# foolwood/SiamMask

Hardware: NVIDIA H100
Metric: search-region frames/sec (127/255 SiamMask-sharp) (higher is better)
Workload: dtype f16x3 (hi+lo split fp16 operands on wgmma, f32 accumulate; f32 CUDA-core xcorr/refine)

## Files before the change

### siammask_b200/csrc/common.cuh

```cuda
#pragma once
#include <cuda.h>
#include <cuda_fp16.h>
#include <cuda_runtime.h>
#include <cstdint>
#include <cstdio>
#include <stdexcept>
#include <string>
#include <vector>

struct sm_image_desc;

namespace smk {

struct Act {
  __half* hi = nullptr;
  __half* lo = nullptr;
  int B = 0, H = 0, W = 0, C = 0;
  int sexp = 0;
  __host__ __device__ size_t numel() const { return (size_t)B * H * W * C; }
  __host__ __device__ int M() const { return B * H * W; }
};

struct ConvGeom {
  int Cin, Cout, KH, KW, stride, pad, dil;
  __host__ __device__ int out_size(int in) const { return (in + 2 * pad - dil * (KH - 1) - 1) / stride + 1; }
};

enum OutMode : int { OUT_NHWC_SPLIT = 0, OUT_NHWC_F32 = 1, OUT_NCHW_F32 = 2 };

struct Epilogue {
  const float* alpha = nullptr;
  const float* beta = nullptr;
  const __half* res_hi = nullptr;
  const __half* res_lo = nullptr;
  __half* out_hi = nullptr;
  __half* out_lo = nullptr;
  float* out_f32 = nullptr;
  int out_mode = OUT_NHWC_SPLIT;
  int relu = 0;
  int* ovf = nullptr;
};

__device__ __forceinline__ void flag_if_out_of_range(float absmax, int* ovf) {
  if (ovf != nullptr && !(absmax <= 65504.f)) atomicOr(ovf, 1);
}
constexpr int kStatusBadSlot = 2;

struct GemmSegment {
  CUtensorMap tmA[2];
  int kind;
  int mode;
  int num_kb, cblks, KW;
  int stride, pad, dil;
  int b_col0;
};

struct GemmParams {
  GemmSegment seg[2];
  int nseg;
  CUtensorMap tmB[2];
  int M, Cout, Ho, Wo;
  int n_tiles, m_tiles;
  int reverse_m;
  Epilogue ep;
};

struct GemmInput {
  Act in;
  ConvGeom g;
  int w_col0;
};

struct TrackerHp {
  double context_amount, penalty_k, window_influence, lr;
  int32_t exemplar_size, instance_size, total_stride, base_size, out_size, reserved;
};

struct CudaError : std::runtime_error {
  using std::runtime_error::runtime_error;
};

#define SMK_CUDA(expr)                                                                              \
  do {                                                                                              \
    cudaError_t _e = (expr);                                                                        \
    if (_e != cudaSuccess)                                                                          \
      throw smk::CudaError(std::string(#expr) + " failed: " + cudaGetErrorString(_e) + " at " +    \
                           __FILE__ + ":" + std::to_string(__LINE__));                              \
  } while (0)

#define SMK_CHECK(cond, msg)                                                                        \
  do {                                                                                              \
    if (!(cond)) throw std::runtime_error(std::string("check failed: ") + #cond + " — " + (msg));   \
  } while (0)

template <typename K>
inline void ensure_dynamic_smem(K kernel, int bytes, unsigned long long& done_mask) {
  int dev = 0;
  SMK_CUDA(cudaGetDevice(&dev));
  const unsigned long long bit = 1ull << (dev & 63);
  if (done_mask & bit) return;
  SMK_CUDA(cudaFuncSetAttribute(kernel, cudaFuncAttributeMaxDynamicSharedMemorySize, bytes));
  done_mask |= bit;
}


bool gemm_conv_supported(const ConvGeom& g);
void launch_gemm_conv(const Act& in, const ConvGeom& g, const __half* w_hi, const __half* w_lo, int cout_pad,
                      const Epilogue& ep, int nsplit, int num_sms, cudaStream_t st);
void launch_gemm_multi(const GemmInput* convs, int nconv, const Act* residual, int res_col0, const __half* w_hi,
                       const __half* w_lo, int cout_pad, int w_ld, const Epilogue& ep, int nsplit, int num_sms,
                       cudaStream_t st, bool reverse_m = false);

CUtensorMap make_map_tiled_nd(const __half* base, int rank, const uint64_t* dims, const uint64_t* strides_bytes,
                              const uint32_t* box, int swizzle_bytes);

bool patch_conv_supported(const Act& in, const ConvGeom& g);
void launch_conv3x3_patch(const Act& in, const ConvGeom& g, const __half* w_hi, const __half* w_lo, int w_ld,
                          const Epilogue& ep, int nsplit, int num_sms, cudaStream_t st);

void launch_stem_tc(const float* x_nchw, int B, int S, const __half* w_hi, const __half* w_lo, const float* alpha,
                    const float* beta, Act out, int num_sms, cudaStream_t st, int* ovf = nullptr);

void launch_ref_conv(const Act& in, const ConvGeom& g, const float* w_krsc_cout, const Epilogue& ep,
                     cudaStream_t st);
void launch_stem(const float* x_nchw, int B, int S, const float* w, const float* alpha, const float* beta, Act out,
                 cudaStream_t st);
void launch_maxpool3s2(const Act& in, Act out, cudaStream_t st);
void launch_xcorr_nhwc(const Act& x, int c_off, const __half* k_hi, const __half* k_lo, int kh, int kw, Act out,
                       float mul, int* ovf, cudaStream_t st, const int32_t* slots = nullptr, int num_slots = 0);
void launch_scatter_slots(const __half* src_hi, const __half* src_lo, __half* dst_hi, __half* dst_lo,
                          const int32_t* slots, int B, int num_slots, int n, int* status, cudaStream_t st);
void launch_paste_labels(const float* masks, int side, const double* maps, const uint8_t* anno, const int32_t* obj_off,
                         const int32_t* objects, int G, int H, int W, double seg_thr, uint8_t* labels, cudaStream_t st,
                         const sm_image_desc* desc = nullptr);
void launch_paste_labels_iou(const float* masks, int side, const double* maps, const uint8_t* anno,
                             const int32_t* obj_off, const int32_t* objects, const int32_t* target_ids, int G, int H,
                             int W, double seg_thr, uint8_t* labels, const double* thrs, int T, int32_t* counts,
                             cudaStream_t st, const sm_image_desc* desc = nullptr);
void launch_label_boxes(const uint8_t* anno, int G, int H, int W, const int32_t* queries, int Q, int32_t* boxes,
                        cudaStream_t st, const sm_image_desc* desc = nullptr);
void launch_vot_overlap(const float* poly_a, const float* poly_b, int B, int W, int H, float* overlap, cudaStream_t st,
                        const int32_t* wh = nullptr);
void launch_absmax(const Act& a, float* slot, cudaStream_t st);
void launch_xcorr_nchw_f32(const float* x, const float* k, float* out, int planes, int H, int W, int kh, int kw,
                           cudaStream_t st);
int launch_xcorr_bulk_f32(const float* x, const float* k, float* out, int planes, int H, int W, int kh, int kw,
                          cudaStream_t st);
void launch_crop_center(const Act& in, int crop, Act out, cudaStream_t st);
void launch_refine_crop(const Act& in, const int32_t* pos, int pos_max, int scale, int padv, int size, Act out,
                        cudaStream_t st);
void launch_gather_corr(const Act& corr, const int32_t* pos, float* out, float mul, cudaStream_t st);
void launch_gather_mask_col(const float* mask, const int32_t* pos, int B, int C, int R, float* out, cudaStream_t st);
void launch_deconv(const float* p3, const float* w, const float* bias, float* out, int B, int Cin, int N,
                   int cout, cudaStream_t st);
void launch_split_to_f32(const Act& in, float* out, cudaStream_t st, float mul = 1.f);
void launch_import_nchw(const float* x_nchw, Act out, cudaStream_t st);
void launch_warp_affine(const float* src, int sh, int sw, const double* maps, float* dst, int dh, int dw, float border,
                        int B, cudaStream_t st, const sm_image_desc* dst_desc = nullptr);
void launch_tracker_prepare(int B, const double* state, const int32_t* avg, const TrackerHp& hp, int32_t* boxes,
                            double* tsz, double* aux, cudaStream_t st);
void launch_tracker_update(int B, double* state, const float* rec, const double* aux, const int32_t* imsize,
                           const TrackerHp& hp, int A, int R, double* maps, double* out, cudaStream_t st,
                           const double* hp_table = nullptr);
void launch_crop_resize(const uint8_t* frames, size_t frame_stride, int H, int W, const int32_t* box, int B, int model,
                        float* out, cudaStream_t st, const int32_t* frame_idx = nullptr,
                        const sm_image_desc* desc = nullptr);
void launch_select(const float* cls, const float* loc, const float* anchors, const float* window, const double* tsz,
                   int B, int A, int R, double penalty_k, double window_influence, int32_t* best_idx, int32_t* pos,
                   float* rec, cudaStream_t st, const double* hp = nullptr);
void launch_mask_iou(const float* masks, int side, const double* maps, const uint8_t* anno, const int32_t* video, int B,
                     int H, int W, const double* thrs, int T, int32_t* counts, cudaStream_t st);
void launch_small_conv3x3_maps(const float* a, const float* b, int B, int Hi, int Wi, int Ho, int Wo, int Cin, int Cout,
                               const int* ymap, const int* xmap, const float* w, const float* bias, int relu,
                               float* out, cudaStream_t st);
std::vector<int> nearest_index_table(int out_size, int in_size);
int gemm_cout_pad(int cout);

}
```

### siammask_b200/csrc/conv_gemm_sm90.cu

```cuda
#include "common.cuh"
#include "ptx.cuh"

#include <cstdlib>
#include <cstring>
#include <mutex>
#include <unordered_map>

namespace smk {

namespace {

constexpr int BLOCK_M = 128;
constexpr int BLOCK_K = 64;
constexpr int CIN_GRAIN = 64;
constexpr int MMA_K = 16;
constexpr int SMEM_LIMIT = 227 * 1024;
constexpr int NUM_CONSUMER_WARPS = 8;
constexpr int NUM_THREADS = 128 + 32 * NUM_CONSUMER_WARPS;
constexpr int PRODUCER_REGS = 40;
constexpr int CONSUMER_REGS = 232;

template <int BLOCK_N, int NSPLIT>
struct Cfg {
  static constexpr int A_TILE_BYTES = BLOCK_M * BLOCK_K * 2;
  static constexpr int B_TILE_BYTES = BLOCK_N * BLOCK_K * 2;
  static constexpr int STAGE_BYTES = NSPLIT * (A_TILE_BYTES + B_TILE_BYTES);
  static constexpr int RAW_STAGES = (SMEM_LIMIT - 2048) / STAGE_BYTES;
  static constexpr int STAGES = RAW_STAGES > 6 ? 6 : RAW_STAGES;
  static constexpr int SMEM_BYTES = STAGES * STAGE_BYTES + 1024  + 256 ;
  static constexpr int ACC = BLOCK_N / 2;
  static_assert(STAGES >= 2, "pipeline needs at least two stages");
  static_assert(BLOCK_N % 16 == 0 && BLOCK_N >= 16 && BLOCK_N <= 128, "N tile (register accumulators)");
  static_assert(B_TILE_BYTES % 1024 == 0, "stage parts stay 1024-aligned (swizzle atoms)");
  static_assert(SMEM_BYTES <= SMEM_LIMIT, "shared memory budget");
};

__device__ __forceinline__ int m_block(const GemmParams& p, int tile) {
  const int mb = tile / p.n_tiles;
  return p.reverse_m ? p.m_tiles - 1 - mb : mb;
}

template <int BLOCK_N, int NSPLIT>
__global__ void __launch_bounds__(NUM_THREADS, 1) conv_gemm_kernel(const __grid_constant__ GemmParams p) {
  using C = Cfg<BLOCK_N, NSPLIT>;
  constexpr int STAGES = C::STAGES;
  constexpr int A_TILE_BYTES = C::A_TILE_BYTES;

  extern __shared__ uint8_t smem_raw[];
  uint8_t* smem = reinterpret_cast<uint8_t*>((reinterpret_cast<uintptr_t>(smem_raw) + 1023) & ~uintptr_t(1023));
  uint64_t* full_bar = reinterpret_cast<uint64_t*>(smem + STAGES * C::STAGE_BYTES);
  uint64_t* empty_bar = full_bar + STAGES;

  const int warp = __shfl_sync(0xffffffffu, (int)(threadIdx.x >> 5), 0);
  const int lane = threadIdx.x & 31;
  const int num_tiles = p.m_tiles * p.n_tiles;

  if (threadIdx.x == 0) {
    for (int i = 0; i < NSPLIT; ++i) {
      for (int sgi = 0; sgi < p.nseg; ++sgi) tma_prefetch_desc(&p.seg[sgi].tmA[i]);
      tma_prefetch_desc(&p.tmB[i]);
    }
    for (int s = 0; s < STAGES; ++s) {
      mbar_init(&full_bar[s], 1);
      mbar_init(&empty_bar[s], NUM_CONSUMER_WARPS);
    }
    fence_barrier_init();
  }
  __syncthreads();

  if (warp < 4) {
    setmaxnreg_dec<PRODUCER_REGS>();
    if (warp != 0) return;
    const bool leader = elect_one();
    int stage = 0;
    uint32_t phase = 0;
    auto acquire = [&](uint32_t bytes) {
      mbar_wait(&empty_bar[stage], phase ^ 1);
      if (leader) mbar_arrive_expect_tx(&full_bar[stage], bytes);
    };
    auto load_2d = [&](void* dst, const CUtensorMap* map, int c0, int c1) {
      if (leader) tma_load_2d(dst, map, &full_bar[stage], c0, c1);
    };
    for (int tile = blockIdx.x; tile < num_tiles; tile += gridDim.x) {
      const int m0 = m_block(p, tile) * BLOCK_M;
      const int n0 = (tile % p.n_tiles) * BLOCK_N;
      const int q = m0 % p.Wo;
      const int t = m0 / p.Wo;
      const int pq = t % p.Ho;
      const int nb = t / p.Ho;
      for (int sgi = 0; sgi < p.nseg; ++sgi) {
        const GemmSegment& sg = p.seg[sgi];
        if (sg.kind == 1) {
#pragma unroll 1
          for (int kb = 0; kb < BLOCK_N / BLOCK_K; ++kb) {
            acquire(C::STAGE_BYTES);
            uint8_t* st = smem + stage * C::STAGE_BYTES;
#pragma unroll
            for (int s = 0; s < NSPLIT; ++s) {
              load_2d(st + s * A_TILE_BYTES, &sg.tmA[s], n0 + kb * BLOCK_K, m0);
              load_2d(st + NSPLIT * A_TILE_BYTES + s * C::B_TILE_BYTES, &p.tmB[s], sg.b_col0 + n0 + kb * BLOCK_K, n0);
            }
            __syncwarp();
            if (++stage == STAGES) { stage = 0; phase ^= 1; }
          }
          continue;
        }
        const int wb = q * sg.stride - sg.pad;
        const int hb = pq * sg.stride - sg.pad;
#pragma unroll 1
        for (int kb = 0; kb < sg.num_kb; ++kb) {
          acquire(C::STAGE_BYTES);
          uint8_t* st = smem + stage * C::STAGE_BYTES;
          const int tap = kb / sg.cblks;
          const int c0 = (kb - tap * sg.cblks) * BLOCK_K;
#pragma unroll
          for (int s = 0; s < NSPLIT; ++s) {
            uint8_t* a_dst = st + s * A_TILE_BYTES;
            if (sg.mode == 0) {
              load_2d(a_dst, &sg.tmA[s], c0, m0);
            } else if (leader) {
              const int r = tap / sg.KW;
              const int sx = tap - r * sg.KW;
              tma_load_im2col_4d(a_dst, &sg.tmA[s], &full_bar[stage], c0, wb, hb, nb,
                                 static_cast<uint16_t>(sx * sg.dil), static_cast<uint16_t>(r * sg.dil));
            }
            load_2d(st + NSPLIT * A_TILE_BYTES + s * C::B_TILE_BYTES, &p.tmB[s], sg.b_col0 + kb * BLOCK_K, n0);
          }
          __syncwarp();
          if (++stage == STAGES) { stage = 0; phase ^= 1; }
        }
      }
    }
    return;
  }

  setmaxnreg_inc<CONSUMER_REGS>();
  const int wg = (warp >> 2) - 1;
  const int wl = warp & 3;
  const Epilogue& ep = p.ep;
  const int HoWo = p.Ho * p.Wo;
  float acc[C::ACC];
  float acc2[C::ACC];
  int stage = 0;
  uint32_t phase = 0;
  for (int tile = blockIdx.x; tile < num_tiles; tile += gridDim.x) {
#pragma unroll
    for (int i = 0; i < C::ACC; ++i) { acc[i] = 0.f; acc2[i] = 0.f; }
    int prev = -1;
    for (int sgi = 0; sgi < p.nseg; ++sgi) {
      const GemmSegment& sg = p.seg[sgi];
      const bool ident = sg.kind == 1;
      const int nkb = ident ? BLOCK_N / BLOCK_K : sg.num_kb;
#pragma unroll 1
      for (int kb = 0; kb < nkb; ++kb) {
        mbar_wait(&full_bar[stage], phase);
        const uint32_t a_hi = smem_u32(smem + stage * C::STAGE_BYTES) + wg * (64 * BLOCK_K * 2);
        const uint32_t b_hi = smem_u32(smem + stage * C::STAGE_BYTES) + NSPLIT * A_TILE_BYTES;
        const uint64_t da_hi0 = wgmma_desc_kmajor<128>(a_hi);
        const uint64_t db_hi0 = wgmma_desc_kmajor<128>(b_hi);
        const uint64_t da_lo0 = wgmma_desc_kmajor<128>(a_hi + A_TILE_BYTES);
        const uint64_t db_lo0 = wgmma_desc_kmajor<128>(b_hi + C::B_TILE_BYTES);
        wgmma_fence();
#pragma unroll
        for (int k = 0; k < BLOCK_K / MMA_K; ++k) {
          const uint64_t kadd = static_cast<uint64_t>(k * MMA_K * 2 / 16);
          wgmma_f16<BLOCK_N>(acc, da_hi0 + kadd, db_hi0 + kadd);
          if constexpr (NSPLIT == 2) {
            wgmma_f16<BLOCK_N>(acc2, da_hi0 + kadd, db_lo0 + kadd);
            wgmma_f16<BLOCK_N>(acc2, da_lo0 + kadd, db_hi0 + kadd);
          }
        }
        wgmma_commit();
        wgmma_wait<1>();
        if (prev >= 0) {
          __syncwarp();
          if (lane == 0) mbar_arrive(&empty_bar[prev]);
        }
        prev = stage;
        if (++stage == STAGES) { stage = 0; phase ^= 1; }
      }
    }
    wgmma_wait<0>();
    fence_regs(acc);
    if constexpr (NSPLIT == 2) fence_regs(acc2);
    __syncwarp();
    if (lane == 0) mbar_arrive(&empty_bar[prev]);

    const int row0 = m_block(p, tile) * BLOCK_M + wg * 64 + wl * 16 + (lane >> 2);
    const int col0 = (tile % p.n_tiles) * BLOCK_N + 2 * (lane & 3);
    float amax = 0.f;
#pragma unroll
    for (int h = 0; h < 2; ++h) {
      const int m = row0 + 8 * h;
      if (m >= p.M) continue;
      const int b = m / HoWo;
      const int hw = m - b * HoWo;
#pragma unroll
      for (int j = 0; j < BLOCK_N / 8; ++j) {
        const int n = col0 + 8 * j;
        float v0 = acc[4 * j + 2 * h], v1 = acc[4 * j + 2 * h + 1];
        if constexpr (NSPLIT == 2) {
          v0 += acc2[4 * j + 2 * h];
          v1 += acc2[4 * j + 2 * h + 1];
        }
        const float2 al = __ldg(reinterpret_cast<const float2*>(ep.alpha + n));
        const float2 be = __ldg(reinterpret_cast<const float2*>(ep.beta + n));
        v0 = fmaf(v0, al.x, be.x);
        v1 = fmaf(v1, al.y, be.y);
        const size_t off = static_cast<size_t>(m) * p.Cout + n;
        if (ep.res_hi != nullptr) {
          const float2 f = __half22float2(*reinterpret_cast<const __half2*>(ep.res_hi + off));
          v0 += f.x;
          v1 += f.y;
          if (ep.res_lo != nullptr) {
            const float2 l = __half22float2(*reinterpret_cast<const __half2*>(ep.res_lo + off));
            v0 += l.x;
            v1 += l.y;
          }
        }
        if (ep.relu) {
          v0 = fmaxf(v0, 0.f);
          v1 = fmaxf(v1, 0.f);
        }
        if (ep.out_mode == OUT_NHWC_SPLIT) {
          amax = fmaxf(amax, fmaxf(fabsf(v0), fabsf(v1)));
          const __half2 hv = __floats2half2_rn(v0, v1);
          const float2 hf = __half22float2(hv);
          *reinterpret_cast<__half2*>(ep.out_hi + off) = hv;
          if (ep.out_lo != nullptr)
            *reinterpret_cast<__half2*>(ep.out_lo + off) = __floats2half2_rn(v0 - hf.x, v1 - hf.y);
        } else if (ep.out_mode == OUT_NHWC_F32) {
          *reinterpret_cast<float2*>(ep.out_f32 + off) = make_float2(v0, v1);
        } else if (n < p.Cout) {
          float* dst = ep.out_f32 + (static_cast<size_t>(b) * p.Cout + n) * HoWo + hw;
          __stcs(dst, v0);
          if (n + 1 < p.Cout) __stcs(dst + HoWo, v1);
        }
      }
    }
    if (ep.out_mode == OUT_NHWC_SPLIT) flag_if_out_of_range(amax, ep.ovf);
  }
}

using EncodeTiledFn = CUresult (*)(CUtensorMap*, CUtensorMapDataType, cuuint32_t, void*, const cuuint64_t*,
                                   const cuuint64_t*, const cuuint32_t*, const cuuint32_t*, CUtensorMapInterleave,
                                   CUtensorMapSwizzle, CUtensorMapL2promotion, CUtensorMapFloatOOBfill);
using EncodeIm2colFn = CUresult (*)(CUtensorMap*, CUtensorMapDataType, cuuint32_t, void*, const cuuint64_t*,
                                    const cuuint64_t*, const int*, const int*, cuuint32_t, cuuint32_t,
                                    const cuuint32_t*, CUtensorMapInterleave, CUtensorMapSwizzle,
                                    CUtensorMapL2promotion, CUtensorMapFloatOOBfill);

struct DriverApi {
  EncodeTiledFn tiled = nullptr;
  EncodeIm2colFn im2col = nullptr;
  int driver_version = 0;
};

const DriverApi& driver_api() {
  static DriverApi api;
  static std::once_flag once;
  std::call_once(once, [] {
    void* fn = nullptr;
    cudaDriverEntryPointQueryResult q;
    SMK_CUDA(cudaGetDriverEntryPoint("cuTensorMapEncodeTiled", &fn, cudaEnableDefault, &q));
    SMK_CHECK(fn != nullptr && q == cudaDriverEntryPointSuccess, "cuTensorMapEncodeTiled not available");
    api.tiled = reinterpret_cast<EncodeTiledFn>(fn);
    fn = nullptr;
    SMK_CUDA(cudaGetDriverEntryPoint("cuTensorMapEncodeIm2col", &fn, cudaEnableDefault, &q));
    SMK_CHECK(fn != nullptr && q == cudaDriverEntryPointSuccess, "cuTensorMapEncodeIm2col not available");
    api.im2col = reinterpret_cast<EncodeIm2colFn>(fn);
    SMK_CUDA(cudaDriverGetVersion(&api.driver_version));
  });
  return api;
}

struct MapKey {
  uint64_t v[16];
  bool operator==(const MapKey& o) const { return std::memcmp(v, o.v, sizeof v) == 0; }
};
struct MapKeyHash {
  size_t operator()(const MapKey& k) const {
    uint64_t h = 0x9E3779B97F4A7C15ull;
    for (uint64_t x : k.v) { h ^= x + 0x9E3779B97F4A7C15ull + (h << 6) + (h >> 2); }
    return (size_t)h;
  }
};
template <typename F>
CUtensorMap cached_map(const MapKey& key, F&& encode) {
  static std::mutex mu;
  static std::unordered_map<MapKey, CUtensorMap, MapKeyHash> cache;
  int dev = 0;
  cudaGetDevice(&dev);
  MapKey k = key;
  k.v[15] = (uint64_t)dev;
  std::lock_guard<std::mutex> lock(mu);
  auto it = cache.find(k);
  if (it != cache.end()) return it->second;
  if (cache.size() > 65536) cache.clear();
  CUtensorMap m = encode();
  cache.emplace(k, m);
  return m;
}

CUtensorMap make_map_2d_raw(const __half* base, uint64_t inner, uint64_t outer, uint32_t box_inner, uint32_t box_outer) {
  CUtensorMap m;
  cuuint64_t dims[2] = {inner, outer};
  cuuint64_t strides[1] = {inner * sizeof(__half)};
  cuuint32_t box[2] = {box_inner, box_outer};
  cuuint32_t estr[2] = {1, 1};
  const CUtensorMapSwizzle sw = box_inner == 64 ? CU_TENSOR_MAP_SWIZZLE_128B : CU_TENSOR_MAP_SWIZZLE_64B;
  CUresult r = driver_api().tiled(&m, CU_TENSOR_MAP_DATA_TYPE_FLOAT16, 2, const_cast<__half*>(base), dims, strides,
                                  box, estr, CU_TENSOR_MAP_INTERLEAVE_NONE, sw,
                                  CU_TENSOR_MAP_L2_PROMOTION_L2_256B, CU_TENSOR_MAP_FLOAT_OOB_FILL_NONE);
  SMK_CHECK(r == CUDA_SUCCESS, "cuTensorMapEncodeTiled failed, code " + std::to_string((int)r));
  return m;
}

CUtensorMap make_map_2d(const __half* base, uint64_t inner, uint64_t outer, uint32_t box_inner, uint32_t box_outer) {
  MapKey k{};
  k.v[0] = 1; k.v[1] = (uint64_t)base; k.v[2] = inner; k.v[3] = outer; k.v[4] = box_inner; k.v[5] = box_outer;
  return cached_map(k, [&] { return make_map_2d_raw(base, inner, outer, box_inner, box_outer); });
}

CUtensorMap make_map_im2col_raw(const __half* base, const Act& in, const ConvGeom& g, int bk) {
  CUtensorMap m;
  cuuint64_t dims[4] = {(cuuint64_t)in.C, (cuuint64_t)in.W, (cuuint64_t)in.H, (cuuint64_t)in.B};
  cuuint64_t strides[3] = {(cuuint64_t)in.C * 2, (cuuint64_t)in.W * in.C * 2, (cuuint64_t)in.H * in.W * in.C * 2};
  int lower[2] = {-g.pad, -g.pad};
  int upper[2] = {g.pad - (g.KW - 1) * g.dil, g.pad - (g.KH - 1) * g.dil};
  cuuint32_t estr[4] = {1, (cuuint32_t)g.stride, (cuuint32_t)g.stride, 1};
  const DriverApi& api = driver_api();
  CUresult r = api.im2col(&m, CU_TENSOR_MAP_DATA_TYPE_FLOAT16, 4, const_cast<__half*>(base), dims, strides, lower,
                          upper, bk, BLOCK_M, estr, CU_TENSOR_MAP_INTERLEAVE_NONE,
                          bk == 64 ? CU_TENSOR_MAP_SWIZZLE_128B : CU_TENSOR_MAP_SWIZZLE_64B,
                          CU_TENSOR_MAP_L2_PROMOTION_L2_256B, CU_TENSOR_MAP_FLOAT_OOB_FILL_NONE);
  SMK_CHECK(r == CUDA_SUCCESS, "cuTensorMapEncodeIm2col failed, code " + std::to_string((int)r));
  if (api.driver_version <= 13010 && in.numel() * sizeof(__half) < 131072)
    reinterpret_cast<uint64_t*>(&m)[1] &= ~(1ull << 21);
  return m;
}

CUtensorMap make_map_im2col(const __half* base, const Act& in, const ConvGeom& g, int bk) {
  MapKey k{};
  k.v[0] = 3; k.v[1] = (uint64_t)base;
  k.v[2] = ((uint64_t)in.B << 32) | (uint32_t)in.H; k.v[3] = ((uint64_t)in.W << 32) | (uint32_t)in.C;
  k.v[4] = ((uint64_t)g.KH << 32) | (uint32_t)g.KW; k.v[5] = ((uint64_t)g.stride << 32) | (uint32_t)g.pad;
  k.v[6] = ((uint64_t)g.dil << 32) | (uint32_t)bk;
  return cached_map(k, [&] { return make_map_im2col_raw(base, in, g, bk); });
}

template <int BLOCK_N, int NSPLIT>
void launch_cfg(const GemmParams& p, int num_sms, cudaStream_t st) {
  using C = Cfg<BLOCK_N, NSPLIT>;
  auto kern = conv_gemm_kernel<BLOCK_N, NSPLIT>;
  static unsigned long long attr_done = 0;
  ensure_dynamic_smem(kern, C::SMEM_BYTES, attr_done);
  const int tiles = p.m_tiles * p.n_tiles;
  const int grid = tiles < num_sms ? tiles : num_sms;
  kern<<<grid, NUM_THREADS, C::SMEM_BYTES, st>>>(p);
  SMK_CUDA(cudaGetLastError());
}

}

static CUtensorMap make_map_2d_any_raw(const __half* base, uint64_t inner, uint64_t outer, uint32_t box_inner, uint32_t box_outer,
                            int swizzle_bytes) {
  CUtensorMap m;
  cuuint64_t dims[2] = {inner, outer};
  cuuint64_t strides[1] = {inner * sizeof(__half)};
  cuuint32_t box[2] = {box_inner, box_outer};
  cuuint32_t estr[2] = {1, 1};
  const CUtensorMapSwizzle sw = swizzle_bytes == 128 ? CU_TENSOR_MAP_SWIZZLE_128B
                                : swizzle_bytes == 64 ? CU_TENSOR_MAP_SWIZZLE_64B : CU_TENSOR_MAP_SWIZZLE_32B;
  CUresult r = driver_api().tiled(&m, CU_TENSOR_MAP_DATA_TYPE_FLOAT16, 2, const_cast<__half*>(base), dims, strides,
                                  box, estr, CU_TENSOR_MAP_INTERLEAVE_NONE, sw, CU_TENSOR_MAP_L2_PROMOTION_L2_128B,
                                  CU_TENSOR_MAP_FLOAT_OOB_FILL_NONE);
  SMK_CHECK(r == CUDA_SUCCESS, "cuTensorMapEncodeTiled failed, code " + std::to_string((int)r));
  return m;
}

CUtensorMap make_map_2d_any(const __half* base, uint64_t inner, uint64_t outer, uint32_t box_inner, uint32_t box_outer,
                            int swizzle_bytes) {
  MapKey k{};
  k.v[0] = 5; k.v[1] = (uint64_t)base; k.v[2] = inner; k.v[3] = outer; k.v[4] = box_inner; k.v[5] = box_outer;
  k.v[6] = (uint64_t)swizzle_bytes;
  return cached_map(k, [&] { return make_map_2d_any_raw(base, inner, outer, box_inner, box_outer, swizzle_bytes); });
}

static CUtensorMap make_map_tiled_nd_raw(const __half* base, int rank, const uint64_t* dims,
                                         const uint64_t* strides_bytes, const uint32_t* box, int swizzle_bytes) {
  SMK_CHECK(rank >= 2 && rank <= 5, "tensor map rank");
  CUtensorMap m;
  cuuint64_t d[5], sb[4];
  cuuint32_t bx[5], es[5];
  for (int i = 0; i < rank; ++i) { d[i] = dims[i]; bx[i] = box[i]; es[i] = 1; }
  for (int i = 0; i + 1 < rank; ++i) sb[i] = strides_bytes[i];
  const CUtensorMapSwizzle sw = swizzle_bytes == 128 ? CU_TENSOR_MAP_SWIZZLE_128B
                                : swizzle_bytes == 64 ? CU_TENSOR_MAP_SWIZZLE_64B
                                : swizzle_bytes == 32 ? CU_TENSOR_MAP_SWIZZLE_32B : CU_TENSOR_MAP_SWIZZLE_NONE;
  CUresult r = driver_api().tiled(&m, CU_TENSOR_MAP_DATA_TYPE_FLOAT16, (cuuint32_t)rank, const_cast<__half*>(base), d, sb,
                                  bx, es, CU_TENSOR_MAP_INTERLEAVE_NONE, sw, CU_TENSOR_MAP_L2_PROMOTION_L2_256B,
                                  CU_TENSOR_MAP_FLOAT_OOB_FILL_NONE);
  SMK_CHECK(r == CUDA_SUCCESS, "cuTensorMapEncodeTiled (nd) failed, code " + std::to_string((int)r));
  return m;
}

CUtensorMap make_map_tiled_nd(const __half* base, int rank, const uint64_t* dims, const uint64_t* strides_bytes,
                              const uint32_t* box, int swizzle_bytes) {
  SMK_CHECK(rank >= 2 && rank <= 5, "tensor map rank");
  MapKey k{};
  k.v[0] = 4 | ((uint64_t)rank << 8) | ((uint64_t)swizzle_bytes << 16);
  k.v[1] = (uint64_t)base;
  for (int i = 0; i < rank; ++i) k.v[2 + i] = dims[i] | ((uint64_t)box[i] << 40);
  for (int i = 0; i + 1 < rank; ++i) k.v[7 + i] = strides_bytes[i];
  return cached_map(k, [&] { return make_map_tiled_nd_raw(base, rank, dims, strides_bytes, box, swizzle_bytes); });
}

bool gemm_conv_supported(const ConvGeom& g) { return g.Cin % CIN_GRAIN == 0 && g.Cout >= 1; }

int gemm_cout_pad(int cout) {
  if (cout <= 16) return 16;
  if (cout <= 32) return 32;
  if (cout <= 64) return 64;
  if (cout <= 128) return 128;
  return (cout + 255) / 256 * 256;
}

void launch_gemm_conv(const Act& in, const ConvGeom& g, const __half* w_hi, const __half* w_lo, int cout_pad,
                      const Epilogue& ep, int nsplit, int num_sms, cudaStream_t st) {
  GemmInput gi{in, g, 0};
  launch_gemm_multi(&gi, 1, nullptr, -1, w_hi, w_lo, cout_pad, g.KH * g.KW * g.Cin, ep, nsplit, num_sms, st);
}

void launch_gemm_multi(const GemmInput* convs, int nconv, const Act* residual, int res_col0, const __half* w_hi,
                       const __half* w_lo, int cout_pad, int w_ld, const Epilogue& ep_in, int nsplit, int num_sms,
                       cudaStream_t st, bool reverse_m) {
  SMK_CHECK(nconv >= 1 && nconv <= 2, "1 or 2 convolution segments");
  SMK_CHECK(nconv + (residual != nullptr ? 1 : 0) <= 2, "at most two K segments");
  Epilogue ep = ep_in;
  const ConvGeom& g0 = convs[0].g;
  const Act& in0 = convs[0].in;
  const int Ho = g0.out_size(in0.H), Wo = g0.out_size(in0.W);
  GemmParams p;
  p.M = in0.B * Ho * Wo;
  p.Cout = g0.Cout;
  p.Ho = Ho;
  p.Wo = Wo;
  const int block_n = cout_pad < 128 ? cout_pad : 128;
  const int bk = BLOCK_K;
  SMK_CHECK(cout_pad % block_n == 0, "cout_pad must be a multiple of the N tile");
  if (ep.out_mode != OUT_NCHW_F32) SMK_CHECK(g0.Cout == cout_pad, "NHWC outputs need Cout to match the padded tile width");
  p.n_tiles = cout_pad / block_n;
  p.m_tiles = (p.M + BLOCK_M - 1) / BLOCK_M;
  p.reverse_m = reverse_m ? 1 : 0;
  p.nseg = 0;
  for (int i = 0; i < nconv; ++i) {
    const ConvGeom& g = convs[i].g;
    const Act& in = convs[i].in;
    SMK_CHECK(gemm_conv_supported(g), "Cin must be a multiple of 64 for the tensor-core conv");
    SMK_CHECK(in.C == g.Cin && g.Cout == g0.Cout && in.B == in0.B, "segment channels/batch mismatch");
    SMK_CHECK(g.out_size(in.H) == Ho && g.out_size(in.W) == Wo, "segments must produce the same output size");
    SMK_CHECK(nsplit == 1 || (in.lo != nullptr && w_lo != nullptr), "exact mode needs lo planes");
    GemmSegment& sg = p.seg[p.nseg++];
    sg.kind = 0;
    sg.cblks = g.Cin / bk;
    sg.num_kb = g.KH * g.KW * sg.cblks;
    sg.KW = g.KW;
    sg.stride = g.stride;
    sg.pad = g.pad;
    sg.dil = g.dil;
    sg.mode = (g.KH == 1 && g.KW == 1 && g.stride == 1 && g.pad == 0) ? 0 : 1;
    sg.b_col0 = convs[i].w_col0;
    SMK_CHECK(sg.b_col0 % 64 == 0 && sg.b_col0 + g.KH * g.KW * g.Cin <= w_ld, "weight column range");
    for (int s = 0; s < nsplit; ++s) {
      const __half* a = s == 0 ? in.hi : in.lo;
      sg.tmA[s] = sg.mode == 0 ? make_map_2d(a, g.Cin, (uint64_t)in.M(), bk, BLOCK_M) : make_map_im2col(a, in, g, bk);
    }
    if (nsplit == 1) sg.tmA[1] = sg.tmA[0];
  }
  if (residual != nullptr) {
    SMK_CHECK(res_col0 >= 0 && res_col0 % 64 == 0 && res_col0 + g0.Cout <= w_ld && block_n % 64 == 0,
              "identity segment needs a diagonal block in the packed weights");
    SMK_CHECK(residual->C == g0.Cout && residual->M() == p.M, "residual shape");
    SMK_CHECK(nsplit == 1 || residual->lo != nullptr, "exact mode residual needs both planes");
    GemmSegment& sg = p.seg[p.nseg++];
    sg.kind = 1;
    sg.mode = 0;
    sg.num_kb = block_n / bk;
    sg.cblks = sg.KW = sg.stride = sg.dil = 1;
    sg.pad = 0;
    sg.b_col0 = res_col0;
    for (int s = 0; s < nsplit; ++s)
      sg.tmA[s] = make_map_2d(s == 0 ? residual->hi : residual->lo, g0.Cout, (uint64_t)p.M, bk, BLOCK_M);
    if (nsplit == 1) sg.tmA[1] = sg.tmA[0];
    ep.res_hi = ep.res_lo = nullptr;
  }
  if (p.nseg == 1) p.seg[1] = p.seg[0];
  for (int s = 0; s < nsplit; ++s)
    p.tmB[s] = make_map_2d(s == 0 ? w_hi : w_lo, (uint64_t)w_ld, cout_pad, bk, block_n);
  if (nsplit == 1) p.tmB[1] = p.tmB[0];
  p.ep = ep;

#define SMK_DISPATCH(BN)                                             \
  case BN:                                                           \
    if (nsplit == 2) launch_cfg<BN, 2>(p, num_sms, st);              \
    else launch_cfg<BN, 1>(p, num_sms, st);                          \
    break;
  switch (block_n) {
    SMK_DISPATCH(16)
    SMK_DISPATCH(32)
    SMK_DISPATCH(64)
    SMK_DISPATCH(128)
    default: SMK_CHECK(false, "unsupported N tile");
  }
#undef SMK_DISPATCH
}

}
```

### siammask_b200/csrc/engine.cu

```cuda
#include "../../include/siammask_b200.h"
#include "common.cuh"

#include <algorithm>
#include <cmath>
#include <cstdlib>
#include <cstring>
#include <map>
#include <memory>
#include <unordered_map>

namespace smk {

namespace {

constexpr float BN_EPS = 1e-5f;
constexpr size_t ALIGN = 256;
inline size_t align_up(size_t x) { return (x + ALIGN - 1) / ALIGN * ALIGN; }

thread_local std::string g_last_error;

struct ConvW {
  ConvGeom g{};
  int cout_pad = 0;
  bool gemm_ok = false;
  std::string conv_key, bn_key;
  ConvGeom g2{};
  std::string conv_key2, bn_key2;
  bool fused2 = false, has_diag = false;
  int w_ld = 0, col2 = 0, col_diag = -1;
  size_t off_beta2 = 0;
  float* beta2 = nullptr;
  size_t off_whi = 0, off_wlo = 0, off_wref = 0, off_alpha = 0, off_beta = 0;
  __half* w_hi = nullptr;
  __half* w_lo = nullptr;
  float* w_ref = nullptr;
  float* alpha = nullptr;
  float* beta = nullptr;
  int s_in = 0, s_in2 = 0, s_res = 0, s_out = 0;
  bool f32_out = false;
  std::vector<std::string> cat_keys;
  std::string src_in, src_in2, src_res;
  std::vector<double> shift, shift2;
};

constexpr const char* kSearchCat = "heads.conv_search_cat";

struct F32T {
  float* p = nullptr;
  int B = 0, H = 0, W = 0, C = 0;
};

struct ProfRec {
  std::string name, cat;
  double flops = 0, bytes = 0;
  cudaEvent_t e0 = nullptr, e1 = nullptr;
};

struct Arena {
  uint8_t* base = nullptr;
  size_t cap = 0, off = 0, peak = 0;
  bool measure = false;
  void reset() { off = 0; }
  void* alloc(size_t bytes) {
    off = align_up(off);
    void* p = base + off;
    off += bytes;
    peak = std::max(peak, off);
    if (!measure) SMK_CHECK(off <= cap, "workspace arena exhausted");
    return p;
  }
};

struct Lane {
  int id = 0;
  Arena search, refine;
  cudaStream_t own = nullptr;
  cudaStream_t aux[3] = {nullptr, nullptr, nullptr};
  int cap_B = 0;
};
constexpr int kMaxLanes = 2;
constexpr int kLaneMinB = 8;

}

class Engine {
 public:
  explicit Engine(const sm_config& cfg);
  ~Engine() { release(); }

  void load_weights(const sm_tensor_desc* t, int n);
  void adopt_weights();
  void calibrate(int B, const float* z, const float* x, cudaStream_t st);
  int status();
  void weight_blob(void** p, size_t* bytes) { *p = blob_; *bytes = blob_bytes_; }

  void do_template(int slot0, int B, const float* z, cudaStream_t st, const int32_t* slots = nullptr);
  void do_track(int slot0, int B, const float* x, float* cls, float* loc, float* mask, int flags, cudaStream_t st);
  void do_refine(int B, const int32_t* pos, float* out, cudaStream_t st);
  void set_graphs(bool on) { use_graphs_ = on; }
  void track_host(int slot0, int B, const float* xh, float* clsh, float* loch, const int32_t* posh, float* maskh,
                  cudaStream_t st);
  int track_host_async(int slot0, int B, const float* xh, float* clsh, float* loch, const int32_t* posh, float* maskh,
                       cudaStream_t st);
  void host_wait(int ticket);
  struct StepIO {
    const float* x = nullptr;
    const double* tsz = nullptr;
    const float* anchors = nullptr;
    const float* window = nullptr;
    double penalty_k = 0, window_influence = 0;
    const double* hp = nullptr;
    int flags = 0;
    float* cls = nullptr; float* loc = nullptr; float* mask = nullptr;
    int32_t* best = nullptr; int32_t* pos = nullptr; float* rec = nullptr;
    float* refine = nullptr;
    float* mask_col = nullptr;
  };
  void do_step(int slot0, int B, const StepIO& io, cudaStream_t st, const int32_t* slots = nullptr);
  int step_host_async(int slot0, int B, const sm_step_io& io, cudaStream_t st);
  void do_export(const char* what, float* out, int64_t* shape4, cudaStream_t st);

  void set_profiling(bool on) { profiling_ = on; }
  std::string profile_dump();
  int64_t launches() const { return launches_; }
  size_t bytes() const { return total_bytes_; }
  const sm_config& cfg() const { return cfg_; }
  int score_size() const { return R_; }

 private:
  void construct(const sm_config& cfg);
  ConvW& add_layer(const std::string& conv_key, const std::string& bn_key, ConvGeom g);
  void build_layer_table();
  void assign_blob_layout();
  void size_arenas();
  void fold_layer(ConvW& L, const std::map<std::string, const sm_tensor_desc*>& sd, uint8_t* host);
  void quantize_layer(ConvW& L, uint8_t* host);
  void quantize_stem(uint8_t* host);
  void write_scale_table(uint8_t* host);
  void read_scale_table(const uint8_t* host);
  void upload_blob();
  int tscale(const std::string& name) const {
    auto it = tscale_.find(name);
    return it == tscale_.end() ? 0 : it->second;
  }
  void note_tensor(const Act& a, const std::string& name, cudaStream_t st, const Act* same_scale_as = nullptr);
  void note_tensor(const F32T& t, const std::string& name);
  Act alloc_act(Arena& ar, int B, int H, int W, int C);
  F32T alloc_f32(Arena& ar, int B, int H, int W, int C);
  Act conv(const Act& in, const ConvW& L, bool relu, const Act* res, Arena& ar, cudaStream_t st,
           const Act* in2 = nullptr);
  void conv_into(const Act& in, const ConvW& L, Epilogue ep, cudaStream_t st, const Act* res = nullptr,
                 const Act* in2 = nullptr);
  F32T conv_f32(const Act& in, const ConvW& L, bool relu, Arena& ar, cudaStream_t st);
  Act backbone(const float* x, int B, int S, Arena& ar, std::map<std::string, Act>* keep, cudaStream_t st);
  F32T small(const F32T& a, const F32T* b, int Ho, const ConvW& L, bool relu, float* out_override, Arena& ar,
             cudaStream_t st);
  const ConvW& L(const std::string& k) const {
    auto it = layers_.find(k);
    SMK_CHECK(it != layers_.end(), "unknown layer " + k);
    return it->second;
  }
  const int* updown_map(int out, int in) const {
    auto it = maps_.find(out * 1000 + in);
    SMK_CHECK(it != maps_.end(), "no upsample map");
    return it->second;
  }

  sm_config cfg_;
  bool exact_;
  int num_sms_ = 132;
  int R_ = 0;
  std::map<std::string, ConvW> layers_;
  std::vector<std::string> layer_order_;
  size_t off_deconv_w_ = 0, off_deconv_b_ = 0, off_ones_ = 0;
  size_t off_stem_whi_ = 0, off_stem_wlo_ = 0, off_stem_alpha_ = 0;
  __half* stem_whi_ = nullptr;
  __half* stem_wlo_ = nullptr;
  float* stem_alpha_ = nullptr;
  float* deconv_w_ = nullptr;
  float* deconv_b_ = nullptr;
  float* ones_ = nullptr;
  uint8_t* blob_ = nullptr;
  size_t blob_bytes_ = 0;
  bool weights_ready_ = false;
  std::vector<uint8_t> host_blob_;
  size_t off_scales_ = 0;
  std::map<std::string, int> tscale_;
  int* ovf_flag_ = nullptr;
  bool calibrating_ = false;
  std::unordered_map<const void*, std::string> tensor_name_;
  std::vector<std::string> absmax_names_;
  float* absmax_dev_ = nullptr;
  static constexpr int kAbsmaxSlots = 256;

  Arena templ_arena_;
  Lane lanes_[kMaxLanes];
  int n_lanes_ = 1;
  __half* kcache_hi_ = nullptr;
  __half* kcache_lo_ = nullptr;
  __half* kscatter_ = nullptr;
  int n_branches_ = 2;
  float* stage_x_[2] = {nullptr, nullptr};
  float* stage_cls_[2] = {nullptr, nullptr};
  float* stage_loc_[2] = {nullptr, nullptr};
  float* stage_mask_[2] = {nullptr, nullptr};
  int32_t* stage_pos_[2] = {nullptr, nullptr};
  double* stage_tsz_[2] = {nullptr, nullptr};
  float* stage_rec_[2] = {nullptr, nullptr};
  int32_t* stage_best_[2] = {nullptr, nullptr};
  float* stage_maskcol_[2] = {nullptr, nullptr};
  float* mask_raw_ = nullptr;
  void step_lane(Lane& ln, int slot0, int B, const StepIO& io, cudaStream_t st, const int32_t* slots = nullptr);
  void release();
  cudaStream_t h2d_stream_ = nullptr, d2h_stream_ = nullptr;
  cudaEvent_t h2d_done_[2] = {nullptr, nullptr}, d2h_done_[2] = {nullptr, nullptr};
  bool set_busy_[2] = {false, false};
  uint64_t host_calls_ = 0;
  int* maps_dev_ = nullptr;
  std::map<int, const int*> maps_;

  std::map<std::string, Act> templ_named_;
  std::map<std::string, Act>* taps_ = nullptr;
  std::map<std::string, F32T>* taps_f32_ = nullptr;
  struct CallState {
    std::map<std::string, Act> named[kMaxLanes];
    std::map<std::string, F32T> named_f32[kMaxLanes];
    int split_n = 1;
    int split_off[kMaxLanes + 1] = {};
    int last_B = 0;
    bool have_mask_feats = false;
  };
  CallState state_;

  int64_t launches_ = 0;
  size_t total_bytes_ = 0;
  bool measuring_ = false;

  std::unordered_map<const void*, int> last_end_;
  int end_of(const Act& a) const {
    auto it = last_end_.find(a.hi);
    return it == last_end_.end() ? +1 : it->second;
  }

  struct GraphEntry {
    int seen = 0;
    cudaGraphExec_t exec = nullptr;
    CallState state;
    int64_t launches = 0;
  };
  bool use_graphs_ = false;
  std::map<std::vector<uint64_t>, GraphEntry> graphs_;
  void track_lane(Lane& ln, int slot0, int B, const float* x, float* cls, float* loc, float* mask, int flags,
                  cudaStream_t st, const int32_t* slots = nullptr);
  void refine_lane(Lane& ln, int B, const int32_t* pos, float* out, cudaStream_t st);
  bool lanes_dirty_ = false;
  cudaEvent_t lane_done_[2][kMaxLanes] = {};
  void join_lanes(cudaStream_t st) {
    if (!lanes_dirty_) return;
    for (int l = 0; l < n_lanes_; ++l) order_after(lanes_[l].own, st);
    lanes_dirty_ = false;
  }
  static int lanes_for(int n_lanes, int B) { return std::max(1, std::min(n_lanes, B / kLaneMinB)); }
  static int chunk(int B, int nl, int l) { return B / nl + (l < B % nl ? 1 : 0); }
  void split_batch(int B) {
    CallState& s = state_;
    s.split_n = (profiling_ || calibrating_) ? 1 : lanes_for(n_lanes_, B);
    s.split_off[0] = 0;
    for (int l = 0; l < s.split_n; ++l) {
      s.split_off[l + 1] = s.split_off[l] + chunk(B, s.split_n, l);
      SMK_CHECK(chunk(B, s.split_n, l) <= lanes_[l].cap_B, "lane workspace too small for this batch");
    }
  }
  static constexpr int kJoined = -1;
  template <typename F>
  void run_lanes(cudaStream_t st, int set, F&& body);
  struct Copy { void* dst; const void* src; size_t bytes; };
  int next_set();
  template <typename Coupled, typename F>
  int host_call(int t, int B, bool mask_feats, cudaStream_t st, std::initializer_list<Copy> h2d,
                std::initializer_list<Copy> d2h, Coupled&& coupled, F&& body);
  template <typename F>
  void run_with_graph(const std::vector<uint64_t>& key, cudaStream_t st, F&& body) {
    if (!use_graphs_ || profiling_ || calibrating_) { body(); return; }
    GraphEntry& ge = graphs_[key];
    if (ge.exec != nullptr) {
      SMK_CUDA(cudaGraphLaunch(ge.exec, st));
      state_ = ge.state;
      launches_ += ge.launches;
      return;
    }
    if (ge.seen++ == 0) { body(); return; }
    const int64_t l0 = launches_;
    cudaGraph_t graph = nullptr;
    SMK_CUDA(cudaStreamBeginCapture(st, cudaStreamCaptureModeThreadLocal));
    try {
      body();
    } catch (...) {
      cudaStreamEndCapture(st, &graph);
      if (graph) cudaGraphDestroy(graph);
      throw;
    }
    SMK_CUDA(cudaStreamEndCapture(st, &graph));
    SMK_CUDA(cudaGraphInstantiate(&ge.exec, graph, 0));
    SMK_CUDA(cudaGraphDestroy(graph));
    ge.state = state_;
    ge.launches = launches_ - l0;
    SMK_CUDA(cudaGraphLaunch(ge.exec, st));
  }

  static constexpr int kAux = 3;
  std::vector<cudaEvent_t> sync_events_;
  size_t sync_next_ = 0;
  cudaEvent_t next_sync_event() {
    cudaEvent_t e = sync_events_[sync_next_];
    sync_next_ = (sync_next_ + 1) % sync_events_.size();
    return e;
  }
  bool concurrent() const { return !profiling_ && !calibrating_; }
  void order_after(cudaStream_t from, cudaStream_t to) {
    if (from == to || measuring_) return;
    cudaEvent_t e = next_sync_event();
    SMK_CUDA(cudaEventRecord(e, from));
    SMK_CUDA(cudaStreamWaitEvent(to, e, 0));
  }

  bool profiling_ = false;
  std::vector<ProfRec> prof_;
  std::vector<cudaEvent_t> event_pool_;
  cudaEvent_t get_event() {
    if (!event_pool_.empty()) { cudaEvent_t e = event_pool_.back(); event_pool_.pop_back(); return e; }
    cudaEvent_t e;
    SMK_CUDA(cudaEventCreate(&e));
    return e;
  }
  template <typename F>
  void launch(cudaStream_t st, int n, const std::string& name, const char* cat, double flops, double bytes,
              F&& enqueue) {
    if (measuring_) return;
    const bool row = profiling_;
    const size_t idx = prof_.size();
    if (row) {
      prof_.push_back(ProfRec{name, cat, flops, bytes, get_event(), get_event()});
      cudaEventRecord(prof_[idx].e0, st);
    }
    enqueue();
    if (row) cudaEventRecord(prof_[idx].e1, st);
    launches_ += n;
  }
};


ConvW& Engine::add_layer(const std::string& conv_key, const std::string& bn_key, ConvGeom g) {
  ConvW w;
  w.g = g;
  w.conv_key = conv_key;
  w.bn_key = bn_key;
  w.gemm_ok = gemm_conv_supported(g);
  w.cout_pad = w.gemm_ok ? gemm_cout_pad(g.Cout) : g.Cout;
  w.w_ld = g.KH * g.KW * g.Cin;
  layer_order_.push_back(conv_key);
  return layers_[conv_key] = w;
}

void Engine::build_layer_table() {
  const std::string F = "features.features.";
  add_layer(F + "conv1", F + "bn1", {3, 64, 7, 7, 2, 0, 1});
  struct LayerSpec { const char* name; int planes, blocks, stride, dilation; };
  const LayerSpec specs[3] = {{"layer1", 64, 3, 1, 1}, {"layer2", 128, 4, 2, 1}, {"layer3", 256, 6, 1, 2}};
  int inplanes = 64;
  for (const auto& sp : specs) {
    for (int i = 0; i < sp.blocks; ++i) {
      const std::string P = F + sp.name + "." + std::to_string(i) + ".";
      int stride = 1, dil = sp.dilation;
      if (i == 0) {
        stride = sp.stride;
        dil = sp.dilation > 1 ? sp.dilation / 2 : 1;
        ConvGeom ds;
        if (sp.stride == 1 && sp.dilation == 1) ds = {inplanes, sp.planes * 4, 1, 1, 1, 0, 1};
        else if (sp.dilation > 1) ds = {inplanes, sp.planes * 4, 3, 3, sp.stride, sp.dilation / 2, sp.dilation / 2};
        else ds = {inplanes, sp.planes * 4, 3, 3, sp.stride, 0, 1};
        add_layer(P + "downsample.0", P + "downsample.1", ds);
      }
      const int pad = dil > 1 ? dil : 2 - stride;
      add_layer(P + "conv1", P + "bn1", {inplanes, sp.planes, 1, 1, 1, 0, 1});
      add_layer(P + "conv2", P + "bn2", {sp.planes, sp.planes, 3, 3, stride, pad, dil});
      ConvW& c3 = add_layer(P + "conv3", P + "bn3", {sp.planes, sp.planes * 4, 1, 1, 1, 0, 1});
      if (i == 0) {
        const ConvW& ds = layers_[P + "downsample.0"];
        c3.fused2 = true;
        c3.g2 = ds.g;
        c3.conv_key2 = ds.conv_key;
        c3.bn_key2 = ds.bn_key;
      } else {
        c3.has_diag = true;
      }
      inplanes = sp.planes * 4;
    }
  }
  add_layer("features.downsample.downsample.0", "features.downsample.downsample.1", {1024, 256, 1, 1, 1, 0, 1});
  std::vector<std::pair<std::string, int>> heads = {{"rpn_model.cls.", 2 * cfg_.anchor_num},
                                                    {"rpn_model.loc.", 4 * cfg_.anchor_num}};
  if (cfg_.with_mask) heads.push_back({"mask_model.mask.", 63 * 63});
  n_branches_ = (int)heads.size();
  for (auto& h : heads) {
    add_layer(h.first + "conv_kernel.0", h.first + "conv_kernel.1", {256, 256, 3, 3, 1, 0, 1});
    add_layer(h.first + "conv_search.0", h.first + "conv_search.1", {256, 256, 3, 3, 1, 0, 1});
    add_layer(h.first + "head.0", h.first + "head.1", {256, 256, 1, 1, 1, 0, 1});
    add_layer(h.first + "head.3", "", {256, h.second, 1, 1, 1, 0, 1});
  }
  {
    ConvW& cat = add_layer(kSearchCat, "", {256, 256 * n_branches_, 3, 3, 1, 0, 1});
    for (auto& h : heads) cat.cat_keys.push_back(h.first + "conv_search.0");
  }
  if (cfg_.with_mask) {
    const std::string R = "refine_model.";
    auto c3 = [&](const std::string& k, int ci, int co) { add_layer(R + k, "", {ci, co, 3, 3, 1, 1, 1}); };
    c3("v0.0", 64, 16);  c3("v0.2", 16, 4);
    c3("v1.0", 256, 64); c3("v1.2", 64, 16);
    c3("v2.0", 512, 128); c3("v2.2", 128, 32);
    c3("h2.0", 32, 32);  c3("h2.2", 32, 32);
    c3("h1.0", 16, 16);  c3("h1.2", 16, 16);
    c3("h0.0", 4, 4);    c3("h0.2", 4, 4);
    c3("post0", 32, 16); c3("post1", 16, 4); c3("post2", 4, 1);
  }
}

void Engine::assign_blob_layout() {
  size_t off = 0;
  for (const auto& k : layer_order_) {
    ConvW& w = layers_[k];
    const size_t K = (size_t)w.g.KH * w.g.KW * w.g.Cin;
    w.w_ld = (int)K;
    if (w.fused2) { w.col2 = w.w_ld; w.w_ld += w.g2.KH * w.g2.KW * w.g2.Cin; }
    if (w.has_diag) { w.col_diag = w.w_ld; w.w_ld += w.g.Cout; }
    if (w.gemm_ok) {
      w.off_whi = off; off = align_up(off + (size_t)w.cout_pad * w.w_ld * sizeof(__half));
      w.off_wlo = off; off = align_up(off + (size_t)w.cout_pad * w.w_ld * sizeof(__half));
    }
    w.off_beta2 = off; off = align_up(off + (size_t)w.cout_pad * sizeof(float));
    w.off_wref = off;  off = align_up(off + K * w.g.Cout * sizeof(float));
    w.off_alpha = off; off = align_up(off + (size_t)w.cout_pad * sizeof(float));
    w.off_beta = off;  off = align_up(off + (size_t)w.cout_pad * sizeof(float));
  }
  off_ones_ = off; off = align_up(off + 4096 * sizeof(float));
  off_stem_whi_ = off; off = align_up(off + 64 * 192 * sizeof(__half));
  off_stem_wlo_ = off; off = align_up(off + 64 * 192 * sizeof(__half));
  off_stem_alpha_ = off; off = align_up(off + 64 * sizeof(float));
  if (cfg_.with_mask) {
    off_deconv_w_ = off; off = align_up(off + (size_t)256 * 7200 * sizeof(float));
    off_deconv_b_ = off; off = align_up(off + 32 * sizeof(float));
  }
  off_scales_ = off; off = align_up(off + (layer_order_.size() * 4 + 4) * sizeof(int32_t));
  blob_bytes_ = off;
}

Engine::Engine(const sm_config& cfg) : cfg_(cfg), exact_(cfg.precision == SM_PRECISION_EXACT) {
  try {
    construct(cfg);
  } catch (...) {
    release();
    throw;
  }
}

void Engine::construct(const sm_config& cfg) {
  SMK_CHECK(cfg.search_size >= 127 && (cfg.search_size - 127) % 8 == 0, "search_size must be 127 + 8k");
  SMK_CHECK(cfg.max_batch >= 1 && cfg.num_slots >= cfg.max_batch, "need num_slots >= max_batch >= 1");
  SMK_CHECK(cfg.anchor_num >= 1, "anchor_num");
  int dev = 0;
  SMK_CUDA(cudaGetDevice(&dev));
  cudaDeviceProp prop;
  SMK_CUDA(cudaGetDeviceProperties(&prop, dev));
  SMK_CHECK(prop.major == 9 && prop.minor == 0, "siammask_b200 kernels are built for sm_90a only (found sm_" +
                                                    std::to_string(prop.major) + std::to_string(prop.minor) + ")");
  num_sms_ = prop.multiProcessorCount;
  R_ = (cfg.search_size - 127) / 8 + 1 + 8;

  build_layer_table();
  assign_blob_layout();
  SMK_CUDA(cudaMalloc(&blob_, blob_bytes_));
  SMK_CUDA(cudaMalloc(&ovf_flag_, sizeof(int)));
  SMK_CUDA(cudaMemset(ovf_flag_, 0, sizeof(int)));
  for (auto& kv : layers_) {
    ConvW& w = kv.second;
    if (w.gemm_ok) {
      w.w_hi = reinterpret_cast<__half*>(blob_ + w.off_whi);
      w.w_lo = reinterpret_cast<__half*>(blob_ + w.off_wlo);
    }
    w.w_ref = reinterpret_cast<float*>(blob_ + w.off_wref);
    w.alpha = reinterpret_cast<float*>(blob_ + w.off_alpha);
    w.beta = reinterpret_cast<float*>(blob_ + w.off_beta);
    w.beta2 = reinterpret_cast<float*>(blob_ + w.off_beta2);
  }
  ones_ = reinterpret_cast<float*>(blob_ + off_ones_);
  stem_whi_ = reinterpret_cast<__half*>(blob_ + off_stem_whi_);
  stem_wlo_ = reinterpret_cast<__half*>(blob_ + off_stem_wlo_);
  stem_alpha_ = reinterpret_cast<float*>(blob_ + off_stem_alpha_);
  if (cfg_.with_mask) {
    deconv_w_ = reinterpret_cast<float*>(blob_ + off_deconv_w_);
    deconv_b_ = reinterpret_cast<float*>(blob_ + off_deconv_b_);
  }

  n_lanes_ = lanes_for(kMaxLanes, cfg.max_batch);
  lanes_[0].cap_B = cfg.max_batch;
  for (int B = 1; B <= cfg.max_batch; ++B) {
    const int nl = lanes_for(n_lanes_, B);
    for (int l = 0; l < nl; ++l) lanes_[l].cap_B = std::max(lanes_[l].cap_B, chunk(B, nl, l));
  }
  size_arenas();
  SMK_CUDA(cudaMalloc(&templ_arena_.base, templ_arena_.cap));
  for (int l = 0; l < n_lanes_; ++l) {
    Lane& ln = lanes_[l];
    ln.id = l;
    SMK_CUDA(cudaMalloc(&ln.search.base, ln.search.cap));
    if (cfg_.with_mask) SMK_CUDA(cudaMalloc(&ln.refine.base, ln.refine.cap));
    for (int i = 0; i < kAux; ++i) SMK_CUDA(cudaStreamCreateWithFlags(&ln.aux[i], cudaStreamNonBlocking));
    SMK_CUDA(cudaStreamCreateWithFlags(&ln.own, cudaStreamNonBlocking));
  }
  const size_t kc = (size_t)n_branches_ * cfg.num_slots * 25 * 256;
  SMK_CUDA(cudaMalloc(&kcache_hi_, kc * sizeof(__half)));
  SMK_CUDA(cudaMalloc(&kcache_lo_, kc * sizeof(__half)));
  SMK_CUDA(cudaMemset(kcache_hi_, 0, kc * sizeof(__half)));
  SMK_CUDA(cudaMemset(kcache_lo_, 0, kc * sizeof(__half)));

  const size_t B = cfg.max_batch, S = cfg.search_size, A = cfg.anchor_num;
  for (int i = 0; i < 2; ++i) {
    SMK_CUDA(cudaMalloc(&stage_x_[i], B * 3 * S * S * sizeof(float)));
    SMK_CUDA(cudaMalloc(&stage_cls_[i], B * 2 * A * R_ * R_ * sizeof(float)));
    SMK_CUDA(cudaMalloc(&stage_loc_[i], B * 4 * A * R_ * R_ * sizeof(float)));
    SMK_CUDA(cudaMalloc(&stage_mask_[i], B * 127 * 127 * sizeof(float)));
    SMK_CUDA(cudaMalloc(&stage_pos_[i], B * 2 * sizeof(int32_t)));
    SMK_CUDA(cudaMalloc(&stage_tsz_[i], B * 2 * sizeof(double)));
    SMK_CUDA(cudaMalloc(&stage_rec_[i], B * 8 * sizeof(float)));
    SMK_CUDA(cudaMalloc(&stage_best_[i], B * sizeof(int32_t)));
    if (cfg_.with_mask) SMK_CUDA(cudaMalloc(&stage_maskcol_[i], B * 3969 * sizeof(float)));
    SMK_CUDA(cudaEventCreateWithFlags(&h2d_done_[i], cudaEventDisableTiming));
    SMK_CUDA(cudaEventCreateWithFlags(&d2h_done_[i], cudaEventDisableTiming));
    for (int l = 0; l < kMaxLanes; ++l) SMK_CUDA(cudaEventCreateWithFlags(&lane_done_[i][l], cudaEventDisableTiming));
  }
  SMK_CUDA(cudaStreamCreateWithFlags(&h2d_stream_, cudaStreamNonBlocking));
  SMK_CUDA(cudaStreamCreateWithFlags(&d2h_stream_, cudaStreamNonBlocking));

  const int pairs[6][2] = {{31, 15}, {61, 31}, {127, 61}, {15, 15}, {31, 31}, {61, 61}};
  std::vector<int> all;
  std::vector<size_t> offs;
  for (auto& pr : pairs) {
    offs.push_back(all.size());
    auto t = nearest_index_table(pr[0], pr[1]);
    all.insert(all.end(), t.begin(), t.end());
  }
  SMK_CUDA(cudaMalloc(&maps_dev_, all.size() * sizeof(int)));
  SMK_CUDA(cudaMemcpy(maps_dev_, all.data(), all.size() * sizeof(int), cudaMemcpyHostToDevice));
  for (int i = 0; i < 6; ++i) maps_[pairs[i][0] * 1000 + pairs[i][1]] = maps_dev_ + offs[i];
  sync_events_.resize(64);
  for (auto& e : sync_events_) SMK_CUDA(cudaEventCreateWithFlags(&e, cudaEventDisableTiming));

  size_t lane_bytes = 0;
  for (auto& ln : lanes_) lane_bytes += ln.search.cap + ln.refine.cap;
  total_bytes_ = blob_bytes_ + templ_arena_.cap + lane_bytes + 2 * kc * sizeof(__half) +
                 2 * (B * 3 * S * S + B * 6 * A * R_ * R_ + B * 127 * 127) * sizeof(float);
}

void Engine::release() {
  cudaFree(blob_);
  cudaFree(templ_arena_.base);
  for (auto& ln : lanes_) {
    cudaFree(ln.search.base);
    cudaFree(ln.refine.base);
    for (int i = 0; i < kAux; ++i) if (ln.aux[i]) cudaStreamDestroy(ln.aux[i]);
    if (ln.own) cudaStreamDestroy(ln.own);
  }
  cudaFree(kcache_hi_);
  cudaFree(kcache_lo_);
  cudaFree(kscatter_);
  for (int i = 0; i < 2; ++i) {
    cudaFree(stage_x_[i]); cudaFree(stage_cls_[i]); cudaFree(stage_loc_[i]); cudaFree(stage_mask_[i]); cudaFree(stage_pos_[i]);
    cudaFree(stage_tsz_[i]); cudaFree(stage_rec_[i]); cudaFree(stage_best_[i]); cudaFree(stage_maskcol_[i]);
    if (h2d_done_[i]) cudaEventDestroy(h2d_done_[i]);
    if (d2h_done_[i]) cudaEventDestroy(d2h_done_[i]);
    for (int l = 0; l < kMaxLanes; ++l) if (lane_done_[i][l]) cudaEventDestroy(lane_done_[i][l]);
  }
  if (h2d_stream_) cudaStreamDestroy(h2d_stream_);
  if (d2h_stream_) cudaStreamDestroy(d2h_stream_);
  cudaFree(maps_dev_);
  cudaFree(mask_raw_);
  cudaFree(ovf_flag_);
  cudaFree(absmax_dev_);
  for (auto e : sync_events_) cudaEventDestroy(e);
  for (auto e : event_pool_) cudaEventDestroy(e);
  for (auto& kv : graphs_) if (kv.second.exec) cudaGraphExecDestroy(kv.second.exec);
}

void Engine::size_arenas() {
  measuring_ = true;
  Arena templ;
  templ.measure = true;
  backbone(nullptr, cfg_.max_batch, 127, templ, nullptr, nullptr);
  templ_arena_.cap = align_up(templ.peak + (1u << 20));
  const int max_flags = cfg_.with_mask ? (SM_TRACK_MASK_FEATURES | SM_TRACK_MASK_HEAD) : 0;
  for (int l = 0; l < n_lanes_; ++l) {
    Lane probe;
    probe.search.measure = probe.refine.measure = true;
    const int B = lanes_[l].cap_B;
    for (int flags = 0; flags <= max_flags; ++flags)
      track_lane(probe, 0, B, nullptr, nullptr, nullptr, nullptr, flags, nullptr, nullptr);
    float out;
    if (cfg_.with_mask) refine_lane(probe, B, nullptr, &out, nullptr);
    lanes_[l].search.cap = align_up(probe.search.peak + (1u << 20));
    if (cfg_.with_mask) lanes_[l].refine.cap = align_up(probe.refine.peak + (1u << 16));
  }
  measuring_ = false;
  state_ = CallState();
}


namespace {
const float* find_tensor(const std::map<std::string, const sm_tensor_desc*>& sd, const std::string& name,
                         size_t expect_numel) {
  auto it = sd.find(name);
  SMK_CHECK(it != sd.end(), "checkpoint is missing tensor '" + name + "'");
  size_t n = 1;
  for (int i = 0; i < it->second->ndim; ++i) n *= (size_t)it->second->shape[i];
  SMK_CHECK(n == expect_numel, "tensor '" + name + "' has " + std::to_string(n) + " elements, expected " +
                                   std::to_string(expect_numel));
  return it->second->data;
}
}

namespace {
void fold_affine(const std::map<std::string, const sm_tensor_desc*>& sd, const std::string& conv_key,
                 const std::string& bn_key, int cout, std::vector<double>& scale, std::vector<double>& shift) {
  scale.assign(cout, 1.0);
  shift.assign(cout, 0.0);
  if (!bn_key.empty()) {
    const float* gm = find_tensor(sd, bn_key + ".weight", cout);
    const float* bt = find_tensor(sd, bn_key + ".bias", cout);
    const float* mu = find_tensor(sd, bn_key + ".running_mean", cout);
    const float* var = find_tensor(sd, bn_key + ".running_var", cout);
    for (int n = 0; n < cout; ++n) {
      scale[n] = (double)gm[n] / std::sqrt((double)var[n] + (double)BN_EPS);
      shift[n] = (double)bt[n] - (double)mu[n] * scale[n];
    }
  } else {
    const float* b = find_tensor(sd, conv_key + ".bias", cout);
    for (int n = 0; n < cout; ++n) shift[n] = b[n];
  }
}
}

void Engine::fold_layer(ConvW& L, const std::map<std::string, const sm_tensor_desc*>& sd, uint8_t* host) {
  const ConvGeom& g = L.g;
  const size_t K = (size_t)g.KH * g.KW * g.Cin;
  if (!L.cat_keys.empty()) {
    float* w_cat = reinterpret_cast<float*>(host + L.off_wref);
    L.shift.assign(g.Cout, 0.0);
    int n0 = 0;
    for (const auto& key : L.cat_keys) {
      const ConvW& src = layers_.at(key);
      SMK_CHECK(src.g.Cin == g.Cin && src.g.KH == g.KH && !src.shift.empty(), "concatenated layers must share their geometry");
      const float* ws = reinterpret_cast<const float*>(host + src.off_wref);
      for (size_t k = 0; k < K; ++k)
        for (int n = 0; n < src.g.Cout; ++n) w_cat[k * g.Cout + n0 + n] = ws[k * src.g.Cout + n];
      for (int n = 0; n < src.g.Cout; ++n) L.shift[n0 + n] = src.shift[n];
      n0 += src.g.Cout;
    }
    return;
  }
  const float* w = find_tensor(sd, L.conv_key + ".weight", K * g.Cout);
  std::vector<double> scale;
  fold_affine(sd, L.conv_key, L.bn_key, g.Cout, scale, L.shift);
  float* w_ref = reinterpret_cast<float*>(host + L.off_wref);
  const int HW = g.KH * g.KW;
  for (int n = 0; n < g.Cout; ++n)
    for (int c = 0; c < g.Cin; ++c)
      for (int t = 0; t < HW; ++t)
        w_ref[((size_t)t * g.Cin + c) * g.Cout + n] = (float)((double)w[((size_t)n * g.Cin + c) * HW + t] * scale[n]);
}

namespace {
int weight_exp(float amax) {
  const int e = amax > 0.f ? (int)std::floor(std::log2(16384.0 / (double)amax)) : 0;
  return std::max(-24, std::min(24, e));
}
}

void Engine::quantize_layer(ConvW& L, uint8_t* host) {
  const ConvGeom& g = L.g;
  const size_t K = (size_t)g.KH * g.KW * g.Cin;
  const size_t K2 = L.fused2 ? (size_t)L.g2.KH * L.g2.KW * L.g2.Cin : 0;
  const float* w_ref = reinterpret_cast<const float*>(host + L.off_wref);
  const ConvW* L2 = L.fused2 ? &layers_.at(L.conv_key2) : nullptr;
  const float* w_ref2 = L2 ? reinterpret_cast<const float*>(host + L2->off_wref) : nullptr;
  float* alpha = reinterpret_cast<float*>(host + L.off_alpha);
  float* beta = reinterpret_cast<float*>(host + L.off_beta);
  float* beta2 = reinterpret_cast<float*>(host + L.off_beta2);
  __half* w_hi = L.gemm_ok ? reinterpret_cast<__half*>(host + L.off_whi) : nullptr;
  __half* w_lo = L.gemm_ok ? reinterpret_cast<__half*>(host + L.off_wlo) : nullptr;
  for (int n = 0; n < L.cout_pad; ++n) { alpha[n] = 0.f; beta[n] = 0.f; beta2[n] = 0.f; }
  const size_t ld = (size_t)L.w_ld;
  const int d2 = L.s_in - L.s_in2;
  for (int n = 0; n < g.Cout; ++n) {
    float amax = 0.f;
    for (size_t k = 0; k < K; ++k) amax = std::max(amax, std::fabs(w_ref[k * g.Cout + n]));
    for (size_t k = 0; k < K2; ++k) amax = std::max(amax, std::fabs(std::ldexp(w_ref2[k * g.Cout + n], d2)));
    beta[n] = (float)std::ldexp(L.shift[n], L.s_out);
    beta2[n] = (float)std::ldexp(L.shift[n] + (L2 ? L2->shift[n] : 0.0), L.s_out);
    alpha[n] = std::ldexp(1.f, L.s_out - L.s_in);
    if (!L.gemm_ok) continue;
    int e = weight_exp(amax);
    if (L.has_diag) {
      const int d = L.s_in - L.s_res;
      e = std::max(-14 - d, std::min(14 - d, e));
      SMK_CHECK(e >= -24 && e <= 24, "activation scales of a residual block are too far apart");
    }
    alpha[n] = std::ldexp(1.f, L.s_out - L.s_in - e);
    __half* rh = w_hi + (size_t)n * ld;
    __half* rl = w_lo + (size_t)n * ld;
    for (size_t k = 0; k < K; ++k) {
      const float fw = std::ldexp(w_ref[k * g.Cout + n], e);
      const __half h = __float2half_rn(fw);
      rh[k] = h;
      rl[k] = __float2half_rn(fw - __half2float(h));
    }
    for (size_t k = 0; k < K2; ++k) {
      const float fw = std::ldexp(w_ref2[k * g.Cout + n], e + d2);
      const __half h = __float2half_rn(fw);
      rh[L.col2 + k] = h;
      rl[L.col2 + k] = __float2half_rn(fw - __half2float(h));
    }
    if (L.has_diag) rh[L.col_diag + n] = __float2half_rn(std::ldexp(1.f, e + L.s_in - L.s_res));
  }
}

void Engine::quantize_stem(uint8_t* host) {
  ConvW& stem = layers_["features.features.conv1"];
  const int s_out = tscale("stem");
  stem.s_out = s_out;
  const float* wref = reinterpret_cast<const float*>(host + stem.off_wref);
  __half* sh = reinterpret_cast<__half*>(host + off_stem_whi_);
  __half* sl = reinterpret_cast<__half*>(host + off_stem_wlo_);
  float* sa = reinterpret_cast<float*>(host + off_stem_alpha_);
  float* sb = reinterpret_cast<float*>(host + stem.off_beta);
  for (int n = 0; n < 64; ++n) {
    float amax = 0.f;
    for (int k = 0; k < 147; ++k) amax = std::max(amax, std::fabs(wref[(size_t)k * 64 + n]));
    const int e = weight_exp(amax);
    sa[n] = std::ldexp(1.f, s_out - e);
    sb[n] = (float)std::ldexp(stem.shift[n], s_out);
    for (int k = 0; k < 147; ++k) {
      const float fw = std::ldexp(wref[(size_t)k * 64 + n], e);
      const __half h = __float2half_rn(fw);
      sh[n * 192 + k] = h;
      sl[n * 192 + k] = __float2half_rn(fw - __half2float(h));
    }
  }
}

static const char* kNamedTensors[4] = {"stem", "corr_cls", "corr_loc", "corr_mask"};
void Engine::write_scale_table(uint8_t* host) {
  int32_t* t = reinterpret_cast<int32_t*>(host + off_scales_);
  size_t i = 0;
  for (const auto& k : layer_order_) {
    const ConvW& w = layers_[k];
    t[i++] = w.s_in; t[i++] = w.s_in2; t[i++] = w.s_res; t[i++] = w.s_out;
  }
  for (const char* nm : kNamedTensors) t[i++] = tscale(nm);
}
void Engine::read_scale_table(const uint8_t* host) {
  const int32_t* t = reinterpret_cast<const int32_t*>(host + off_scales_);
  size_t i = 0;
  for (const auto& k : layer_order_) {
    ConvW& w = layers_[k];
    w.s_in = t[i++]; w.s_in2 = t[i++]; w.s_res = t[i++]; w.s_out = t[i++];
  }
  for (const char* nm : kNamedTensors) tscale_[nm] = t[i++];
}

void Engine::upload_blob() {
  write_scale_table(host_blob_.data());
  SMK_CUDA(cudaMemcpy(blob_, host_blob_.data(), blob_bytes_, cudaMemcpyHostToDevice));
}

void Engine::adopt_weights() {
  std::vector<uint8_t> tbl(blob_bytes_ - off_scales_);
  SMK_CUDA(cudaMemcpy(tbl.data(), blob_ + off_scales_, tbl.size(), cudaMemcpyDeviceToHost));
  read_scale_table(tbl.data() - off_scales_);
  host_blob_.clear();
  weights_ready_ = true;
}

void Engine::load_weights(const sm_tensor_desc* t, int n) {
  std::map<std::string, const sm_tensor_desc*> sd;
  for (int i = 0; i < n; ++i) {
    SMK_CHECK(t[i].name != nullptr && t[i].data != nullptr, "null tensor descriptor");
    std::string name = t[i].name;
    if (name.rfind("module.", 0) == 0) name = name.substr(7);
    sd[name] = &t[i];
  }
  host_blob_.assign(blob_bytes_, 0);
  uint8_t* host = host_blob_.data();
  tscale_.clear();
  for (const auto& k : layer_order_) {
    ConvW& w = layers_[k];
    w.s_in = w.s_in2 = w.s_res = w.s_out = 0;
    fold_layer(w, sd, host);
  }
  for (const auto& k : layer_order_) quantize_layer(layers_[k], host);
  float* ones = reinterpret_cast<float*>(host + off_ones_);
  for (int i = 0; i < 4096; ++i) ones[i] = 1.f;
  quantize_stem(host);
  if (cfg_.with_mask) {
    const float* dw = find_tensor(sd, "refine_model.deconv.weight", (size_t)256 * 32 * 225);
    const float* db = find_tensor(sd, "refine_model.deconv.bias", 32);
    float* wd = reinterpret_cast<float*>(host + off_deconv_w_);
    for (int k = 0; k < 256; ++k)
      for (int co = 0; co < 32; ++co)
        for (int p = 0; p < 225; ++p) wd[(size_t)k * 7200 + p * 32 + co] = dw[((size_t)k * 32 + co) * 225 + p];
    std::memcpy(host + off_deconv_b_, db, 32 * sizeof(float));
  }
  upload_blob();
  weights_ready_ = true;
}


void Engine::calibrate(int B, const float* z, const float* x, cudaStream_t st) {
  SMK_CHECK(weights_ready_ && !host_blob_.empty(), "calibrate() needs weights loaded through sm_engine_load_weights on this engine");
  SMK_CHECK(cfg_.backend == SM_BACKEND_TENSOR, "calibrate() applies to the tensor-core backend");
  SMK_CHECK(B >= 1 && B <= cfg_.max_batch && z != nullptr && x != nullptr, "calibration batch");
  join_lanes(st);
  const size_t A = cfg_.anchor_num, RR = (size_t)R_ * R_;
  float *cls = nullptr, *loc = nullptr, *mask = nullptr, *ref = nullptr;
  int32_t* pos = nullptr;
  struct Tmp { std::vector<void*> p; ~Tmp() { for (void* q : p) cudaFree(q); } } tmp;
  auto dalloc = [&](size_t bytes) { void* q = nullptr; SMK_CUDA(cudaMalloc(&q, bytes)); tmp.p.push_back(q); return q; };
  cls = static_cast<float*>(dalloc(B * 2 * A * RR * sizeof(float)));
  loc = static_cast<float*>(dalloc(B * 4 * A * RR * sizeof(float)));
  if (cfg_.with_mask) {
    mask = static_cast<float*>(dalloc((size_t)B * 3969 * RR * sizeof(float)));
    ref = static_cast<float*>(dalloc((size_t)B * 127 * 127 * sizeof(float)));
    pos = static_cast<int32_t*>(dalloc((size_t)B * 2 * sizeof(int32_t)));
    std::vector<int32_t> hp((size_t)B * 2, R_ / 2);
    SMK_CUDA(cudaMemcpy(pos, hp.data(), hp.size() * sizeof(int32_t), cudaMemcpyHostToDevice));
  }
  if (absmax_dev_ == nullptr) SMK_CUDA(cudaMalloc(&absmax_dev_, kAbsmaxSlots * sizeof(float)));
  for (auto& kv : graphs_) if (kv.second.exec) cudaGraphExecDestroy(kv.second.exec);
  graphs_.clear();

  auto scale_of = [&](const std::string& name) -> int {
    auto it = layers_.find(name);
    return it != layers_.end() ? it->second.s_out : tscale(name);
  };
  auto set_scale = [&](const std::string& name, int v) {
    auto it = layers_.find(name);
    if (it != layers_.end()) it->second.s_out = it->second.f32_out ? 0 : v;
    else tscale_[name] = v;
  };
  auto rewire_and_upload = [&]() {
    {
      const ConvW& cat = layers_.at(kSearchCat);
      if (!cat.src_in.empty())
        for (const auto& k : cat.cat_keys) {
          ConvW& w = layers_.at(k);
          w.src_in = cat.src_in;
          w.s_out = cat.s_out;
        }
    }
    for (auto& kv : layers_) {
      ConvW& w = kv.second;
      if (!w.src_in.empty()) w.s_in = scale_of(w.src_in);
      if (!w.src_in2.empty()) w.s_in2 = scale_of(w.src_in2);
      if (!w.src_res.empty()) w.s_res = scale_of(w.src_res);
    }
    for (const auto& k : layer_order_) quantize_layer(layers_[k], host_blob_.data());
    quantize_stem(host_blob_.data());
    upload_blob();
  };

  bool settled = false;
  for (int iter = 0; iter < 12 && !settled; ++iter) {
    SMK_CUDA(cudaMemsetAsync(absmax_dev_, 0, kAbsmaxSlots * sizeof(float), st));
    SMK_CUDA(cudaMemsetAsync(ovf_flag_, 0, sizeof(int), st));
    struct Guard { Engine* e; ~Guard() { e->calibrating_ = false; e->tensor_name_.clear(); } } guard{this};
    calibrating_ = true;
    absmax_names_.clear();
    tensor_name_.clear();
    do_template(0, B, z, st);
    if (cfg_.with_mask) {
      do_track(0, B, x, cls, loc, mask, SM_TRACK_MASK_FEATURES | SM_TRACK_MASK_HEAD, st);
      do_refine(B, pos, ref, st);
    } else {
      do_track(0, B, x, cls, loc, nullptr, 0, st);
    }
    SMK_CUDA(cudaStreamSynchronize(st));
    calibrating_ = false;
    std::vector<float> mx(absmax_names_.size());
    SMK_CUDA(cudaMemcpy(mx.data(), absmax_dev_, mx.size() * sizeof(float), cudaMemcpyDeviceToHost));
    bool any_inf = false, any_zero = false;
    for (float v : mx) {
      if (!(v <= 65504.f)) any_inf = true;
      if (v == 0.f) any_zero = true;
    }
    if (any_inf || (any_zero && iter < 8)) {
      for (size_t i = 0; i < mx.size(); ++i) {
        const int step = !(mx[i] <= 65504.f) ? -10 : (mx[i] == 0.f && iter < 8) ? +10 : 0;
        if (step != 0) set_scale(absmax_names_[i], std::max(-60, std::min(60, scale_of(absmax_names_[i]) + step)));
      }
      rewire_and_upload();
      continue;
    }
    settled = true;
    for (size_t i = 0; i < mx.size(); ++i) {
      if (mx[i] == 0.f) continue;
      const int cur = scale_of(absmax_names_[i]);
      if (mx[i] >= 256.f && mx[i] <= 4096.f) continue;
      int want = cur + (int)std::lround(std::log2(1024.0 / (double)mx[i]));
      want = std::max(-60, std::min(60, want));
      const auto it = layers_.find(absmax_names_[i]);
      if (it != layers_.end() && it->second.f32_out) want = 0;
      if (want != cur) { set_scale(absmax_names_[i], want); settled = false; }
    }
    if (!settled) rewire_and_upload();
  }
  SMK_CHECK(settled, "calibrate(): activation scales did not settle (non-finite network outputs?)");
}

int Engine::status() {
  int v = 0;
  SMK_CUDA(cudaDeviceSynchronize());
  SMK_CUDA(cudaMemcpy(&v, ovf_flag_, sizeof(int), cudaMemcpyDeviceToHost));
  return v;
}


Act Engine::alloc_act(Arena& ar, int B, int H, int W, int C) {
  Act a;
  a.B = B; a.H = H; a.W = W; a.C = C;
  a.hi = static_cast<__half*>(ar.alloc(a.numel() * sizeof(__half)));
  a.lo = exact_ ? static_cast<__half*>(ar.alloc(a.numel() * sizeof(__half))) : nullptr;
  return a;
}

F32T Engine::alloc_f32(Arena& ar, int B, int H, int W, int C) {
  F32T t;
  t.B = B; t.H = H; t.W = W; t.C = C;
  t.p = static_cast<float*>(ar.alloc((size_t)B * H * W * C * sizeof(float)));
  return t;
}

void Engine::conv_into(const Act& in, const ConvW& Lw, Epilogue ep, cudaStream_t st, const Act* res,
                       const Act* in2) {
  ep.beta = Lw.beta;
  const double M = (double)in.B * Lw.g.out_size(in.H) * Lw.g.out_size(in.W);
  double K = (double)Lw.g.KH * Lw.g.KW * Lw.g.Cin;
  const bool tc = cfg_.backend == SM_BACKEND_TENSOR && Lw.gemm_ok;
  SMK_CHECK(in2 == nullptr || (tc && Lw.fused2), "fused second input needs the tensor-core path");
  if (in2 != nullptr) K += (double)Lw.g2.KH * Lw.g2.KW * Lw.g2.Cin;
  if (calibrating_) {
    ConvW& W = const_cast<ConvW&>(Lw);
    auto name_of = [&](const Act& a) {
      auto it = tensor_name_.find(a.hi);
      return it == tensor_name_.end() ? std::string() : it->second;
    };
    W.src_in = name_of(in);
    W.src_in2 = in2 ? name_of(*in2) : std::string();
    W.src_res = res ? name_of(*res) : std::string();
    W.f32_out = ep.out_mode != OUT_NHWC_SPLIT;
  }
  SMK_CHECK(in.sexp == Lw.s_in && (in2 == nullptr || in2->sexp == Lw.s_in2) && (res == nullptr || res->sexp == Lw.s_res),
            "activation scale mismatch at " + Lw.conv_key + " (weights were packed for other scales: re-run calibrate)");
  SMK_CHECK(ep.out_mode == OUT_NHWC_SPLIT || Lw.s_out == 0, "fp32 outputs are unscaled");
  if (ep.out_mode == OUT_NHWC_SPLIT) ep.ovf = ovf_flag_;
  const double flops = 2.0 * M * K * Lw.g.Cout;
  const double bytes = 4.0 * ((double)in.numel() + (in2 ? (double)in2->numel() : 0.0) + M * Lw.g.Cout * (res ? 2 : 1) +
                              K * Lw.g.Cout);
  if (!tc) {
    SMK_CHECK(Lw.s_in == 0 && Lw.s_out == 0, "the SIMT backend runs unscaled activations only");
    ep.alpha = ones_;
    if (res != nullptr) { ep.res_hi = res->hi; ep.res_lo = res->lo; }
    launch(st, 1, Lw.conv_key, "conv_simt", flops, bytes, [&] { launch_ref_conv(in, Lw.g, Lw.w_ref, ep, st); });
    return;
  }
  ep.alpha = Lw.alpha;
  const Act* big = &in;
  if (in2 != nullptr && in2->numel() > big->numel()) big = in2;
  if (res != nullptr && res->numel() > big->numel()) big = res;
  const bool use_patch = in2 == nullptr && res == nullptr && ep.out_mode == OUT_NHWC_SPLIT &&
                         patch_conv_supported(in, Lw.g);
  const bool reverse = !use_patch && end_of(*big) > 0;
  GemmInput gi[2] = {{in, Lw.g, 0}, {in, Lw.g, 0}};
  int nconv = 1;
  const Act* ident = nullptr;
  if (in2 != nullptr) {
    gi[1] = {*in2, Lw.g2, Lw.col2};
    nconv = 2;
    ep.beta = Lw.beta2;
  } else if (res != nullptr) {
    if (Lw.has_diag) ident = res;
    else { ep.res_hi = res->hi; ep.res_lo = res->lo; }
  }
  launch(st, 1, Lw.conv_key, "conv_gemm", flops, bytes, [&] {
    const int now_end = reverse ? -1 : +1;
    last_end_[in.hi] = now_end;
    if (in2 != nullptr) last_end_[in2->hi] = now_end;
    if (res != nullptr) last_end_[res->hi] = now_end;
    if (ep.out_mode == OUT_NHWC_SPLIT) last_end_[ep.out_hi] = now_end;
    if (use_patch)
      launch_conv3x3_patch(in, Lw.g, Lw.w_hi, Lw.w_lo, Lw.w_ld, ep, exact_ ? 2 : 1, num_sms_, st);
    else
      launch_gemm_multi(gi, nconv, ident, Lw.col_diag, Lw.w_hi, Lw.w_lo, Lw.cout_pad, Lw.w_ld, ep, exact_ ? 2 : 1,
                        num_sms_, st, reverse);
  });
}

void Engine::note_tensor(const Act& a, const std::string& name, cudaStream_t st, const Act* same_scale_as) {
  if (measuring_) return;
  if (taps_ != nullptr) (*taps_)[name] = a;
  if (!calibrating_) return;
  if (same_scale_as != nullptr) {
    tensor_name_[a.hi] = tensor_name_[same_scale_as->hi];
    return;
  }
  tensor_name_[a.hi] = name;
  size_t slot = 0;
  for (; slot < absmax_names_.size(); ++slot)
    if (absmax_names_[slot] == name) break;
  if (slot == absmax_names_.size()) {
    SMK_CHECK((int)slot < kAbsmaxSlots, "too many calibrated tensors");
    absmax_names_.push_back(name);
  }
  launch_absmax(a, absmax_dev_ + slot, st);
}

void Engine::note_tensor(const F32T& t, const std::string& name) {
  if (!measuring_ && taps_f32_ != nullptr) (*taps_f32_)[name] = t;
}

Act Engine::conv(const Act& in, const ConvW& Lw, bool relu, const Act* res, Arena& ar, cudaStream_t st,
                 const Act* in2) {
  Act out = alloc_act(ar, in.B, Lw.g.out_size(in.H), Lw.g.out_size(in.W), Lw.g.Cout);
  Epilogue ep;
  ep.relu = relu ? 1 : 0;
  ep.out_mode = OUT_NHWC_SPLIT;
  ep.out_hi = out.hi;
  ep.out_lo = out.lo;
  out.sexp = Lw.s_out;
  conv_into(in, Lw, ep, st, res, in2);
  note_tensor(out, Lw.conv_key, st);
  return out;
}

F32T Engine::conv_f32(const Act& in, const ConvW& Lw, bool relu, Arena& ar, cudaStream_t st) {
  F32T out = alloc_f32(ar, in.B, Lw.g.out_size(in.H), Lw.g.out_size(in.W), Lw.g.Cout);
  Epilogue ep;
  ep.relu = relu ? 1 : 0;
  ep.out_mode = OUT_NHWC_F32;
  ep.out_f32 = out.p;
  conv_into(in, Lw, ep, st);
  note_tensor(out, Lw.conv_key);
  return out;
}

Act Engine::backbone(const float* x, int B, int S, Arena& ar, std::map<std::string, Act>* keep, cudaStream_t st) {
  const std::string F = "features.features.";
  const int So = (S - 7) / 2 + 1;
  Act p0 = alloc_act(ar, B, So, So, 64);
  const ConvW& stem = L(F + "conv1");
  launch(st, 1, "stem", "stem", 2.0 * B * So * So * 64 * 147, 4.0 * B * (3.0 * S * S + 64.0 * So * So), [&] {
    if (cfg_.backend == SM_BACKEND_TENSOR)
      launch_stem_tc(x, B, S, stem_whi_, stem_wlo_, stem_alpha_, stem.beta, p0, num_sms_, st, ovf_flag_);
    else launch_stem(x, B, S, stem.w_ref, ones_, stem.beta, p0, st);
  });
  p0.sexp = stem.s_out;
  note_tensor(p0, "stem", st);
  const int Sp = (So + 2 - 3) / 2 + 1;
  Act y = alloc_act(ar, B, Sp, Sp, 64);
  y.sexp = p0.sexp;
  launch(st, 1, "maxpool", "pool", 0, 4.0 * (p0.numel() + y.numel()), [&] { launch_maxpool3s2(p0, y, st); });
  note_tensor(y, "maxpool", st, &p0);
  last_end_[p0.hi] = +1;
  last_end_[y.hi] = +1;
  if (keep) (*keep)["p0"] = p0;
  const char* names[3] = {"layer1", "layer2", "layer3"};
  const int blocks[3] = {3, 4, 6};
  for (int l = 0; l < 3; ++l) {
    for (int i = 0; i < blocks[l]; ++i) {
      const std::string P = F + names[l] + "." + std::to_string(i) + ".";
      Act t1 = conv(y, L(P + "conv1"), true, nullptr, ar, st);
      Act t2 = conv(t1, L(P + "conv2"), true, nullptr, ar, st);
      const ConvW& c3 = L(P + "conv3");
      if (i == 0 && cfg_.backend == SM_BACKEND_TENSOR && c3.fused2) {
        y = conv(t2, c3, true, nullptr, ar, st, &y);
      } else {
        Act res = y;
        if (i == 0) res = conv(y, L(P + "downsample.0"), false, nullptr, ar, st);
        y = conv(t2, c3, true, &res, ar, st);
      }
    }
    if (keep) (*keep)[std::string("p") + std::to_string(l + 1)] = y;
  }
  Act xf = conv(y, L("features.downsample.downsample.0"), false, nullptr, ar, st);
  if (xf.W < 20) {
    Act c = alloc_act(ar, B, xf.H - 8, xf.W - 8, xf.C);
    c.sexp = xf.sexp;
    launch(st, 1, "crop_center", "misc", 0, 4.0 * (xf.numel() + c.numel()), [&] { launch_crop_center(xf, 4, c, st); });
    note_tensor(c, "crop_center", st, &xf);
    xf = c;
  }
  return xf;
}

static const char* kBranch[3] = {"rpn_model.cls.", "rpn_model.loc.", "mask_model.mask."};
static const char* kCorrName[3] = {"corr_cls", "corr_loc", "corr_mask"};

void Engine::do_template(int slot0, int B, const float* z, cudaStream_t st, const int32_t* slots) {
  SMK_CHECK(weights_ready_, "weights not loaded");
  SMK_CHECK(B >= 1 && B <= cfg_.max_batch && (slots != nullptr || (slot0 >= 0 && slot0 + B <= cfg_.num_slots)),
            "template batch/slot range");
  join_lanes(st);
  const size_t kslot = 25 * 256;
  if (slots != nullptr && kscatter_ == nullptr) {
    const size_t n = (size_t)n_branches_ * cfg_.max_batch * kslot;
    SMK_CUDA(cudaMalloc(&kscatter_, 2 * n * sizeof(__half)));
    total_bytes_ += 2 * n * sizeof(__half);
  }
  templ_arena_.reset();
  templ_named_.clear();
  taps_ = &templ_named_;
  taps_f32_ = nullptr;
  Act zf = backbone(z, B, 127, templ_arena_, nullptr, st);
  SMK_CHECK(zf.H == 7 && zf.W == 7, "template feature must be 7x7");
  templ_named_["zf"] = zf;
  for (int br = 0; br < n_branches_; ++br) {
    const ConvW& ck = L(std::string(kBranch[br]) + "conv_kernel.0");
    Epilogue ep;
    ep.relu = 1;
    ep.out_mode = OUT_NHWC_SPLIT;
    if (slots == nullptr) {
      const size_t off = ((size_t)br * cfg_.num_slots + slot0) * kslot;
      ep.out_hi = kcache_hi_ + off;
      ep.out_lo = exact_ ? kcache_lo_ + off : nullptr;
    } else {
      const size_t n = (size_t)n_branches_ * cfg_.max_batch * kslot;
      ep.out_hi = kscatter_ + (size_t)br * cfg_.max_batch * kslot;
      ep.out_lo = exact_ ? ep.out_hi + n : nullptr;
    }
    conv_into(zf, ck, ep, st);
    if (slots != nullptr) {
      const size_t cache_off = (size_t)br * cfg_.num_slots * kslot;
      launch(st, 1, "scatter_slots", "misc", 0, 2.0 * 2 * B * kslot * (exact_ ? 2 : 1), [&] {
        launch_scatter_slots(ep.out_hi, ep.out_lo, kcache_hi_ + cache_off, exact_ ? kcache_lo_ + cache_off : nullptr,
                             slots, B, cfg_.num_slots, (int)kslot, ovf_flag_, st);
      });
    }
    Act kc;
    kc.hi = ep.out_hi; kc.lo = ep.out_lo; kc.B = B; kc.H = 5; kc.W = 5; kc.C = 256; kc.sexp = ck.s_out;
    note_tensor(kc, ck.conv_key, st);
  }
  taps_ = nullptr;
}

template <typename F>
void Engine::run_lanes(cudaStream_t st, int set, F&& body) {
  const CallState& s = state_;
  if (set != kJoined) {
    lanes_dirty_ = true;
    for (int l = s.split_n - 1; l >= 0; --l) {
      Lane& ln = lanes_[l];
      order_after(st, ln.own);
      SMK_CUDA(cudaStreamWaitEvent(ln.own, h2d_done_[set], 0));
      body(ln, s.split_off[l], s.split_off[l + 1] - s.split_off[l], ln.own);
      SMK_CUDA(cudaEventRecord(lane_done_[set][l], ln.own));
      SMK_CUDA(cudaStreamWaitEvent(d2h_stream_, lane_done_[set][l], 0));
    }
    return;
  }
  const int nl = s.split_n;
  const bool fork = nl > 1 && concurrent();
  auto join = [&] {
    if (fork) for (int l = 1; l < nl; ++l) order_after(lanes_[l].own, st);
  };
  if (fork) for (int l = 1; l < nl; ++l) order_after(st, lanes_[l].own);
  try {
    for (int l = nl - 1; l >= 0; --l)
      body(lanes_[l], s.split_off[l], s.split_off[l + 1] - s.split_off[l], fork && l > 0 ? lanes_[l].own : st);
  } catch (...) {
    try { join(); } catch (...) {}
    throw;
  }
  join();
}

void Engine::do_track(int slot0, int B, const float* x, float* cls, float* loc, float* mask, int flags,
                      cudaStream_t st) {
  SMK_CHECK(weights_ready_, "weights not loaded");
  SMK_CHECK(B >= 1 && B <= cfg_.max_batch && slot0 >= 0 && slot0 + B <= cfg_.num_slots, "track batch/slot range");
  SMK_CHECK(cls != nullptr && loc != nullptr, "cls/loc outputs required");
  const bool want_feats = (flags & SM_TRACK_MASK_FEATURES) != 0;
  const bool want_mask_head = (flags & SM_TRACK_MASK_HEAD) != 0;
  SMK_CHECK(!(want_feats || want_mask_head) || cfg_.with_mask, "engine was built without the mask branch");
  SMK_CHECK(!want_mask_head || mask != nullptr, "mask output buffer required");
  join_lanes(st);
  const std::vector<uint64_t> key = {1, (uint64_t)slot0, (uint64_t)B, (uint64_t)x, (uint64_t)cls, (uint64_t)loc,
                                     (uint64_t)mask, (uint64_t)flags, (uint64_t)st};
  const size_t S = cfg_.search_size, A = cfg_.anchor_num, RR = (size_t)R_ * R_;
  run_with_graph(key, st, [&] {
    split_batch(B);
    run_lanes(st, kJoined, [&](Lane& ln, int b0, int nbat, cudaStream_t ls) {
      track_lane(ln, slot0 + b0, nbat, x + b0 * 3 * S * S, cls + b0 * 2 * A * RR, loc + b0 * 4 * A * RR,
                 mask != nullptr ? mask + (size_t)b0 * 63 * 63 * RR : nullptr, flags, ls);
    });
    state_.last_B = B;
    state_.have_mask_feats = want_feats || want_mask_head;
  });
}

void Engine::track_lane(Lane& ln, int slot0, int B, const float* x, float* cls, float* loc, float* mask, int flags,
                        cudaStream_t st, const int32_t* slots) {
  const bool want_feats = (flags & SM_TRACK_MASK_FEATURES) != 0;
  const bool want_mask_head = (flags & SM_TRACK_MASK_HEAD) != 0;
  Arena& search_arena = ln.search;
  search_arena.reset();
  std::map<std::string, Act>& named = state_.named[ln.id];
  named.clear();
  state_.named_f32[ln.id].clear();
  taps_ = &named;
  taps_f32_ = nullptr;
  Act xf = backbone(x, B, cfg_.search_size, search_arena, &named, st);
  named["search"] = xf;
  const int nb = (want_feats || want_mask_head) ? 3 : 2;
  float* outs[3] = {cls, loc, mask};
  const bool use_cat = nb == n_branches_ && cfg_.backend == SM_BACKEND_TENSOR;
  Act cs_all;
  if (use_cat) cs_all = conv(xf, L(kSearchCat), true, nullptr, search_arena, st);
  for (int br = 0; br < nb; ++br) {
    cudaStream_t bs = (concurrent() && br > 0) ? ln.aux[br - 1] : st;
    order_after(st, bs);
    const std::string P = kBranch[br];
    Act cs = use_cat ? cs_all : conv(xf, L(P + "conv_search.0"), true, nullptr, search_arena, bs);
    Act corr = alloc_act(search_arena, B, cs.H - 4, cs.W - 4, 256);
    const size_t off = ((size_t)br * cfg_.num_slots + (slots != nullptr ? 0 : slot0)) * 25 * 256;
    corr.sexp = tscale(kCorrName[br]);
    const int s_kc = L(P + "conv_kernel.0").s_out;
    launch(bs, 1, kCorrName[br], "xcorr", 2.0 * 25 * corr.numel(),
           4.0 * (2.0 * corr.numel() + (double)B * cs.H * cs.W * 256 + (double)B * 25 * 256), [&] {
      launch_xcorr_nhwc(cs, use_cat ? 256 * br : 0, kcache_hi_ + off, exact_ ? kcache_lo_ + off : nullptr, 5, 5, corr,
                        std::ldexp(1.f, corr.sexp - cs.sexp - s_kc), ovf_flag_, bs, slots, cfg_.num_slots);
      last_end_[corr.hi] = +1;
    });
    note_tensor(corr, kCorrName[br], bs);
    named[kCorrName[br]] = corr;
    if (!(br == 2 && !want_mask_head)) {
      Act h = conv(corr, L(P + "head.0"), true, nullptr, search_arena, bs);
      Epilogue ep;
      ep.relu = 0;
      ep.out_mode = OUT_NCHW_F32;
      ep.out_f32 = outs[br];
      conv_into(h, L(P + "head.3"), ep, bs);
    }
  }
  for (int br = 1; br < nb; ++br) order_after((concurrent()) ? ln.aux[br - 1] : st, st);
  taps_ = nullptr;
}

F32T Engine::small(const F32T& a, const F32T* b, int Ho, const ConvW& Lw, bool relu, float* out_override, Arena& ar,
                   cudaStream_t st) {
  F32T out;
  out.B = a.B; out.H = Ho; out.W = Ho; out.C = Lw.g.Cout;
  out.p = out_override != nullptr ? out_override
                                  : static_cast<float*>(ar.alloc((size_t)a.B * Ho * Ho * Lw.g.Cout * sizeof(float)));
  SMK_CHECK(a.C == Lw.g.Cin && (b == nullptr || (b->C == a.C && b->H == a.H)), "small conv operand shapes");
  launch(st, 1, Lw.conv_key, "refine_small", 2.0 * a.B * Ho * Ho * 9.0 * a.C * Lw.g.Cout,
         4.0 * a.B * ((double)a.H * a.W * a.C * (b ? 2 : 1) + (double)Ho * Ho * Lw.g.Cout), [&] {
    const int* map = updown_map(Ho, a.H);
    launch_small_conv3x3_maps(a.p, b ? b->p : nullptr, a.B, a.H, a.W, Ho, Ho, a.C, Lw.g.Cout, map, map, Lw.w_ref,
                              Lw.beta, relu ? 1 : 0, out.p, st);
  });
  if (out_override == nullptr) note_tensor(out, Lw.conv_key);
  return out;
}

void Engine::do_refine(int B, const int32_t* pos, float* out, cudaStream_t st) {
  SMK_CHECK(state_.have_mask_feats && B == state_.last_B,
            "sm_refine must follow sm_track(..., SM_TRACK_MASK_FEATURES) with the same B");
  SMK_CHECK(cfg_.with_mask, "engine was built without the mask branch");
  join_lanes(st);
  const std::vector<uint64_t> key = {2, (uint64_t)B, (uint64_t)pos, (uint64_t)out, (uint64_t)st,
                                     (uint64_t)state_.named[0]["p0"].hi};
  run_with_graph(key, st, [&] {
    run_lanes(st, kJoined, [&](Lane& ln, int b0, int nbat, cudaStream_t ls) {
      refine_lane(ln, nbat, pos + 2 * b0, out + (size_t)b0 * 127 * 127, ls);
    });
  });
}

void Engine::refine_lane(Lane& ln, int B, const int32_t* pos, float* out, cudaStream_t st) {
  Arena& ar = ln.refine;
  ar.reset();
  const std::string R = "refine_model.";
  std::map<std::string, Act>& named = state_.named[ln.id];
  const Act& p0 = named["p0"];
  const Act& p1 = named["p1"];
  const Act& p2 = named["p2"];
  const Act& corr = named["corr_mask"];
  taps_ = &named;
  taps_f32_ = &state_.named_f32[ln.id];
  cudaStream_t s2 = concurrent() ? ln.aux[0] : st, s1 = concurrent() ? ln.aux[1] : st,
               s0 = concurrent() ? ln.aux[2] : st;
  order_after(st, s2);
  order_after(st, s1);
  order_after(st, s0);
  Act c2 = alloc_act(ar, B, 15, 15, 512);
  c2.sexp = p2.sexp;
  launch(s2, 1, "crop_p2", "refine_misc", 0, 8.0 * c2.numel(), [&] {
    last_end_[c2.hi] = +1;
    launch_refine_crop(p2, pos, R_ - 1, 1, 4, 15, c2, s2);
  });
  note_tensor(c2, "refine:crop_p2", s2, &p2);
  Act v2a = conv(c2, L(R + "v2.0"), true, nullptr, ar, s2);
  F32T v2b = conv_f32(v2a, L(R + "v2.2"), true, ar, s2);
  Act c1 = alloc_act(ar, B, 31, 31, 256);
  c1.sexp = p1.sexp;
  launch(s1, 1, "crop_p1", "refine_misc", 0, 8.0 * c1.numel(), [&] {
    last_end_[c1.hi] = +1;
    launch_refine_crop(p1, pos, R_ - 1, 2, 8, 31, c1, s1);
  });
  note_tensor(c1, "refine:crop_p1", s1, &p1);
  Act v1a = conv(c1, L(R + "v1.0"), true, nullptr, ar, s1);
  F32T v1b = conv_f32(v1a, L(R + "v1.2"), true, ar, s1);
  Act c0 = alloc_act(ar, B, 61, 61, 64);
  c0.sexp = p0.sexp;
  launch(s0, 1, "crop_p0", "refine_misc", 0, 8.0 * c0.numel(), [&] {
    last_end_[c0.hi] = +1;
    launch_refine_crop(p0, pos, R_ - 1, 4, 16, 61, c0, s0);
  });
  note_tensor(c0, "refine:crop_p0", s0, &p0);
  F32T v0a = conv_f32(c0, L(R + "v0.0"), true, ar, s0);
  F32T v0b = small(v0a, nullptr, 61, L(R + "v0.2"), true, nullptr, ar, s0);
  float* p3 = static_cast<float*>(ar.alloc((size_t)B * 256 * sizeof(float)));
  F32T d = alloc_f32(ar, B, 15, 15, 32);
  launch(st, 2, "deconv", "refine_misc", 2.0 * B * 256 * 7200, 4.0 * (256.0 * 7200 + B * 7200.0), [&] {
    launch_gather_corr(corr, pos, p3, std::ldexp(1.f, -corr.sexp), st);
    launch_deconv(p3, deconv_w_, deconv_b_, d.p, B, 256, 7200, 32, st);
  });
  note_tensor(F32T{p3, B, 1, 1, 256}, "refine:p3");
  note_tensor(d, "refine:deconv");
  F32T h2a = small(d, nullptr, 15, L(R + "h2.0"), true, nullptr, ar, st);
  F32T h2b = small(h2a, nullptr, 15, L(R + "h2.2"), true, nullptr, ar, st);
  order_after(s2, st);
  F32T o0 = small(h2b, &v2b, 31, L(R + "post0"), false, nullptr, ar, st);
  F32T h1a = small(o0, nullptr, 31, L(R + "h1.0"), true, nullptr, ar, st);
  F32T h1b = small(h1a, nullptr, 31, L(R + "h1.2"), true, nullptr, ar, st);
  order_after(s1, st);
  F32T o1 = small(h1b, &v1b, 61, L(R + "post1"), false, nullptr, ar, st);
  F32T h0a = small(o1, nullptr, 61, L(R + "h0.0"), true, nullptr, ar, st);
  F32T h0b = small(h0a, nullptr, 61, L(R + "h0.2"), true, nullptr, ar, st);
  order_after(s0, st);
  small(h0b, &v0b, 127, L(R + "post2"), false, out, ar, st);
  taps_ = nullptr;
  taps_f32_ = nullptr;
}

int Engine::next_set() {
  const int t = (int)(host_calls_++ & 1);
  if (set_busy_[t]) host_wait(t);
  return t;
}

template <typename Coupled, typename F>
int Engine::host_call(int t, int B, bool mask_feats, cudaStream_t st, std::initializer_list<Copy> h2d,
                      std::initializer_list<Copy> d2h, Coupled&& coupled, F&& body) {
  for (const Copy& c : h2d)
    if (c.src != nullptr) SMK_CUDA(cudaMemcpyAsync(c.dst, c.src, c.bytes, cudaMemcpyHostToDevice, h2d_stream_));
  SMK_CUDA(cudaEventRecord(h2d_done_[t], h2d_stream_));
  if (lanes_for(n_lanes_, B) >= 2 && !use_graphs_ && concurrent()) {
    split_batch(B);
    run_lanes(st, t, body);
    state_.last_B = B;
    state_.have_mask_feats = mask_feats;
  } else {
    SMK_CUDA(cudaStreamWaitEvent(st, h2d_done_[t], 0));
    coupled();
    SMK_CUDA(cudaEventRecord(lane_done_[t][0], st));
    SMK_CUDA(cudaStreamWaitEvent(d2h_stream_, lane_done_[t][0], 0));
  }
  for (const Copy& c : d2h)
    if (c.dst != nullptr) SMK_CUDA(cudaMemcpyAsync(c.dst, c.src, c.bytes, cudaMemcpyDeviceToHost, d2h_stream_));
  SMK_CUDA(cudaEventRecord(d2h_done_[t], d2h_stream_));
  set_busy_[t] = true;
  return t;
}

int Engine::track_host_async(int slot0, int B, const float* xh, float* clsh, float* loch, const int32_t* posh,
                             float* maskh, cudaStream_t st) {
  const size_t S = cfg_.search_size, A = cfg_.anchor_num, RR = (size_t)R_ * R_;
  SMK_CHECK(B >= 1 && B <= cfg_.max_batch, "batch");
  SMK_CHECK(weights_ready_, "weights not loaded");
  SMK_CHECK(slot0 >= 0 && slot0 + B <= cfg_.num_slots, "track batch/slot range");
  const bool refine = posh != nullptr && maskh != nullptr;
  SMK_CHECK(!refine || cfg_.with_mask, "engine was built without the mask branch");
  const int flags = refine ? SM_TRACK_MASK_FEATURES : 0;
  const int t = next_set();
  return host_call(
      t, B, refine, st,
      {{stage_x_[t], xh, (size_t)B * 3 * S * S * sizeof(float)},
       {stage_pos_[t], refine ? posh : nullptr, (size_t)B * 2 * sizeof(int32_t)}},
      {{clsh, stage_cls_[t], (size_t)B * 2 * A * RR * sizeof(float)},
       {loch, stage_loc_[t], (size_t)B * 4 * A * RR * sizeof(float)},
       {refine ? maskh : nullptr, stage_mask_[t], (size_t)B * 127 * 127 * sizeof(float)}},
      [&] {
        do_track(slot0, B, stage_x_[t], stage_cls_[t], stage_loc_[t], nullptr, flags, st);
        if (refine) do_refine(B, stage_pos_[t], stage_mask_[t], st);
      },
      [&](Lane& ln, int b0, int nbat, cudaStream_t ls) {
        track_lane(ln, slot0 + b0, nbat, stage_x_[t] + b0 * 3 * S * S, stage_cls_[t] + b0 * 2 * A * RR,
                   stage_loc_[t] + b0 * 4 * A * RR, nullptr, flags, ls);
        if (refine) refine_lane(ln, nbat, stage_pos_[t] + 2 * b0, stage_mask_[t] + (size_t)b0 * 127 * 127, ls);
      });
}

void Engine::host_wait(int ticket) {
  SMK_CHECK(ticket == 0 || ticket == 1, "bad ticket");
  if (!set_busy_[ticket]) return;
  SMK_CUDA(cudaEventSynchronize(d2h_done_[ticket]));
  set_busy_[ticket] = false;
}

void Engine::track_host(int slot0, int B, const float* xh, float* clsh, float* loch, const int32_t* posh, float* maskh,
                        cudaStream_t st) {
  host_wait(track_host_async(slot0, B, xh, clsh, loch, posh, maskh, st));
}


namespace {
Engine::StepIO slice_io(const Engine::StepIO& io, int b0, size_t S, size_t A, size_t RR) {
  Engine::StepIO o = io;
  o.x = io.x + (size_t)b0 * 3 * S * S;
  o.tsz = io.tsz + 2 * (size_t)b0;
  if (io.hp) o.hp = io.hp + 3 * (size_t)b0;
  o.cls = io.cls + (size_t)b0 * 2 * A * RR;
  o.loc = io.loc + (size_t)b0 * 4 * A * RR;
  if (io.mask) o.mask = io.mask + (size_t)b0 * 3969 * RR;
  o.best = io.best + b0;
  o.pos = io.pos + 2 * (size_t)b0;
  o.rec = io.rec + 8 * (size_t)b0;
  if (io.refine) o.refine = io.refine + (size_t)b0 * 127 * 127;
  if (io.mask_col) o.mask_col = io.mask_col + (size_t)b0 * 3969;
  return o;
}
}

void Engine::step_lane(Lane& ln, int slot0, int B, const StepIO& io, cudaStream_t st, const int32_t* slots) {
  track_lane(ln, slot0, B, io.x, io.cls, io.loc, io.mask, io.flags, st, slots);
  launch(st, 1, "select", "select", 0, 4.0 * B * 6.0 * cfg_.anchor_num * R_ * R_, [&] {
    launch_select(io.cls, io.loc, io.anchors, io.window, io.tsz, B, cfg_.anchor_num, R_, io.penalty_k,
                  io.window_influence, io.best, io.pos, io.rec, st, io.hp);
  });
  if (io.refine != nullptr) refine_lane(ln, B, io.pos, io.refine, st);
  if (io.mask_col != nullptr)
    launch(st, 1, "mask_col", "misc", 0, 8.0 * B * 3969, [&] {
      launch_gather_mask_col(io.mask, io.pos, B, 3969, R_, io.mask_col, st);
    });
}

void Engine::do_step(int slot0, int B, const StepIO& io, cudaStream_t st, const int32_t* slots) {
  SMK_CHECK(weights_ready_, "weights not loaded");
  SMK_CHECK(B >= 1 && B <= cfg_.max_batch && (slots != nullptr || (slot0 >= 0 && slot0 + B <= cfg_.num_slots)),
            "step batch/slot range");
  SMK_CHECK(io.x && io.tsz && io.anchors && io.window && io.cls && io.loc && io.best && io.pos && io.rec, "null argument");
  const bool want_feats = (io.flags & SM_TRACK_MASK_FEATURES) != 0, want_head = (io.flags & SM_TRACK_MASK_HEAD) != 0;
  SMK_CHECK(!(want_feats || want_head || io.refine) || cfg_.with_mask, "engine was built without the mask branch");
  SMK_CHECK(io.refine == nullptr || want_feats, "refine output needs SM_TRACK_MASK_FEATURES");
  SMK_CHECK(!want_head || io.mask != nullptr, "mask output buffer required");
  SMK_CHECK(io.mask_col == nullptr || want_head, "mask column needs SM_TRACK_MASK_HEAD");
  join_lanes(st);
  uint64_t pk_bits, wi_bits;
  std::memcpy(&pk_bits, &io.penalty_k, sizeof(pk_bits));
  std::memcpy(&wi_bits, &io.window_influence, sizeof(wi_bits));
  const std::vector<uint64_t> key = {3, (uint64_t)slot0, (uint64_t)B, (uint64_t)io.x, (uint64_t)io.tsz, (uint64_t)io.cls,
                                     (uint64_t)io.loc, (uint64_t)io.mask, (uint64_t)io.flags, (uint64_t)io.pos,
                                     (uint64_t)io.rec, (uint64_t)io.refine, (uint64_t)io.mask_col, (uint64_t)st,
                                     (uint64_t)io.anchors, (uint64_t)io.window, (uint64_t)slots, pk_bits, wi_bits,
                                     (uint64_t)io.hp};
  const size_t S = cfg_.search_size, A = cfg_.anchor_num, RR = (size_t)R_ * R_;
  run_with_graph(key, st, [&] {
    split_batch(B);
    run_lanes(st, kJoined, [&](Lane& ln, int b0, int nbat, cudaStream_t ls) {
      step_lane(ln, slot0 + b0, nbat, slice_io(io, b0, S, A, RR), ls, slots != nullptr ? slots + b0 : nullptr);
    });
    state_.last_B = B;
    state_.have_mask_feats = want_feats || want_head;
  });
}

int Engine::step_host_async(int slot0, int B, const sm_step_io& h, cudaStream_t st) {
  const size_t S = cfg_.search_size, A = cfg_.anchor_num, RR = (size_t)R_ * R_;
  SMK_CHECK(B >= 1 && B <= cfg_.max_batch, "batch");
  SMK_CHECK(weights_ready_, "weights not loaded");
  SMK_CHECK(slot0 >= 0 && slot0 + B <= cfg_.num_slots, "step batch/slot range");
  SMK_CHECK(h.x_host && h.tsz_host && h.anchors_dev && h.window_dev && h.records_host, "null argument");
  const bool want_feats = (h.flags & SM_TRACK_MASK_FEATURES) != 0, want_head = (h.flags & SM_TRACK_MASK_HEAD) != 0;
  SMK_CHECK(!(want_feats || want_head || h.refine_host) || cfg_.with_mask, "engine was built without the mask branch");
  SMK_CHECK(h.refine_host == nullptr || want_feats, "refine output needs SM_TRACK_MASK_FEATURES");
  SMK_CHECK(h.mask_col_host == nullptr || want_head, "mask column needs SM_TRACK_MASK_HEAD");
  if (want_head && mask_raw_ == nullptr)
    SMK_CUDA(cudaMalloc(&mask_raw_, (size_t)cfg_.max_batch * 3969 * RR * sizeof(float)));
  const int t = next_set();
  StepIO io;
  io.x = stage_x_[t]; io.tsz = stage_tsz_[t]; io.anchors = h.anchors_dev; io.window = h.window_dev;
  io.penalty_k = h.penalty_k; io.window_influence = h.window_influence; io.flags = h.flags;
  io.cls = stage_cls_[t]; io.loc = stage_loc_[t]; io.mask = want_head ? mask_raw_ : nullptr;
  io.best = stage_best_[t]; io.pos = stage_pos_[t]; io.rec = stage_rec_[t];
  io.refine = h.refine_host != nullptr ? stage_mask_[t] : nullptr;
  io.mask_col = h.mask_col_host != nullptr ? stage_maskcol_[t] : nullptr;
  return host_call(
      t, B, want_feats || want_head, st,
      {{stage_x_[t], h.x_host, (size_t)B * 3 * S * S * sizeof(float)},
       {stage_tsz_[t], h.tsz_host, (size_t)B * 2 * sizeof(double)}},
      {{h.records_host, stage_rec_[t], (size_t)B * 8 * sizeof(float)},
       {h.refine_host, stage_mask_[t], (size_t)B * 127 * 127 * sizeof(float)},
       {h.mask_col_host, stage_maskcol_[t], (size_t)B * 3969 * sizeof(float)},
       {h.cls_host, stage_cls_[t], (size_t)B * 2 * A * RR * sizeof(float)},
       {h.loc_host, stage_loc_[t], (size_t)B * 4 * A * RR * sizeof(float)}},
      [&] { do_step(slot0, B, io, st); },
      [&](Lane& ln, int b0, int nbat, cudaStream_t ls) {
        step_lane(ln, slot0 + b0, nbat, slice_io(io, b0, S, A, RR), ls);
      });
}

void Engine::do_export(const char* what, float* out, int64_t* shape4, cudaStream_t st) {
  join_lanes(st);
  const std::string name = what;
  const std::string missing = "no cached tensor named '" + name + "'";
  auto put_act = [&](const Act& a, float* dst) {
    if (dst != nullptr)
      launch(st, 1, "export", "misc", 0, 8.0 * a.numel(), [&] { launch_split_to_f32(a, dst, st, std::ldexp(1.f, -a.sexp)); });
  };
  if (name == "zf" || name.rfind("template:", 0) == 0) {
    auto it = templ_named_.find(name == "zf" ? name : name.substr(9));
    SMK_CHECK(it != templ_named_.end(), missing);
    const Act& a = it->second;
    if (shape4 != nullptr) { shape4[0] = a.B; shape4[1] = a.C; shape4[2] = a.H; shape4[3] = a.W; }
    put_act(a, out);
    return;
  }
  int total_B = 0;
  for (int l = 0; l < state_.split_n; ++l) {
    const std::map<std::string, Act>& named = state_.named[l];
    const std::map<std::string, F32T>& named_f32 = state_.named_f32[l];
    auto it = named.find(name);
    auto jt = named_f32.find(name);
    SMK_CHECK(it != named.end() || jt != named_f32.end(), missing);
    int B, C, H, W;
    if (it != named.end()) {
      const Act& a = it->second;
      B = a.B; C = a.C; H = a.H; W = a.W;
      put_act(a, out != nullptr ? out + (size_t)total_B * C * H * W : nullptr);
    } else {
      const F32T& t = jt->second;
      B = t.B; C = t.C; H = t.H; W = t.W;
      if (out != nullptr) {
        const size_t n = (size_t)B * H * W * C, hw = (size_t)H * W;
        std::vector<float> nhwc(n), nchw(n);
        SMK_CUDA(cudaMemcpyAsync(nhwc.data(), t.p, n * sizeof(float), cudaMemcpyDeviceToHost, st));
        SMK_CUDA(cudaStreamSynchronize(st));
        for (size_t b = 0; b < (size_t)B; ++b)
          for (size_t p = 0; p < hw; ++p)
            for (size_t c = 0; c < (size_t)C; ++c) nchw[(b * C + c) * hw + p] = nhwc[(b * hw + p) * C + c];
        SMK_CUDA(cudaMemcpyAsync(out + (size_t)total_B * C * hw, nchw.data(), n * sizeof(float), cudaMemcpyHostToDevice,
                                 st));
        SMK_CUDA(cudaStreamSynchronize(st));
      }
    }
    if (shape4 != nullptr) { shape4[1] = C; shape4[2] = H; shape4[3] = W; }
    total_B += B;
  }
  if (shape4 != nullptr) shape4[0] = total_B;
}

std::string Engine::profile_dump() {
  SMK_CUDA(cudaDeviceSynchronize());
  std::string out;
  for (auto& r : prof_) {
    float ms = 0.f;
    cudaEventElapsedTime(&ms, r.e0, r.e1);
    char line[512];
    snprintf(line, sizeof line, "%s\t%s\t%.6f\t%.0f\t%.0f\n", r.name.c_str(), r.cat.c_str(), ms, r.flops, r.bytes);
    out += line;
    event_pool_.push_back(r.e0);
    event_pool_.push_back(r.e1);
  }
  prof_.clear();
  return out;
}


static void conv2d_op(const float* x, const float* w, const float* scale, const float* shift, float* out, int B,
                      int Cin, int H, int W, int Cout, int KH, int KW, int stride, int pad, int dil, int relu,
                      int backend, int precision, cudaStream_t st) {
  ConvGeom g{Cin, Cout, KH, KW, stride, pad, dil};
  const bool exact = precision == SM_PRECISION_EXACT;
  const bool use_gemm = backend == SM_BACKEND_TENSOR;
  SMK_CHECK(!use_gemm || gemm_conv_supported(g), "tensor-core conv needs Cin % 64 == 0");
  const size_t K = (size_t)KH * KW * Cin;
  const int cout_pad = use_gemm ? gemm_cout_pad(Cout) : Cout;
  std::vector<float> hw(K * Cout), hs(Cout, 1.f), hb(Cout, 0.f);
  SMK_CUDA(cudaStreamSynchronize(st));
  SMK_CUDA(cudaMemcpy(hw.data(), w, hw.size() * sizeof(float), cudaMemcpyDeviceToHost));
  if (scale) SMK_CUDA(cudaMemcpy(hs.data(), scale, Cout * sizeof(float), cudaMemcpyDeviceToHost));
  if (shift) SMK_CUDA(cudaMemcpy(hb.data(), shift, Cout * sizeof(float), cudaMemcpyDeviceToHost));
  std::vector<float> wref(K * Cout), alpha(cout_pad, 0.f), beta(cout_pad, 0.f);
  std::vector<__half> whi((size_t)cout_pad * K, __float2half_rn(0.f)), wlo((size_t)cout_pad * K, __float2half_rn(0.f));
  const int HW = KH * KW;
  for (int n = 0; n < Cout; ++n) {
    float amax = 0.f;
    for (int c = 0; c < Cin; ++c)
      for (int t = 0; t < HW; ++t) {
        const float fw = (float)((double)hw[((size_t)n * Cin + c) * HW + t] * (double)hs[n]);
        wref[((size_t)t * Cin + c) * Cout + n] = fw;
        amax = std::max(amax, std::fabs(fw));
      }
    beta[n] = hb[n];
    alpha[n] = 1.f;
    if (use_gemm) {
      const int e = weight_exp(amax);
      alpha[n] = std::ldexp(1.f, -e);
      for (int c = 0; c < Cin; ++c)
        for (int t = 0; t < HW; ++t) {
          const float fw = std::ldexp(wref[((size_t)t * Cin + c) * Cout + n], e);
          const __half h = __float2half_rn(fw);
          whi[((size_t)n * HW + t) * Cin + c] = h;
          wlo[((size_t)n * HW + t) * Cin + c] = __float2half_rn(fw - __half2float(h));
        }
    }
  }
  const int Ho = g.out_size(H), Wo = g.out_size(W);
  Act in;
  in.B = B; in.H = H; in.W = W; in.C = Cin;
  __half *d_whi = nullptr, *d_wlo = nullptr;
  float *d_wref = nullptr, *d_alpha = nullptr, *d_beta = nullptr;
  SMK_CUDA(cudaMalloc(&in.hi, in.numel() * sizeof(__half)));
  if (exact) SMK_CUDA(cudaMalloc(&in.lo, in.numel() * sizeof(__half)));
  SMK_CUDA(cudaMalloc(&d_whi, whi.size() * sizeof(__half)));
  SMK_CUDA(cudaMalloc(&d_wlo, wlo.size() * sizeof(__half)));
  SMK_CUDA(cudaMalloc(&d_wref, wref.size() * sizeof(float)));
  SMK_CUDA(cudaMalloc(&d_alpha, alpha.size() * sizeof(float)));
  SMK_CUDA(cudaMalloc(&d_beta, beta.size() * sizeof(float)));
  SMK_CUDA(cudaMemcpy(d_whi, whi.data(), whi.size() * sizeof(__half), cudaMemcpyHostToDevice));
  SMK_CUDA(cudaMemcpy(d_wlo, wlo.data(), wlo.size() * sizeof(__half), cudaMemcpyHostToDevice));
  SMK_CUDA(cudaMemcpy(d_wref, wref.data(), wref.size() * sizeof(float), cudaMemcpyHostToDevice));
  SMK_CUDA(cudaMemcpy(d_alpha, alpha.data(), alpha.size() * sizeof(float), cudaMemcpyHostToDevice));
  SMK_CUDA(cudaMemcpy(d_beta, beta.data(), beta.size() * sizeof(float), cudaMemcpyHostToDevice));
  launch_import_nchw(x, in, st);
  Epilogue ep;
  ep.alpha = d_alpha;
  ep.beta = d_beta;
  ep.relu = relu;
  ep.out_mode = OUT_NCHW_F32;
  ep.out_f32 = out;
  int dev = 0, sms = 132;
  SMK_CUDA(cudaGetDevice(&dev));
  SMK_CUDA(cudaDeviceGetAttribute(&sms, cudaDevAttrMultiProcessorCount, dev));
  (void)Ho; (void)Wo;
  if (use_gemm && patch_conv_supported(in, g)) {
    Act o;
    o.B = B; o.H = Ho; o.W = Wo; o.C = Cout;
    SMK_CUDA(cudaMalloc(&o.hi, o.numel() * sizeof(__half)));
    if (exact) SMK_CUDA(cudaMalloc(&o.lo, o.numel() * sizeof(__half)));
    Epilogue e2 = ep;
    e2.out_mode = OUT_NHWC_SPLIT;
    e2.out_hi = o.hi;
    e2.out_lo = o.lo;
    e2.out_f32 = nullptr;
    launch_conv3x3_patch(in, g, d_whi, d_wlo, (int)K, e2, exact ? 2 : 1, sms, st);
    launch_split_to_f32(o, out, st);
    SMK_CUDA(cudaStreamSynchronize(st));
    cudaFree(o.hi); cudaFree(o.lo);
  } else if (use_gemm) launch_gemm_conv(in, g, d_whi, d_wlo, cout_pad, ep, exact ? 2 : 1, sms, st);
  else launch_ref_conv(in, g, d_wref, ep, st);
  SMK_CUDA(cudaStreamSynchronize(st));
  cudaFree(in.hi); cudaFree(in.lo); cudaFree(d_whi); cudaFree(d_wlo); cudaFree(d_wref); cudaFree(d_alpha); cudaFree(d_beta);
}

}


struct sm_engine {
  std::unique_ptr<smk::Engine> impl;
};

#define SM_API_BEGIN try {
#define SM_API_END                                  \
  return 0;                                         \
  }                                                 \
  catch (const std::exception& ex) {                \
    smk::g_last_error = ex.what();                  \
    return -1;                                      \
  }                                                 \
  catch (...) {                                     \
    smk::g_last_error = "unknown error";            \
    return -1;                                      \
  }

static void require_device() {
  int ndev = 0;
  SMK_CHECK(cudaGetDeviceCount(&ndev) == cudaSuccess && ndev > 0, "no CUDA device: siammask_b200 has no CPU fallback");
}

extern "C" {

const char* sm_last_error(void) { return smk::g_last_error.c_str(); }
const char* sm_version(void) { return "siammask_b200 0.1 (sm_90a)"; }

int sm_engine_create(const sm_config* cfg, sm_engine** out) {
  SM_API_BEGIN
  SMK_CHECK(cfg != nullptr && out != nullptr, "null argument");
  require_device();
  auto* e = new sm_engine;
  try {
    e->impl.reset(new smk::Engine(*cfg));
  } catch (...) {
    delete e;
    throw;
  }
  *out = e;
  SM_API_END
}

void sm_engine_destroy(sm_engine* e) { delete e; }

int sm_engine_load_weights(sm_engine* e, const sm_tensor_desc* tensors, int32_t n) {
  SM_API_BEGIN
  SMK_CHECK(e && tensors && n > 0, "null argument");
  e->impl->load_weights(tensors, n);
  SM_API_END
}

int sm_engine_weight_blob(sm_engine* e, void** dev_ptr, size_t* bytes) {
  SM_API_BEGIN
  SMK_CHECK(e && dev_ptr && bytes, "null argument");
  e->impl->weight_blob(dev_ptr, bytes);
  SM_API_END
}

int sm_engine_adopt_weights(sm_engine* e) {
  SM_API_BEGIN
  SMK_CHECK(e, "null argument");
  e->impl->adopt_weights();
  SM_API_END
}

int sm_engine_calibrate(sm_engine* e, int32_t B, const float* z_nchw, const float* x_nchw, void* stream) {
  SM_API_BEGIN
  SMK_CHECK(e && z_nchw && x_nchw, "null argument");
  e->impl->calibrate(B, z_nchw, x_nchw, static_cast<cudaStream_t>(stream));
  SM_API_END
}

int sm_engine_status(sm_engine* e, int32_t* flags) {
  SM_API_BEGIN
  SMK_CHECK(e && flags, "null argument");
  *flags = e->impl->status();
  SM_API_END
}

int sm_template(sm_engine* e, int32_t slot0, int32_t B, const float* z, void* stream) {
  SM_API_BEGIN
  SMK_CHECK(e && z, "null argument");
  e->impl->do_template(slot0, B, z, static_cast<cudaStream_t>(stream));
  SM_API_END
}

int sm_track(sm_engine* e, int32_t slot0, int32_t B, const float* x, float* cls, float* loc, float* mask, int32_t flags,
             void* stream) {
  SM_API_BEGIN
  SMK_CHECK(e && x, "null argument");
  e->impl->do_track(slot0, B, x, cls, loc, mask, flags, static_cast<cudaStream_t>(stream));
  SM_API_END
}

int sm_refine(sm_engine* e, int32_t B, const int32_t* pos, float* out, void* stream) {
  SM_API_BEGIN
  SMK_CHECK(e && pos && out, "null argument");
  e->impl->do_refine(B, pos, out, static_cast<cudaStream_t>(stream));
  SM_API_END
}

int sm_track_host(sm_engine* e, int32_t slot0, int32_t B, const float* x_host, float* cls_host, float* loc_host,
                  const int32_t* pos_host, float* mask_out_host, void* stream) {
  SM_API_BEGIN
  SMK_CHECK(e && x_host && cls_host && loc_host, "null argument");
  e->impl->track_host(slot0, B, x_host, cls_host, loc_host, pos_host, mask_out_host, static_cast<cudaStream_t>(stream));
  SM_API_END
}

int sm_track_host_async(sm_engine* e, int32_t slot0, int32_t B, const float* x_host, float* cls_host, float* loc_host,
                        const int32_t* pos_host, float* mask_out_host, void* stream, int32_t* ticket) {
  SM_API_BEGIN
  SMK_CHECK(e && x_host && cls_host && loc_host && ticket, "null argument");
  *ticket = e->impl->track_host_async(slot0, B, x_host, cls_host, loc_host, pos_host, mask_out_host,
                                      static_cast<cudaStream_t>(stream));
  SM_API_END
}

int sm_track_host_wait(sm_engine* e, int32_t ticket) {
  SM_API_BEGIN
  SMK_CHECK(e, "null argument");
  e->impl->host_wait(ticket);
  SM_API_END
}

int sm_step(sm_engine* e, int32_t slot0, int32_t B, const float* x, const double* target_sz_in_crop, const float* anchors,
            const float* window, double penalty_k, double window_influence, int32_t flags, float* cls, float* loc,
            float* mask, int32_t* best_idx, int32_t* pos, float* records, float* refine_out, float* mask_col,
            void* stream) {
  SM_API_BEGIN
  SMK_CHECK(e, "null argument");
  smk::Engine::StepIO io;
  io.x = x; io.tsz = target_sz_in_crop; io.anchors = anchors; io.window = window;
  io.penalty_k = penalty_k; io.window_influence = window_influence; io.flags = flags;
  io.cls = cls; io.loc = loc; io.mask = mask; io.best = best_idx; io.pos = pos; io.rec = records;
  io.refine = refine_out; io.mask_col = mask_col;
  e->impl->do_step(slot0, B, io, static_cast<cudaStream_t>(stream));
  SM_API_END
}

int sm_template_slots(sm_engine* e, int32_t B, const int32_t* slots, const float* z, void* stream) {
  SM_API_BEGIN
  SMK_CHECK(e && slots && z, "null argument");
  e->impl->do_template(0, B, z, static_cast<cudaStream_t>(stream), slots);
  SM_API_END
}

int sm_step_slots(sm_engine* e, int32_t B, const int32_t* slots, const float* x, const double* target_sz_in_crop,
                  const float* anchors, const float* window, double penalty_k, double window_influence, int32_t flags,
                  float* cls, float* loc, float* mask, int32_t* best_idx, int32_t* pos, float* records, float* refine_out,
                  float* mask_col, void* stream) {
  SM_API_BEGIN
  SMK_CHECK(e && slots, "null argument");
  smk::Engine::StepIO io;
  io.x = x; io.tsz = target_sz_in_crop; io.anchors = anchors; io.window = window;
  io.penalty_k = penalty_k; io.window_influence = window_influence; io.flags = flags;
  io.cls = cls; io.loc = loc; io.mask = mask; io.best = best_idx; io.pos = pos; io.rec = records;
  io.refine = refine_out; io.mask_col = mask_col;
  e->impl->do_step(0, B, io, static_cast<cudaStream_t>(stream), slots);
  SM_API_END
}

int sm_step_slots_hp(sm_engine* e, int32_t B, const int32_t* slots, const double* hp, const float* x,
                     const double* target_sz_in_crop, const float* anchors, const float* window, int32_t flags, float* cls,
                     float* loc, float* mask, int32_t* best_idx, int32_t* pos, float* records, float* refine_out,
                     float* mask_col, void* stream) {
  SM_API_BEGIN
  SMK_CHECK(e && slots && hp, "null argument");
  smk::Engine::StepIO io;
  io.x = x; io.tsz = target_sz_in_crop; io.anchors = anchors; io.window = window; io.hp = hp; io.flags = flags;
  io.cls = cls; io.loc = loc; io.mask = mask; io.best = best_idx; io.pos = pos; io.rec = records;
  io.refine = refine_out; io.mask_col = mask_col;
  e->impl->do_step(0, B, io, static_cast<cudaStream_t>(stream), slots);
  SM_API_END
}

int sm_step_host_async(sm_engine* e, int32_t slot0, int32_t B, const sm_step_io* io, void* stream, int32_t* ticket) {
  SM_API_BEGIN
  SMK_CHECK(e && io && ticket, "null argument");
  *ticket = e->impl->step_host_async(slot0, B, *io, static_cast<cudaStream_t>(stream));
  SM_API_END
}

int sm_xcorr_depthwise(const float* x, const float* k, float* out, int32_t B, int32_t C, int32_t H, int32_t W, int32_t kh,
                       int32_t kw, void* stream) {
  SM_API_BEGIN
  SMK_CHECK(x && k && out, "null argument");
  require_device();
  smk::launch_xcorr_nchw_f32(x, k, out, B * C, H, W, kh, kw, static_cast<cudaStream_t>(stream));
  SM_API_END
}

int sm_conv2d(const float* x, const float* w, const float* scale, const float* shift, float* out, int32_t B, int32_t Cin,
              int32_t H, int32_t W, int32_t Cout, int32_t KH, int32_t KW, int32_t stride, int32_t pad, int32_t dil,
              int32_t relu, int32_t backend, int32_t precision, void* stream) {
  SM_API_BEGIN
  SMK_CHECK(x && w && out, "null argument");
  require_device();
  smk::conv2d_op(x, w, scale, shift, out, B, Cin, H, W, Cout, KH, KW, stride, pad, dil, relu, backend, precision,
                 static_cast<cudaStream_t>(stream));
  SM_API_END
}

int sm_crop_resize(const uint8_t* frames, size_t frame_stride, int32_t H, int32_t W, const int32_t* boxes, int32_t B,
                   int32_t model_size, float* out, void* stream) {
  SM_API_BEGIN
  SMK_CHECK(frames && boxes && out && B >= 1 && H > 0 && W > 0 && model_size > 0, "bad argument");
  require_device();
  smk::launch_crop_resize(frames, frame_stride, H, W, boxes, B, model_size, out, static_cast<cudaStream_t>(stream));
  SM_API_END
}

int sm_crop_resize_indexed(const uint8_t* frames, size_t frame_stride, int32_t H, int32_t W, const int32_t* frame_idx,
                           const int32_t* boxes, int32_t B, int32_t model_size, float* out, void* stream) {
  SM_API_BEGIN
  SMK_CHECK(frames && frame_idx && boxes && out && B >= 1 && H > 0 && W > 0 && model_size > 0, "bad argument");
  require_device();
  smk::launch_crop_resize(frames, frame_stride, H, W, boxes, B, model_size, out, static_cast<cudaStream_t>(stream),
                          frame_idx);
  SM_API_END
}

int sm_crop_resize_ragged(const uint8_t* frames, const sm_image_desc* frame_desc, const int32_t* frame_idx,
                          const int32_t* boxes, int32_t B, int32_t model_size, float* out, void* stream) {
  SM_API_BEGIN
  SMK_CHECK(B >= 0 && model_size > 0, "bad argument");
  if (B == 0) return 0;
  SMK_CHECK(frames && frame_desc && frame_idx && boxes && out, "null argument");
  require_device();
  smk::launch_crop_resize(frames, 0, 0, 0, boxes, B, model_size, out, static_cast<cudaStream_t>(stream), frame_idx,
                          frame_desc);
  SM_API_END
}

int sm_paste_labels_ragged(const float* masks, int32_t side, const double* maps, const uint8_t* anno,
                           const int32_t* obj_offsets, const int32_t* objects, const sm_image_desc* video_desc, int32_t G,
                           int32_t max_h, int32_t max_w, double seg_thr, uint8_t* labels, void* stream) {
  SM_API_BEGIN
  SMK_CHECK(G >= 0 && max_h >= 1 && max_w >= 1 && side > 0, "bad argument");
  SMK_CHECK(seg_thr >= -1.0, "seg_thr must be >= -1 (objects that miss a pixel are skipped as value -1)");
  if (G == 0) return 0;
  SMK_CHECK(obj_offsets && objects && video_desc && labels, "null argument");
  require_device();
  smk::launch_paste_labels(masks, side, maps, anno, obj_offsets, objects, G, max_h, max_w, seg_thr, labels,
                           static_cast<cudaStream_t>(stream), video_desc);
  SM_API_END
}

int sm_paste_labels_iou_ragged(const float* masks, int32_t side, const double* maps, const uint8_t* anno,
                               const int32_t* obj_offsets, const int32_t* objects, const int32_t* target_ids,
                               const sm_image_desc* video_desc, int32_t G, int32_t max_h, int32_t max_w, double seg_thr,
                               uint8_t* labels, const double* thrs, int32_t T, int32_t* counts, void* stream) {
  SM_API_BEGIN
  SMK_CHECK(G >= 0 && max_h >= 1 && max_w >= 1 && side > 0, "bad argument");
  SMK_CHECK(seg_thr >= -1.0, "seg_thr must be >= -1 (objects that miss a pixel are skipped as value -1)");
  SMK_CHECK((int64_t)max_h * max_w <= INT32_MAX, "frame too large for int32 counts");
  SMK_CHECK(T >= 1 && T <= 32, "1 <= T <= 32 thresholds");
  if (G == 0) return 0;
  SMK_CHECK(anno && obj_offsets && objects && target_ids && video_desc && labels && thrs && counts, "null argument");
  require_device();
  smk::launch_paste_labels_iou(masks, side, maps, anno, obj_offsets, objects, target_ids, G, max_h, max_w, seg_thr,
                               labels, thrs, T, counts, static_cast<cudaStream_t>(stream), video_desc);
  SM_API_END
}

int sm_label_boxes_ragged(const uint8_t* anno, const sm_image_desc* video_desc, int32_t G, const int32_t* queries,
                          int32_t Q, int32_t* boxes, void* stream) {
  SM_API_BEGIN
  SMK_CHECK(G >= 0 && Q >= 0, "bad argument");
  if (Q == 0) return 0;
  SMK_CHECK(anno && video_desc && queries && boxes, "null argument");
  require_device();
  smk::launch_label_boxes(anno, G, 0, 0, queries, Q, boxes, static_cast<cudaStream_t>(stream), video_desc);
  SM_API_END
}

int sm_vot_overlap_sized(const float* poly_a, const float* poly_b, int32_t B, const int32_t* wh, float* overlap,
                         void* stream) {
  SM_API_BEGIN
  SMK_CHECK(B >= 0, "bad argument");
  if (B == 0) return 0;
  SMK_CHECK(poly_a && poly_b && wh && overlap, "null argument");
  require_device();
  smk::launch_vot_overlap(poly_a, poly_b, B, 0, 0, overlap, static_cast<cudaStream_t>(stream), wh);
  SM_API_END
}

int sm_warp_affine_ragged(const float* src, int32_t side, const double* maps, float* dst, const sm_image_desc* dst_desc,
                          int32_t B, int32_t max_h, int32_t max_w, float border_value, void* stream) {
  SM_API_BEGIN
  SMK_CHECK(B >= 0 && side > 0 && max_h >= 1 && max_w >= 1, "bad argument");
  if (B == 0) return 0;
  SMK_CHECK(src && maps && dst && dst_desc, "null argument");
  require_device();
  smk::launch_warp_affine(src, side, side, maps, dst, max_h, max_w, border_value, B, static_cast<cudaStream_t>(stream),
                          dst_desc);
  SM_API_END
}

int sm_paste_labels(const float* masks, int32_t side, const double* maps, const uint8_t* anno, const int32_t* obj_offsets,
                    const int32_t* objects, int32_t G, int32_t H, int32_t W, double seg_thr, uint8_t* labels,
                    void* stream) {
  SM_API_BEGIN
  SMK_CHECK(obj_offsets && objects && labels && G >= 1 && H > 0 && W > 0 && side > 0, "bad argument");
  SMK_CHECK(seg_thr >= -1.0, "seg_thr must be >= -1 (objects that miss a pixel are skipped as value -1)");
  require_device();
  smk::launch_paste_labels(masks, side, maps, anno, obj_offsets, objects, G, H, W, seg_thr, labels,
                           static_cast<cudaStream_t>(stream));
  SM_API_END
}

int sm_paste_labels_iou(const float* masks, int32_t side, const double* maps, const uint8_t* anno,
                        const int32_t* obj_offsets, const int32_t* objects, const int32_t* target_ids, int32_t G,
                        int32_t H, int32_t W, double seg_thr, uint8_t* labels, const double* thrs, int32_t T,
                        int32_t* counts, void* stream) {
  SM_API_BEGIN
  SMK_CHECK(anno && obj_offsets && objects && target_ids && labels && thrs && counts && G >= 1 && H > 0 && W > 0 &&
            side > 0, "bad argument");
  SMK_CHECK(seg_thr >= -1.0, "seg_thr must be >= -1 (objects that miss a pixel are skipped as value -1)");
  SMK_CHECK((int64_t)H * W <= INT32_MAX, "frame too large for int32 counts");
  SMK_CHECK(T >= 1 && T <= 32, "1 <= T <= 32 thresholds");
  require_device();
  smk::launch_paste_labels_iou(masks, side, maps, anno, obj_offsets, objects, target_ids, G, H, W, seg_thr, labels, thrs,
                               T, counts, static_cast<cudaStream_t>(stream));
  SM_API_END
}

int sm_mask_iou(const float* masks, int32_t side, const double* maps, const uint8_t* anno, const int32_t* video,
                int32_t B, int32_t H, int32_t W, const double* thrs, int32_t T, int32_t* counts, void* stream) {
  SM_API_BEGIN
  SMK_CHECK(masks && maps && anno && video && thrs && counts && B >= 1 && H > 0 && W > 0 && side > 0, "bad argument");
  SMK_CHECK((int64_t)H * W <= INT32_MAX, "frame too large for int32 counts");
  SMK_CHECK(T >= 1 && T <= 32, "1 <= T <= 32 thresholds");
  require_device();
  smk::launch_mask_iou(masks, side, maps, anno, video, B, H, W, thrs, T, counts, static_cast<cudaStream_t>(stream));
  SM_API_END
}

int sm_label_boxes(const uint8_t* anno, int32_t G, int32_t H, int32_t W, const int32_t* queries, int32_t Q, int32_t* boxes,
                   void* stream) {
  SM_API_BEGIN
  SMK_CHECK(anno && queries && boxes && G >= 1 && H > 0 && W > 0 && Q >= 1, "bad argument");
  require_device();
  smk::launch_label_boxes(anno, G, H, W, queries, Q, boxes, static_cast<cudaStream_t>(stream));
  SM_API_END
}

int sm_vot_overlap(const float* poly_a, const float* poly_b, int32_t B, int32_t W, int32_t H, float* overlap, void* stream) {
  SM_API_BEGIN
  SMK_CHECK(poly_a && poly_b && overlap && B >= 1 && W > 0 && H > 0, "bad argument");
  SMK_CHECK(((int64_t)W + 1) * ((int64_t)H + 1) <= INT32_MAX, "frame too large for int32 pixel counts");
  require_device();
  smk::launch_vot_overlap(poly_a, poly_b, B, W, H, overlap, static_cast<cudaStream_t>(stream));
  SM_API_END
}

int sm_warp_affine(const float* src, int32_t src_h, int32_t src_w, const double* maps, float* dst, int32_t dst_h,
                   int32_t dst_w, float border_value, int32_t B, void* stream) {
  SM_API_BEGIN
  SMK_CHECK(src && maps && dst && B >= 1 && src_h > 0 && src_w > 0 && dst_h > 0 && dst_w > 0, "bad argument");
  require_device();
  smk::launch_warp_affine(src, src_h, src_w, maps, dst, dst_h, dst_w, border_value, B, static_cast<cudaStream_t>(stream));
  SM_API_END
}

static smk::TrackerHp to_hp(const sm_tracker_hp* h) {
  smk::TrackerHp t;
  t.context_amount = h->context_amount; t.penalty_k = h->penalty_k; t.window_influence = h->window_influence; t.lr = h->lr;
  t.exemplar_size = h->exemplar_size; t.instance_size = h->instance_size; t.total_stride = h->total_stride;
  t.base_size = h->base_size; t.out_size = h->out_size; t.reserved = 0;
  return t;
}

int sm_tracker_prepare(int32_t B, const double* state, const int32_t* avg_chans, const sm_tracker_hp* hp, int32_t* boxes,
                       double* target_sz_in_crop, double* aux, void* stream) {
  SM_API_BEGIN
  SMK_CHECK(state && avg_chans && hp && boxes && target_sz_in_crop && aux && B >= 1, "bad argument");
  require_device();
  smk::launch_tracker_prepare(B, state, avg_chans, to_hp(hp), boxes, target_sz_in_crop, aux, static_cast<cudaStream_t>(stream));
  SM_API_END
}

int sm_tracker_update(int32_t B, double* state, const float* records, const double* aux, const int32_t* im_wh,
                      const sm_tracker_hp* hp, int32_t anchor_num, int32_t score_size, double* maps, double* out,
                      void* stream) {
  SM_API_BEGIN
  SMK_CHECK(state && records && aux && im_wh && hp && B >= 1 && score_size >= 1, "bad argument");
  require_device();
  smk::launch_tracker_update(B, state, records, aux, im_wh, to_hp(hp), anchor_num, score_size, maps, out,
                             static_cast<cudaStream_t>(stream));
  SM_API_END
}

int sm_tracker_update_hp(int32_t B, double* state, const float* records, const double* aux, const int32_t* im_wh,
                         const sm_tracker_hp* hp, const double* hp_table, int32_t anchor_num, int32_t score_size,
                         double* maps, double* out, void* stream) {
  SM_API_BEGIN
  SMK_CHECK(state && records && aux && im_wh && hp && hp_table && B >= 1 && score_size >= 1, "bad argument");
  require_device();
  smk::launch_tracker_update(B, state, records, aux, im_wh, to_hp(hp), anchor_num, score_size, maps, out,
                             static_cast<cudaStream_t>(stream), hp_table);
  SM_API_END
}

int sm_select(sm_engine* e, int32_t B, const float* cls, const float* loc, const float* anchors, const float* window,
              const double* target_sz_in_crop, double penalty_k, double window_influence, int32_t* best_idx, int32_t* pos,
              float* records, void* stream) {
  SM_API_BEGIN
  SMK_CHECK(e && cls && loc && anchors && window && target_sz_in_crop && best_idx && pos && records, "null argument");
  SMK_CHECK(B >= 1, "batch");
  const smk::Engine& eng = *e->impl;
  smk::launch_select(cls, loc, anchors, window, target_sz_in_crop, B, eng.cfg().anchor_num, eng.score_size(), penalty_k,
                     window_influence,
                     best_idx, pos, records, static_cast<cudaStream_t>(stream));
  SM_API_END
}

int sm_export(sm_engine* e, const char* what, float* out, int64_t* shape4, void* stream) {
  SM_API_BEGIN
  SMK_CHECK(e && what, "null argument");
  e->impl->do_export(what, out, shape4, static_cast<cudaStream_t>(stream));
  SM_API_END
}

int sm_engine_set_graphs(sm_engine* e, int32_t on) {
  SM_API_BEGIN
  SMK_CHECK(e, "null argument");
  e->impl->set_graphs(on != 0);
  SM_API_END
}

int sm_profile_enable(sm_engine* e, int32_t on) {
  SM_API_BEGIN
  SMK_CHECK(e, "null argument");
  e->impl->set_profiling(on != 0);
  SM_API_END
}

int64_t sm_profile_dump(sm_engine* e, char* buf, size_t cap) {
  try {
    if (!e) return -1;
    static thread_local std::string pending;
    if (pending.empty()) pending = e->impl->profile_dump();
    if (buf == nullptr || cap <= pending.size()) return (int64_t)pending.size() + 1;
    std::memcpy(buf, pending.c_str(), pending.size() + 1);
    const int64_t n = (int64_t)pending.size();
    pending.clear();
    return n;
  } catch (const std::exception& ex) {
    smk::g_last_error = ex.what();
    return -1;
  }
}

int64_t sm_launch_count(const sm_engine* e) { return e ? e->impl->launches() : 0; }
size_t sm_engine_bytes(const sm_engine* e) { return e ? e->impl->bytes() : 0; }

}
```

### siammask_b200/custom.py

```python
from __future__ import annotations

import ctypes as C
from collections import OrderedDict

import numpy as np
import torch

from . import _lib
from .checkpoint import expected_keys, normalize_keys

DEFAULT_ANCHORS = {"stride": 8, "ratios": [0.33, 0.5, 1, 2, 3], "scales": [8], "round_dight": 0}


class Custom:
    def __init__(self, pretrain: bool = False, anchors: dict | None = None, *, search_size: int = 255,
                 max_batch: int = 1, num_slots: int | None = None, precision: str = "exact",
                 backend: str = "tensor", mask: bool = True, graphs: bool = False, **_unused):
        self.anchors = anchors if anchors is not None else dict(DEFAULT_ANCHORS)
        self.anchor_num = len(self.anchors["ratios"]) * len(self.anchors["scales"])
        self.search_size = int(search_size)
        self.max_batch = int(max_batch)
        self.num_slots = int(num_slots) if num_slots is not None else self.max_batch
        self.precision = {"exact": _lib.SM_PRECISION_EXACT, "fast": _lib.SM_PRECISION_FAST}[precision]
        self.backend = {"tensor": _lib.SM_BACKEND_TENSOR, "simt": _lib.SM_BACKEND_SIMT}[backend]
        self.with_mask = bool(mask)
        self.graphs = bool(graphs)
        self._io: dict = {}
        self.score_size = (self.search_size - 127) // 8 + 1 + 8
        self.training = False
        self._sd: dict[str, torch.Tensor] | None = None
        self._engine = C.c_void_p(None)
        self._device: torch.device | None = None
        self._lib = _lib.load()

    def state_dict(self):
        if self._sd is not None:
            return OrderedDict(self._sd)
        return OrderedDict((k, torch.empty(s, device="meta")) for k, s in
                           expected_keys(self.with_mask, self.with_mask).items())

    def load_state_dict(self, state_dict, strict: bool = False):
        sd = normalize_keys(state_dict)
        want = expected_keys(self.with_mask, self.with_mask)
        missing = [k for k in want if k not in sd]
        if len(missing) == len(want):
            raise AssertionError("load NONE from pretrained checkpoint")
        if missing:
            if strict:
                raise KeyError(f"checkpoint lacks {len(missing)} tensors needed on the hot path, e.g. {missing[:3]}")
            import warnings
            from .checkpoint import synthetic_state_dict
            warnings.warn(f"checkpoint lacks {len(missing)} hot-path tensors (e.g. {missing[:3]}): they keep their "
                          "initial values, as with the reference's strict=False load", RuntimeWarning)
            init = synthetic_state_dict(0, self.with_mask, self.with_mask)
            sd = dict(sd)
            for k in missing:
                sd[k] = init[k]
        for k, shp in want.items():
            if tuple(sd[k].shape) != tuple(shp):
                raise ValueError(f"{k}: shape {tuple(sd[k].shape)} != expected {tuple(shp)}")
        self._sd = {k: sd[k].detach().to("cpu", torch.float32).contiguous() for k in want}
        if self._engine.value:
            self._upload()
        return self

    def eval(self):
        self.training = False
        return self

    def train(self, mode: bool = True):
        if mode:
            raise NotImplementedError("siammask_b200 implements the inference path only")
        return self

    def cuda(self, device=None):
        return self.to(torch.device("cuda", torch.cuda.current_device() if device is None else device))

    def to(self, device):
        device = torch.device(device)
        if device.type != "cuda":
            raise RuntimeError("siammask_b200 runs on CUDA (sm_90a) devices only; there is no CPU path")
        if device.index is None:
            device = torch.device("cuda", torch.cuda.current_device())
        if self._engine.value and self._device == device:
            return self
        self._destroy()
        self._device = device
        with torch.cuda.device(device):
            cfg = _lib.SmConfig(self.search_size, self.max_batch, self.num_slots, self.precision, self.backend,
                                self.anchor_num, int(self.with_mask))
            _lib.check(self._lib.sm_engine_create(C.byref(cfg), C.byref(self._engine)))
            _lib.check(self._lib.sm_engine_set_graphs(self._engine, int(self.graphs)))
            self._io = {}
            self._gstream = torch.cuda.Stream(device) if self.graphs else None
            if self._sd is not None:
                self._upload()
        return self

    def _upload(self):
        descs = (_lib.SmTensorDesc * len(self._sd))()
        keep = []
        for i, (k, t) in enumerate(self._sd.items()):
            name = k.encode()
            keep.append(name)
            descs[i].name = name
            descs[i].data = t.data_ptr()
            descs[i].ndim = t.dim()
            for j, s in enumerate(t.shape):
                descs[i].shape[j] = s
        with torch.cuda.device(self._device):
            _lib.check(self._lib.sm_engine_load_weights(self._engine, descs, len(self._sd)))

    def weight_blob(self) -> torch.Tensor:
        ptr, n = C.c_void_p(), C.c_size_t()
        _lib.check(self._lib.sm_engine_weight_blob(self._engine, C.byref(ptr), C.byref(n)))

        class _Arena:
            __cuda_array_interface__ = {"shape": (n.value,), "typestr": "|u1", "data": (ptr.value, False),
                                        "version": 2}
        t = torch.as_tensor(_Arena(), device=self._device)
        t._sm_owner = self
        return t

    def adopt_weights(self):
        _lib.check(self._lib.sm_engine_adopt_weights(self._engine))

    @torch.no_grad()
    def calibrate(self, z, x):
        z, x = self._prep(z, 127), self._prep(x, self.search_size)
        if z.shape[0] != x.shape[0]:
            raise ValueError("paired sample batch expected")
        with torch.cuda.device(self._device):
            self._fence_in()
            _lib.check(self._lib.sm_engine_calibrate(self._engine, z.shape[0], z.data_ptr(), x.data_ptr(), self._stream()))
            self._fence_out()
        return self

    def status(self) -> int:
        v = C.c_int32()
        _lib.check(self._lib.sm_engine_status(self._engine, C.byref(v)))
        return int(v.value)

    _PACK_MAGIC = b"SMB200PK1"

    def _pack_tag(self) -> bytes:
        return ("%d,%d,%d,%d" % (self.search_size, self.precision, self.anchor_num, int(self.with_mask))).encode()

    def save_packed(self, path: str):
        blob = self.weight_blob()
        torch.cuda.synchronize(self._device)
        with open(path, "wb") as f:
            tag = self._pack_tag()
            f.write(self._PACK_MAGIC + len(tag).to_bytes(4, "little") + tag + blob.numel().to_bytes(8, "little"))
            f.write(blob.cpu().numpy().tobytes())

    def load_packed(self, path: str):
        if not self._engine.value:
            raise RuntimeError("call .to(cuda device) first")
        with open(path, "rb") as f:
            if f.read(len(self._PACK_MAGIC)) != self._PACK_MAGIC:
                raise ValueError("not a siammask_b200 packed-weight file")
            tag = f.read(int.from_bytes(f.read(4), "little"))
            n = int.from_bytes(f.read(8), "little")
            blob = self.weight_blob()
            if tag.split(b",")[2:] != self._pack_tag().split(b",")[2:] or n != blob.numel():
                raise ValueError(f"packed weights were written for a different engine configuration ({tag!r})")
            data = np.frombuffer(f.read(n), dtype=np.uint8)
        blob.copy_(torch.from_numpy(data.copy()))
        torch.cuda.synchronize(self._device)
        self.adopt_weights()
        return self

    def _prep(self, t: torch.Tensor, size: int) -> torch.Tensor:
        if not self._engine.value:
            raise RuntimeError("call .to(cuda device) (and load weights) before inference")
        if t.dim() != 4 or t.shape[1] != 3 or t.shape[2] != size or t.shape[3] != size:
            raise ValueError(f"expected [B,3,{size},{size}], got {tuple(t.shape)}")
        if t.shape[0] > self.max_batch:
            raise ValueError(f"batch {t.shape[0]} > max_batch {self.max_batch}")
        t = t.to(self._device, torch.float32).contiguous()
        if self.graphs:
            buf = self._buf(("in", size, t.shape[0]), t.shape, torch.float32)
            buf.copy_(t)
            return buf
        return t

    def _buf(self, key, shape, dtype):
        if not self.graphs:
            return torch.empty(*shape, device=self._device, dtype=dtype)
        b = self._io.get(key)
        if b is None:
            b = self._io[key] = torch.empty(*shape, device=self._device, dtype=dtype)
        return b

    def _stream(self):
        if self.graphs:
            return C.c_void_p(self._gstream.cuda_stream)
        return C.c_void_p(torch.cuda.current_stream(self._device).cuda_stream)

    def _fence_in(self):
        if self.graphs:
            self._gstream.wait_stream(torch.cuda.current_stream(self._device))

    def _fence_out(self):
        if self.graphs:
            torch.cuda.current_stream(self._device).wait_stream(self._gstream)

    def _check_slots(self, slots, B: int, distinct: bool) -> torch.Tensor:
        if not (isinstance(slots, torch.Tensor) and slots.is_cuda and slots.dtype == torch.int32):
            raise ValueError("slots must be an int32 CUDA tensor")
        if slots.device != self._device:
            raise ValueError(f"slots live on {slots.device}, the engine on {self._device}")
        if slots.dim() != 1 or slots.numel() != B:
            raise ValueError(f"slots must have shape [{B}], got {tuple(slots.shape)}")
        host = slots.cpu().numpy()
        if ((host < 0) | (host >= self.num_slots)).any():
            raise ValueError(f"slot table entries must lie in [0, {self.num_slots})")
        if distinct and np.unique(host).size != B:
            raise ValueError("slot table entries must be distinct")
        return slots.contiguous()

    def _stage_slots(self, slots: torch.Tensor) -> torch.Tensor:
        if self.graphs:
            buf = self._buf(("slots", slots.numel()), (slots.numel(),), torch.int32)
            buf.copy_(slots)
            return buf
        return slots

    def _check_hp(self, hp, B: int) -> torch.Tensor:
        if not (isinstance(hp, torch.Tensor) and hp.is_cuda and hp.dtype == torch.float64):
            raise ValueError("hp must be a float64 CUDA tensor")
        if hp.device != self._device:
            raise ValueError(f"hp lives on {hp.device}, the engine on {self._device}")
        if tuple(hp.shape) != (B, 3):
            raise ValueError(f"hp must have shape [{B}, 3], got {tuple(hp.shape)}")
        if not bool(torch.isfinite(hp).all()):
            raise ValueError("hp entries must be finite")
        return hp.contiguous()

    def _stage_hp(self, hp: torch.Tensor) -> torch.Tensor:
        if self.graphs:
            buf = self._buf(("hp", hp.shape[0]), tuple(hp.shape), torch.float64)
            buf.copy_(hp)
            return buf
        return hp

    @torch.no_grad()
    def template(self, z, slot0: int = 0, slots=None):
        if slots is not None:
            slots = self._check_slots(slots, z.shape[0], distinct=True)
        z = self._prep(z, 127)
        with torch.cuda.device(self._device):
            if slots is not None:
                slots = self._stage_slots(slots)
            self._fence_in()
            if slots is None:
                _lib.check(self._lib.sm_template(self._engine, slot0, z.shape[0], z.data_ptr(), self._stream()))
            else:
                _lib.check(self._lib.sm_template_slots(self._engine, z.shape[0], slots.data_ptr(), z.data_ptr(),
                                                       self._stream()))
            self._fence_out()
        self._keep_slots = slots

    def _track(self, x, slot0, flags):
        x = self._prep(x, self.search_size)
        B, A, R = x.shape[0], self.anchor_num, self.score_size
        cls = self._buf(("cls", B), (B, 2 * A, R, R), torch.float32)
        loc = self._buf(("loc", B), (B, 4 * A, R, R), torch.float32)
        mask = None
        if flags & _lib.SM_TRACK_MASK_HEAD:
            mask = self._buf(("mask", B), (B, 63 * 63, R, R), torch.float32)
        with torch.cuda.device(self._device):
            self._fence_in()
            _lib.check(self._lib.sm_track(self._engine, slot0, B, x.data_ptr(), cls.data_ptr(), loc.data_ptr(),
                                          mask.data_ptr() if mask is not None else None, flags, self._stream()))
            self._fence_out()
        self._last_B = B
        return cls, loc, mask

    @torch.no_grad()
    def track(self, x, slot0: int = 0):
        cls, loc, _ = self._track(x, slot0, 0)
        return cls, loc

    @torch.no_grad()
    def track_mask(self, x, slot0: int = 0, mask_head: bool = True):
        flags = _lib.SM_TRACK_MASK_FEATURES | (_lib.SM_TRACK_MASK_HEAD if mask_head else 0)
        return self._track(x, slot0, flags)

    @torch.no_grad()
    def track_refine(self, pos):
        B = self._last_B
        R = self.score_size
        if isinstance(pos, torch.Tensor) and pos.is_cuda:
            p = pos.to(self._device, torch.int32).reshape(-1, 2)
        else:
            host = np.asarray(pos.cpu() if isinstance(pos, torch.Tensor) else pos, dtype=np.int64).reshape(-1, 2)
            if ((host < 0) | (host >= R)).any():
                raise IndexError(f"refine position out of range [0,{R})")
            p = torch.as_tensor(host.astype(np.int32), device=self._device)
        if p.shape[0] == 1 and B > 1:
            p = p.expand(B, 2)
        p = p.contiguous()
        if p.shape[0] != B:
            raise ValueError(f"pos has {p.shape[0]} rows, last track had batch {B}")
        if self.graphs:
            pb = self._buf(("pos", B), (B, 2), torch.int32)
            pb.copy_(p)
            p = pb
        out = self._buf(("refine", B), (B, 127 * 127), torch.float32)
        with torch.cuda.device(self._device):
            self._fence_in()
            _lib.check(self._lib.sm_refine(self._engine, B, p.data_ptr(), out.data_ptr(), self._stream()))
            self._fence_out()
        return out

    @torch.no_grad()
    def select(self, cls, loc, anchors, window, target_sz_in_crop, penalty_k: float, window_influence: float):
        B = cls.shape[0]
        dev = self._device
        anchors = anchors.to(dev, torch.float32).contiguous()
        window = window.to(dev, torch.float32).contiguous()
        tsz = torch.as_tensor(target_sz_in_crop).to(dev, torch.float64).reshape(B, 2).contiguous()
        n = self.anchor_num * self.score_size ** 2
        if anchors.shape != (n, 4) or window.numel() != n:
            raise ValueError(f"anchors/window must have {n} entries")
        best = torch.empty(B, dtype=torch.int32, device=dev)
        pos = torch.empty(B, 2, dtype=torch.int32, device=dev)
        rec = torch.empty(B, 8, dtype=torch.float32, device=dev)
        with torch.cuda.device(dev):
            self._fence_in()
            _lib.check(self._lib.sm_select(self._engine, B, cls.data_ptr(), loc.data_ptr(), anchors.data_ptr(),
                                           window.data_ptr(), tsz.data_ptr(), float(penalty_k),
                                           float(window_influence), best.data_ptr(), pos.data_ptr(), rec.data_ptr(),
                                           self._stream()))
            self._fence_out()
        return best, pos, rec

    @torch.no_grad()
    def step(self, x, anchors, window, target_sz_in_crop, penalty_k: float, window_influence: float, slot0: int = 0,
             refine: bool = True, mask_head: bool = False, mask_col: bool = False, slots=None, hp=None):
        B = x.shape[0]
        if slots is not None:
            slots = self._check_slots(slots, B, distinct=False)
        if hp is not None:
            hp = self._check_hp(hp, B)
            if slots is None:
                if slot0 < 0 or slot0 + B > self.num_slots:
                    raise ValueError(f"slots {slot0}..{slot0 + B - 1} outside [0, {self.num_slots})")
                slots = torch.arange(slot0, slot0 + B, dtype=torch.int32, device=self._device)
        return self._step(x, anchors, window, target_sz_in_crop, penalty_k, window_influence, slot0, refine, mask_head,
                          mask_col, slots, hp)

    def _step(self, x, anchors, window, target_sz_in_crop, penalty_k, window_influence, slot0=0, refine=True,
              mask_head=False, mask_col=False, slots=None, hp=None):
        x = self._prep(x, self.search_size)
        dev = self._device
        B, A, R = x.shape[0], self.anchor_num, self.score_size
        n = A * R * R
        anchors = anchors.to(dev, torch.float32).contiguous()
        window = window.to(dev, torch.float32).contiguous()
        if anchors.shape != (n, 4) or window.numel() != n:
            raise ValueError(f"anchors/window must have {n} entries")
        tsz = torch.as_tensor(target_sz_in_crop).to(dev, torch.float64).reshape(B, 2).contiguous()
        flags = (_lib.SM_TRACK_MASK_FEATURES if (refine or mask_head) else 0) | (_lib.SM_TRACK_MASK_HEAD if mask_head else 0)
        out = {"cls": self._buf(("cls", B), (B, 2 * A, R, R), torch.float32),
               "loc": self._buf(("loc", B), (B, 4 * A, R, R), torch.float32),
               "mask": self._buf(("mask", B), (B, 63 * 63, R, R), torch.float32) if mask_head else None,
               "best": self._buf(("best", B), (B,), torch.int32), "pos": self._buf(("spos", B), (B, 2), torch.int32),
               "records": self._buf(("rec", B), (B, 8), torch.float32),
               "refine": self._buf(("refine", B), (B, 127 * 127), torch.float32) if refine else None,
               "mask_col": self._buf(("mcol", B), (B, 63 * 63), torch.float32) if (mask_col and mask_head) else None}
        if self.graphs:
            tb = self._buf(("tsz", B), (B, 2), torch.float64)
            tb.copy_(tsz)
            tsz = tb

        def ptr(t):
            return t.data_ptr() if t is not None else None
        outs = (ptr(out["cls"]), ptr(out["loc"]), ptr(out["mask"]), ptr(out["best"]), ptr(out["pos"]),
                ptr(out["records"]), ptr(out["refine"]), ptr(out["mask_col"]), self._stream())
        with torch.cuda.device(dev):
            if slots is not None:
                slots = self._stage_slots(slots)
            if hp is not None:
                hp = self._stage_hp(hp)
            self._fence_in()
            if hp is not None:
                _lib.check(self._lib.sm_step_slots_hp(self._engine, B, slots.data_ptr(), hp.data_ptr(), x.data_ptr(),
                                                      tsz.data_ptr(), anchors.data_ptr(), window.data_ptr(), flags,
                                                      *outs))
            elif slots is None:
                _lib.check(self._lib.sm_step(self._engine, slot0, B, x.data_ptr(), tsz.data_ptr(), anchors.data_ptr(),
                                             window.data_ptr(), float(penalty_k), float(window_influence), flags, *outs))
            else:
                _lib.check(self._lib.sm_step_slots(self._engine, B, slots.data_ptr(), x.data_ptr(), tsz.data_ptr(),
                                                   anchors.data_ptr(), window.data_ptr(), float(penalty_k),
                                                   float(window_influence), flags, *outs))
            self._fence_out()
        self._last_B = B
        self._keep = (anchors, window, tsz, slots, hp)
        return out

    def export(self, what: str) -> torch.Tensor:
        shape = (C.c_int64 * 4)()
        with torch.cuda.device(self._device):
            _lib.check(self._lib.sm_export(self._engine, what.encode(), None, shape, self._stream()))
            out = torch.empty(*[int(s) for s in shape], device=self._device, dtype=torch.float32)
            self._fence_in()
            _lib.check(self._lib.sm_export(self._engine, what.encode(), out.data_ptr(), shape, self._stream()))
            self._fence_out()
        return out

    def profile(self, on: bool):
        _lib.check(self._lib.sm_profile_enable(self._engine, int(on)))

    def profile_dump(self):
        n = int(self._lib.sm_profile_dump(self._engine, None, 0))
        if n < 0:
            _lib.check(-1)
        buf = C.create_string_buffer(n + 16)
        if int(self._lib.sm_profile_dump(self._engine, buf, n + 16)) < 0:
            _lib.check(-1)
        rows = []
        for line in buf.value.decode().splitlines():
            name, cat, ms, fl, by = line.split("\t")
            rows.append((name, cat, float(ms), float(fl), float(by)))
        return rows

    @property
    def launch_count(self) -> int:
        return int(self._lib.sm_launch_count(self._engine))

    @property
    def device_bytes(self) -> int:
        return int(self._lib.sm_engine_bytes(self._engine))

    @property
    def handle(self):
        return self._engine

    def _destroy(self):
        if self._engine.value:
            self._lib.sm_engine_destroy(self._engine)
            self._engine = C.c_void_p(None)

    def __del__(self):
        try:
            self._destroy()
        except Exception:
            pass
```

Measured before the change: 3736.

## Stage GEMM epilogue through shared memory with TMA residual loads and stores

Replaces the identity-block residual segment, which added the residual as extra K-blocks of MMA against a diagonal weight block, with a producer-side TMA load of the residual tile into a per-warpgroup shared staging buffer, applied in the epilogue with a scale. Epilogue outputs (split fp16 planes or f32 NHWC) are written swizzled into staging and emitted with TMA bulk stores, guarded by free/res mbarriers. BLOCK_K becomes adaptive (64 or 32) to fit the staging buffers, which shrinks the pipeline ring. The packed-weight format changes because the diagonal columns are removed. This trades fewer MMA iterations and coalesced stores for lower pipeline depth and extra synchronization.

```diff
diff --git a/siammask_b200/csrc/common.cuh b/siammask_b200/csrc/common.cuh
--- a/siammask_b200/csrc/common.cuh
+++ b/siammask_b200/csrc/common.cuh
@@ -33,6 +33,7 @@
   const float* beta = nullptr;
   const __half* res_hi = nullptr;
   const __half* res_lo = nullptr;
+  float res_scale = 1.f;
   __half* out_hi = nullptr;
   __half* out_lo = nullptr;
   float* out_f32 = nullptr;
@@ -48,7 +49,6 @@
 
 struct GemmSegment {
   CUtensorMap tmA[2];
-  int kind;
   int mode;
   int num_kb, cblks, KW;
   int stride, pad, dil;
@@ -59,6 +59,9 @@
   GemmSegment seg[2];
   int nseg;
   CUtensorMap tmB[2];
+  CUtensorMap tmO[2];
+  CUtensorMap tmR[2];
+  int has_res;
   int M, Cout, Ho, Wo;
   int n_tiles, m_tiles;
   int reverse_m;
@@ -107,7 +110,7 @@
 bool gemm_conv_supported(const ConvGeom& g);
 void launch_gemm_conv(const Act& in, const ConvGeom& g, const __half* w_hi, const __half* w_lo, int cout_pad,
                       const Epilogue& ep, int nsplit, int num_sms, cudaStream_t st);
-void launch_gemm_multi(const GemmInput* convs, int nconv, const Act* residual, int res_col0, const __half* w_hi,
+void launch_gemm_multi(const GemmInput* convs, int nconv, const Act* residual, const __half* w_hi,
                        const __half* w_lo, int cout_pad, int w_ld, const Epilogue& ep, int nsplit, int num_sms,
                        cudaStream_t st, bool reverse_m = false);
 
diff --git a/siammask_b200/csrc/conv_gemm_sm90.cu b/siammask_b200/csrc/conv_gemm_sm90.cu
--- a/siammask_b200/csrc/conv_gemm_sm90.cu
+++ b/siammask_b200/csrc/conv_gemm_sm90.cu
@@ -11,7 +11,7 @@
 namespace {
 
 constexpr int BLOCK_M = 128;
-constexpr int BLOCK_K = 64;
+constexpr int WG_ROWS = 64;
 constexpr int CIN_GRAIN = 64;
 constexpr int MMA_K = 16;
 constexpr int SMEM_LIMIT = 227 * 1024;
@@ -22,34 +22,55 @@
 
 template <int BLOCK_N, int NSPLIT>
 struct Cfg {
+  static constexpr int STAGING_BYTES = WG_ROWS * BLOCK_N * 4;
+  static constexpr int RING_BYTES = SMEM_LIMIT - 2048 - 2 * STAGING_BYTES;
+  static constexpr int stage_bytes(int bk) { return NSPLIT * (BLOCK_M + BLOCK_N) * bk * 2; }
+  static constexpr int BLOCK_K = RING_BYTES / stage_bytes(64) >= 3 ? 64 : 32;
+  static constexpr int SW = BLOCK_K * 2;
   static constexpr int A_TILE_BYTES = BLOCK_M * BLOCK_K * 2;
   static constexpr int B_TILE_BYTES = BLOCK_N * BLOCK_K * 2;
   static constexpr int STAGE_BYTES = NSPLIT * (A_TILE_BYTES + B_TILE_BYTES);
-  static constexpr int RAW_STAGES = (SMEM_LIMIT - 2048) / STAGE_BYTES;
+  static constexpr int RAW_STAGES = RING_BYTES / STAGE_BYTES;
   static constexpr int STAGES = RAW_STAGES > 6 ? 6 : RAW_STAGES;
-  static constexpr int SMEM_BYTES = STAGES * STAGE_BYTES + 1024  + 256 ;
+  static constexpr int SMEM_BYTES = STAGES * STAGE_BYTES + 2 * STAGING_BYTES + 1024  + 256 ;
   static constexpr int ACC = BLOCK_N / 2;
-  static_assert(STAGES >= 2, "pipeline needs at least two stages");
+  static constexpr int H_BOX = BLOCK_N < 64 ? BLOCK_N : 64;
+  static constexpr int F_BOX = BLOCK_N < 32 ? BLOCK_N : 32;
+  static constexpr int H_PLANE = WG_ROWS * BLOCK_N * 2;
+  static_assert(STAGES >= 3, "pipeline needs at least three stages");
   static_assert(BLOCK_N % 16 == 0 && BLOCK_N >= 16 && BLOCK_N <= 128, "N tile (register accumulators)");
-  static_assert(B_TILE_BYTES % 1024 == 0, "stage parts stay 1024-aligned (swizzle atoms)");
+  static_assert(STAGE_BYTES % 1024 == 0 && B_TILE_BYTES % 1024 == 0, "stage parts stay 1024-aligned (swizzle atoms)");
   static_assert(SMEM_BYTES <= SMEM_LIMIT, "shared memory budget");
 };
 
 __device__ __forceinline__ int m_block(const GemmParams& p, int tile) {
   const int mb = tile / p.n_tiles;
   return p.reverse_m ? p.m_tiles - 1 - mb : mb;
+}
+
+template <int SPAN>
+__device__ __forceinline__ uint32_t swizzle(uint32_t o) {
+  return o ^ (((o >> 7) & (SPAN / 16 - 1)) << 4);
+}
+
+__device__ __forceinline__ void named_barrier_sync(int id, int threads) {
+  asm volatile("bar.sync %0, %1;" ::"r"(id), "r"(threads) : "memory");
 }
 
 template <int BLOCK_N, int NSPLIT>
 __global__ void __launch_bounds__(NUM_THREADS, 1) conv_gemm_kernel(const __grid_constant__ GemmParams p) {
   using C = Cfg<BLOCK_N, NSPLIT>;
   constexpr int STAGES = C::STAGES;
+  constexpr int BLOCK_K = C::BLOCK_K;
   constexpr int A_TILE_BYTES = C::A_TILE_BYTES;
 
   extern __shared__ uint8_t smem_raw[];
-  uint8_t* smem = reinterpret_cast<uint8_t*>((reinterpret_cast<uintptr_t>(smem_raw) + 1023) & ~uintptr_t(1023));
-  uint64_t* full_bar = reinterpret_cast<uint64_t*>(smem + STAGES * C::STAGE_BYTES);
+  uint8_t* smem = smem_raw + ((1024u - (smem_u32(smem_raw) & 1023u)) & 1023u);
+  uint8_t* staging = smem + STAGES * C::STAGE_BYTES;
+  uint64_t* full_bar = reinterpret_cast<uint64_t*>(staging + 2 * C::STAGING_BYTES);
   uint64_t* empty_bar = full_bar + STAGES;
+  uint64_t* free_bar = empty_bar + STAGES;
+  uint64_t* res_bar = free_bar + 2;
 
   const int warp = __shfl_sync(0xffffffffu, (int)(threadIdx.x >> 5), 0);
   const int lane = threadIdx.x & 31;
@@ -63,6 +84,10 @@
     for (int s = 0; s < STAGES; ++s) {
       mbar_init(&full_bar[s], 1);
       mbar_init(&empty_bar[s], NUM_CONSUMER_WARPS);
+    }
+    for (int w = 0; w < 2; ++w) {
+      mbar_init(&free_bar[w], 1);
+      mbar_init(&res_bar[w], 1);
     }
     fence_barrier_init();
   }
@@ -74,14 +99,8 @@
     const bool leader = elect_one();
     int stage = 0;
     uint32_t phase = 0;
-    auto acquire = [&](uint32_t bytes) {
-      mbar_wait(&empty_bar[stage], phase ^ 1);
-      if (leader) mbar_arrive_expect_tx(&full_bar[stage], bytes);
-    };
-    auto load_2d = [&](void* dst, const CUtensorMap* map, int c0, int c1) {
-      if (leader) tma_load_2d(dst, map, &full_bar[stage], c0, c1);
-    };
-    for (int tile = blockIdx.x; tile < num_tiles; tile += gridDim.x) {
+    uint32_t iter = 0;
+    for (int tile = blockIdx.x; tile < num_tiles; tile += gridDim.x, ++iter) {
       const int m0 = m_block(p, tile) * BLOCK_M;
       const int n0 = (tile % p.n_tiles) * BLOCK_N;
       const int q = m0 % p.Wo;
@@ -90,46 +109,55 @@
       const int nb = t / p.Ho;
       for (int sgi = 0; sgi < p.nseg; ++sgi) {
         const GemmSegment& sg = p.seg[sgi];
-        if (sg.kind == 1) {
-#pragma unroll 1
-          for (int kb = 0; kb < BLOCK_N / BLOCK_K; ++kb) {
-            acquire(C::STAGE_BYTES);
-            uint8_t* st = smem + stage * C::STAGE_BYTES;
-#pragma unroll
-            for (int s = 0; s < NSPLIT; ++s) {
-              load_2d(st + s * A_TILE_BYTES, &sg.tmA[s], n0 + kb * BLOCK_K, m0);
-              load_2d(st + NSPLIT * A_TILE_BYTES + s * C::B_TILE_BYTES, &p.tmB[s], sg.b_col0 + n0 + kb * BLOCK_K, n0);
-            }
-            __syncwarp();
-            if (++stage == STAGES) { stage = 0; phase ^= 1; }
-          }
-          continue;
-        }
         const int wb = q * sg.stride - sg.pad;
         const int hb = pq * sg.stride - sg.pad;
 #pragma unroll 1
         for (int kb = 0; kb < sg.num_kb; ++kb) {
-          acquire(C::STAGE_BYTES);
+          mbar_wait(&empty_bar[stage], phase ^ 1);
+          if (leader) mbar_arrive_expect_tx(&full_bar[stage], C::STAGE_BYTES);
           uint8_t* st = smem + stage * C::STAGE_BYTES;
           const int tap = kb / sg.cblks;
           const int c0 = (kb - tap * sg.cblks) * BLOCK_K;
 #pragma unroll
           for (int s = 0; s < NSPLIT; ++s) {
             uint8_t* a_dst = st + s * A_TILE_BYTES;
-            if (sg.mode == 0) {
-              load_2d(a_dst, &sg.tmA[s], c0, m0);
-            } else if (leader) {
-              const int r = tap / sg.KW;
-              const int sx = tap - r * sg.KW;
-              tma_load_im2col_4d(a_dst, &sg.tmA[s], &full_bar[stage], c0, wb, hb, nb,
-                                 static_cast<uint16_t>(sx * sg.dil), static_cast<uint16_t>(r * sg.dil));
+            if (leader) {
+              if (sg.mode == 0) {
+                tma_load_2d(a_dst, &sg.tmA[s], &full_bar[stage], c0, m0);
+              } else {
+                const int r = tap / sg.KW;
+                const int sx = tap - r * sg.KW;
+                tma_load_im2col_4d(a_dst, &sg.tmA[s], &full_bar[stage], c0, wb, hb, nb,
+                                   static_cast<uint16_t>(sx * sg.dil), static_cast<uint16_t>(r * sg.dil));
+              }
+              tma_load_2d(st + NSPLIT * A_TILE_BYTES + s * C::B_TILE_BYTES, &p.tmB[s], &full_bar[stage],
+                          sg.b_col0 + kb * BLOCK_K, n0);
             }
-            load_2d(st + NSPLIT * A_TILE_BYTES + s * C::B_TILE_BYTES, &p.tmB[s], sg.b_col0 + kb * BLOCK_K, n0);
           }
           __syncwarp();
           if (++stage == STAGES) { stage = 0; phase ^= 1; }
         }
       }
+      if (p.has_res) {
+#pragma unroll 1
+        for (int w = 0; w < 2; ++w) {
+          mbar_wait(&free_bar[w], iter & 1);
+          const int r0 = m0 + w * WG_ROWS;
+          if (leader) {
+            mbar_arrive_expect_tx(&res_bar[w], r0 < p.M ? NSPLIT * C::H_PLANE : 0);
+            if (r0 < p.M) {
+              uint8_t* dst = staging + w * C::STAGING_BYTES;
+#pragma unroll
+              for (int s = 0; s < NSPLIT; ++s)
+#pragma unroll
+                for (int b = 0; b < BLOCK_N / C::H_BOX; ++b)
+                  tma_load_2d(dst + s * C::H_PLANE + b * (WG_ROWS * C::H_BOX * 2), &p.tmR[s], &res_bar[w],
+                              n0 + b * C::H_BOX, r0);
+            }
+          }
+          __syncwarp();
+        }
+      }
     }
     return;
   }
@@ -137,29 +165,30 @@
   setmaxnreg_inc<CONSUMER_REGS>();
   const int wg = (warp >> 2) - 1;
   const int wl = warp & 3;
+  const bool store_thread = wl == 0 && lane == 0;
   const Epilogue& ep = p.ep;
   const int HoWo = p.Ho * p.Wo;
+  uint8_t* my_staging = staging + wg * C::STAGING_BYTES;
   float acc[C::ACC];
   float acc2[C::ACC];
   int stage = 0;
   uint32_t phase = 0;
-  for (int tile = blockIdx.x; tile < num_tiles; tile += gridDim.x) {
+  uint32_t iter = 0;
+  for (int tile = blockIdx.x; tile < num_tiles; tile += gridDim.x, ++iter) {
 #pragma unroll
     for (int i = 0; i < C::ACC; ++i) { acc[i] = 0.f; acc2[i] = 0.f; }
     int prev = -1;
     for (int sgi = 0; sgi < p.nseg; ++sgi) {
-      const GemmSegment& sg = p.seg[sgi];
-      const bool ident = sg.kind == 1;
-      const int nkb = ident ? BLOCK_N / BLOCK_K : sg.num_kb;
+      const int nkb = p.seg[sgi].num_kb;
 #pragma unroll 1
       for (int kb = 0; kb < nkb; ++kb) {
         mbar_wait(&full_bar[stage], phase);
-        const uint32_t a_hi = smem_u32(smem + stage * C::STAGE_BYTES) + wg * (64 * BLOCK_K * 2);
+        const uint32_t a_hi = smem_u32(smem + stage * C::STAGE_BYTES) + wg * (WG_ROWS * BLOCK_K * 2);
         const uint32_t b_hi = smem_u32(smem + stage * C::STAGE_BYTES) + NSPLIT * A_TILE_BYTES;
-        const uint64_t da_hi0 = wgmma_desc_kmajor<128>(a_hi);
-        const uint64_t db_hi0 = wgmma_desc_kmajor<128>(b_hi);
-        const uint64_t da_lo0 = wgmma_desc_kmajor<128>(a_hi + A_TILE_BYTES);
-        const uint64_t db_lo0 = wgmma_desc_kmajor<128>(b_hi + C::B_TILE_BYTES);
+        const uint64_t da_hi0 = wgmma_desc_kmajor<C::SW>(a_hi);
+        const uint64_t db_hi0 = wgmma_desc_kmajor<C::SW>(b_hi);
+        const uint64_t da_lo0 = wgmma_desc_kmajor<C::SW>(a_hi + A_TILE_BYTES);
+        const uint64_t db_lo0 = wgmma_desc_kmajor<C::SW>(b_hi + C::B_TILE_BYTES);
         wgmma_fence();
 #pragma unroll
         for (int k = 0; k < BLOCK_K / MMA_K; ++k) {
@@ -175,6 +204,9 @@
         if (prev >= 0) {
           __syncwarp();
           if (lane == 0) mbar_arrive(&empty_bar[prev]);
+        } else if (store_thread) {
+          tma_store_wait_read<0>();
+          mbar_arrive(&free_bar[wg]);
         }
         prev = stage;
         if (++stage == STAGES) { stage = 0; phase ^= 1; }
@@ -186,18 +218,55 @@
     __syncwarp();
     if (lane == 0) mbar_arrive(&empty_bar[prev]);
 
-    const int row0 = m_block(p, tile) * BLOCK_M + wg * 64 + wl * 16 + (lane >> 2);
-    const int col0 = (tile % p.n_tiles) * BLOCK_N + 2 * (lane & 3);
+    const int m0 = m_block(p, tile) * BLOCK_M + wg * WG_ROWS;
+    const int n0 = (tile % p.n_tiles) * BLOCK_N;
+    const int rl = wl * 16 + (lane >> 2);
+    const int cl = 2 * (lane & 3);
+    if (ep.out_mode == OUT_NCHW_F32) {
+#pragma unroll
+      for (int h = 0; h < 2; ++h) {
+        const int m = m0 + rl + 8 * h;
+        if (m >= p.M) continue;
+        const int b = m / HoWo;
+        const int hw = m - b * HoWo;
+#pragma unroll
+        for (int j = 0; j < BLOCK_N / 8; ++j) {
+          const int n = n0 + cl + 8 * j;
+          float v0 = acc[4 * j + 2 * h], v1 = acc[4 * j + 2 * h + 1];
+          if constexpr (NSPLIT == 2) {
+            v0 += acc2[4 * j + 2 * h];
+            v1 += acc2[4 * j + 2 * h + 1];
+          }
+          const float2 al = __ldg(reinterpret_cast<const float2*>(ep.alpha + n));
+          const float2 be = __ldg(reinterpret_cast<const float2*>(ep.beta + n));
+          v0 = fmaf(v0, al.x, be.x);
+          v1 = fmaf(v1, al.y, be.y);
+          if (ep.relu) {
+            v0 = fmaxf(v0, 0.f);
+            v1 = fmaxf(v1, 0.f);
+          }
+          if (n < p.Cout) {
+            float* dst = ep.out_f32 + (static_cast<size_t>(b) * p.Cout + n) * HoWo + hw;
+            __stcs(dst, v0);
+            if (n + 1 < p.Cout) __stcs(dst + HoWo, v1);
+          }
+        }
+      }
+      continue;
+    }
+
+    mbar_wait(p.has_res ? &res_bar[wg] : &free_bar[wg], iter & 1);
+    const bool split = ep.out_mode == OUT_NHWC_SPLIT;
+    const bool two_planes = ep.out_lo != nullptr;
     float amax = 0.f;
 #pragma unroll
     for (int h = 0; h < 2; ++h) {
-      const int m = row0 + 8 * h;
-      if (m >= p.M) continue;
-      const int b = m / HoWo;
-      const int hw = m - b * HoWo;
+      const int r = rl + 8 * h;
+      const bool row_in = m0 + r < p.M;
 #pragma unroll
       for (int j = 0; j < BLOCK_N / 8; ++j) {
-        const int n = col0 + 8 * j;
+        const int c = cl + 8 * j;
+        const int n = n0 + c;
         float v0 = acc[4 * j + 2 * h], v1 = acc[4 * j + 2 * h + 1];
         if constexpr (NSPLIT == 2) {
           v0 += acc2[4 * j + 2 * h];
@@ -207,39 +276,54 @@
         const float2 be = __ldg(reinterpret_cast<const float2*>(ep.beta + n));
         v0 = fmaf(v0, al.x, be.x);
         v1 = fmaf(v1, al.y, be.y);
-        const size_t off = static_cast<size_t>(m) * p.Cout + n;
-        if (ep.res_hi != nullptr) {
-          const float2 f = __half22float2(*reinterpret_cast<const __half2*>(ep.res_hi + off));
-          v0 += f.x;
-          v1 += f.y;
-          if (ep.res_lo != nullptr) {
-            const float2 l = __half22float2(*reinterpret_cast<const __half2*>(ep.res_lo + off));
-            v0 += l.x;
-            v1 += l.y;
+        const uint32_t oh = (c / C::H_BOX) * (WG_ROWS * C::H_BOX * 2) +
+                            swizzle<C::H_BOX * 2>(r * (C::H_BOX * 2) + (c % C::H_BOX) * 2);
+        if (p.has_res) {
+          float2 f = __half22float2(*reinterpret_cast<const __half2*>(my_staging + oh));
+          if constexpr (NSPLIT == 2) {
+            const float2 l = __half22float2(*reinterpret_cast<const __half2*>(my_staging + C::H_PLANE + oh));
+            f.x += l.x;
+            f.y += l.y;
           }
+          v0 += f.x * ep.res_scale;
+          v1 += f.y * ep.res_scale;
         }
         if (ep.relu) {
           v0 = fmaxf(v0, 0.f);
           v1 = fmaxf(v1, 0.f);
         }
-        if (ep.out_mode == OUT_NHWC_SPLIT) {
-          amax = fmaxf(amax, fmaxf(fabsf(v0), fabsf(v1)));
+        if (split) {
+          if (row_in) amax = fmaxf(amax, fmaxf(fabsf(v0), fabsf(v1)));
           const __half2 hv = __floats2half2_rn(v0, v1);
           const float2 hf = __half22float2(hv);
-          *reinterpret_cast<__half2*>(ep.out_hi + off) = hv;
-          if (ep.out_lo != nullptr)
-            *reinterpret_cast<__half2*>(ep.out_lo + off) = __floats2half2_rn(v0 - hf.x, v1 - hf.y);
-        } else if (ep.out_mode == OUT_NHWC_F32) {
-          *reinterpret_cast<float2*>(ep.out_f32 + off) = make_float2(v0, v1);
-        } else if (n < p.Cout) {
-          float* dst = ep.out_f32 + (static_cast<size_t>(b) * p.Cout + n) * HoWo + hw;
-          __stcs(dst, v0);
-          if (n + 1 < p.Cout) __stcs(dst + HoWo, v1);
+          *reinterpret_cast<__half2*>(my_staging + oh) = hv;
+          if (two_planes)
+            *reinterpret_cast<__half2*>(my_staging + C::H_PLANE + oh) = __floats2half2_rn(v0 - hf.x, v1 - hf.y);
+        } else {
+          const uint32_t of = (c / C::F_BOX) * (WG_ROWS * C::F_BOX * 4) +
+                              swizzle<C::F_BOX * 4>(r * (C::F_BOX * 4) + (c % C::F_BOX) * 4);
+          *reinterpret_cast<float2*>(my_staging + of) = make_float2(v0, v1);
         }
       }
     }
-    if (ep.out_mode == OUT_NHWC_SPLIT) flag_if_out_of_range(amax, ep.ovf);
-  }
+    fence_proxy_async();
+    named_barrier_sync(1 + wg, 128);
+    if (store_thread && m0 < p.M) {
+      if (split) {
+        for (int s = 0; s < (two_planes ? 2 : 1); ++s)
+#pragma unroll
+          for (int b = 0; b < BLOCK_N / C::H_BOX; ++b)
+            tma_store_2d(&p.tmO[s], my_staging + s * C::H_PLANE + b * (WG_ROWS * C::H_BOX * 2), n0 + b * C::H_BOX, m0);
+      } else {
+#pragma unroll
+        for (int b = 0; b < BLOCK_N / C::F_BOX; ++b)
+          tma_store_2d(&p.tmO[0], my_staging + b * (WG_ROWS * C::F_BOX * 4), n0 + b * C::F_BOX, m0);
+      }
+      tma_store_commit();
+    }
+    if (split) flag_if_out_of_range(amax, ep.ovf);
+  }
+  if (store_thread) tma_store_wait_all();
 }
 
 using EncodeTiledFn = CUresult (*)(CUtensorMap*, CUtensorMapDataType, cuuint32_t, void*, const cuuint64_t*,
@@ -349,18 +433,6 @@
   return cached_map(k, [&] { return make_map_im2col_raw(base, in, g, bk); });
 }
 
-template <int BLOCK_N, int NSPLIT>
-void launch_cfg(const GemmParams& p, int num_sms, cudaStream_t st) {
-  using C = Cfg<BLOCK_N, NSPLIT>;
-  auto kern = conv_gemm_kernel<BLOCK_N, NSPLIT>;
-  static unsigned long long attr_done = 0;
-  ensure_dynamic_smem(kern, C::SMEM_BYTES, attr_done);
-  const int tiles = p.m_tiles * p.n_tiles;
-  const int grid = tiles < num_sms ? tiles : num_sms;
-  kern<<<grid, NUM_THREADS, C::SMEM_BYTES, st>>>(p);
-  SMK_CUDA(cudaGetLastError());
-}
-
 }
 
 static CUtensorMap make_map_2d_any_raw(const __half* base, uint64_t inner, uint64_t outer, uint32_t box_inner, uint32_t box_outer,
@@ -426,34 +498,83 @@
   return (cout + 255) / 256 * 256;
 }
 
+static CUtensorMap make_map_2d_f32(const float* base, uint64_t inner, uint64_t outer, uint32_t box_inner,
+                                   uint32_t box_outer, int swizzle_bytes) {
+  MapKey k{};
+  k.v[0] = 6; k.v[1] = (uint64_t)base; k.v[2] = inner; k.v[3] = outer; k.v[4] = box_inner; k.v[5] = box_outer;
+  k.v[6] = (uint64_t)swizzle_bytes;
+  return cached_map(k, [&] {
+    CUtensorMap m;
+    cuuint64_t dims[2] = {inner, outer};
+    cuuint64_t strides[1] = {inner * sizeof(float)};
+    cuuint32_t box[2] = {box_inner, box_outer};
+    cuuint32_t estr[2] = {1, 1};
+    const CUtensorMapSwizzle sw = swizzle_bytes == 128 ? CU_TENSOR_MAP_SWIZZLE_128B
+                                  : swizzle_bytes == 64 ? CU_TENSOR_MAP_SWIZZLE_64B : CU_TENSOR_MAP_SWIZZLE_32B;
+    CUresult r = driver_api().tiled(&m, CU_TENSOR_MAP_DATA_TYPE_FLOAT32, 2, const_cast<float*>(base), dims, strides,
+                                    box, estr, CU_TENSOR_MAP_INTERLEAVE_NONE, sw, CU_TENSOR_MAP_L2_PROMOTION_L2_128B,
+                                    CU_TENSOR_MAP_FLOAT_OOB_FILL_NONE);
+    SMK_CHECK(r == CUDA_SUCCESS, "cuTensorMapEncodeTiled (f32) failed, code " + std::to_string((int)r));
+    return m;
+  });
+}
+
+template <int BLOCK_N, int NSPLIT>
+static void launch_cfg(GemmParams& p, const GemmInput* convs, const __half* w_hi, const __half* w_lo, int cout_pad,
+                       int w_ld, int num_sms, cudaStream_t st) {
+  using C = Cfg<BLOCK_N, NSPLIT>;
+  constexpr int bk = C::BLOCK_K;
+  for (int i = 0; i < p.nseg; ++i) {
+    const ConvGeom& g = convs[i].g;
+    const Act& in = convs[i].in;
+    GemmSegment& sg = p.seg[i];
+    sg.cblks = g.Cin / bk;
+    sg.num_kb = g.KH * g.KW * sg.cblks;
+    for (int s = 0; s < NSPLIT; ++s) {
+      const __half* a = s == 0 ? in.hi : in.lo;
+      sg.tmA[s] = sg.mode == 0 ? make_map_2d(a, g.Cin, (uint64_t)in.M(), bk, BLOCK_M) : make_map_im2col(a, in, g, bk);
+    }
+    if (NSPLIT == 1) sg.tmA[1] = sg.tmA[0];
+  }
+  if (p.nseg == 1) p.seg[1] = p.seg[0];
+  for (int s = 0; s < NSPLIT; ++s) p.tmB[s] = make_map_2d(s == 0 ? w_hi : w_lo, (uint64_t)w_ld, cout_pad, bk, BLOCK_N);
+  if (NSPLIT == 1) p.tmB[1] = p.tmB[0];
+
+  auto kern = conv_gemm_kernel<BLOCK_N, NSPLIT>;
+  static unsigned long long attr_done = 0;
+  ensure_dynamic_smem(kern, C::SMEM_BYTES, attr_done);
+  const int tiles = p.m_tiles * p.n_tiles;
+  const int grid = tiles < num_sms ? tiles : num_sms;
+  kern<<<grid, NUM_THREADS, C::SMEM_BYTES, st>>>(p);
+  SMK_CUDA(cudaGetLastError());
+}
+
 void launch_gemm_conv(const Act& in, const ConvGeom& g, const __half* w_hi, const __half* w_lo, int cout_pad,
                       const Epilogue& ep, int nsplit, int num_sms, cudaStream_t st) {
   GemmInput gi{in, g, 0};
-  launch_gemm_multi(&gi, 1, nullptr, -1, w_hi, w_lo, cout_pad, g.KH * g.KW * g.Cin, ep, nsplit, num_sms, st);
-}
-
-void launch_gemm_multi(const GemmInput* convs, int nconv, const Act* residual, int res_col0, const __half* w_hi,
-                       const __half* w_lo, int cout_pad, int w_ld, const Epilogue& ep_in, int nsplit, int num_sms,
+  launch_gemm_multi(&gi, 1, nullptr, w_hi, w_lo, cout_pad, g.KH * g.KW * g.Cin, ep, nsplit, num_sms, st);
+}
+
+void launch_gemm_multi(const GemmInput* convs, int nconv, const Act* residual, const __half* w_hi,
+                       const __half* w_lo, int cout_pad, int w_ld, const Epilogue& ep, int nsplit, int num_sms,
                        cudaStream_t st, bool reverse_m) {
   SMK_CHECK(nconv >= 1 && nconv <= 2, "1 or 2 convolution segments");
-  SMK_CHECK(nconv + (residual != nullptr ? 1 : 0) <= 2, "at most two K segments");
-  Epilogue ep = ep_in;
   const ConvGeom& g0 = convs[0].g;
   const Act& in0 = convs[0].in;
   const int Ho = g0.out_size(in0.H), Wo = g0.out_size(in0.W);
   GemmParams p;
+  std::memset(&p, 0, sizeof p);
   p.M = in0.B * Ho * Wo;
   p.Cout = g0.Cout;
   p.Ho = Ho;
   p.Wo = Wo;
   const int block_n = cout_pad < 128 ? cout_pad : 128;
-  const int bk = BLOCK_K;
   SMK_CHECK(cout_pad % block_n == 0, "cout_pad must be a multiple of the N tile");
   if (ep.out_mode != OUT_NCHW_F32) SMK_CHECK(g0.Cout == cout_pad, "NHWC outputs need Cout to match the padded tile width");
   p.n_tiles = cout_pad / block_n;
   p.m_tiles = (p.M + BLOCK_M - 1) / BLOCK_M;
   p.reverse_m = reverse_m ? 1 : 0;
-  p.nseg = 0;
+  p.nseg = nconv;
   for (int i = 0; i < nconv; ++i) {
     const ConvGeom& g = convs[i].g;
     const Act& in = convs[i].in;
@@ -461,10 +582,7 @@
     SMK_CHECK(in.C == g.Cin && g.Cout == g0.Cout && in.B == in0.B, "segment channels/batch mismatch");
     SMK_CHECK(g.out_size(in.H) == Ho && g.out_size(in.W) == Wo, "segments must produce the same output size");
     SMK_CHECK(nsplit == 1 || (in.lo != nullptr && w_lo != nullptr), "exact mode needs lo planes");
-    GemmSegment& sg = p.seg[p.nseg++];
-    sg.kind = 0;
-    sg.cblks = g.Cin / bk;
-    sg.num_kb = g.KH * g.KW * sg.cblks;
+    GemmSegment& sg = p.seg[i];
     sg.KW = g.KW;
     sg.stride = g.stride;
     sg.pad = g.pad;
@@ -472,39 +590,33 @@
     sg.mode = (g.KH == 1 && g.KW == 1 && g.stride == 1 && g.pad == 0) ? 0 : 1;
     sg.b_col0 = convs[i].w_col0;
     SMK_CHECK(sg.b_col0 % 64 == 0 && sg.b_col0 + g.KH * g.KW * g.Cin <= w_ld, "weight column range");
-    for (int s = 0; s < nsplit; ++s) {
-      const __half* a = s == 0 ? in.hi : in.lo;
-      sg.tmA[s] = sg.mode == 0 ? make_map_2d(a, g.Cin, (uint64_t)in.M(), bk, BLOCK_M) : make_map_im2col(a, in, g, bk);
-    }
-    if (nsplit == 1) sg.tmA[1] = sg.tmA[0];
+  }
+  const uint32_t hbox = block_n < 64 ? block_n : 64, fbox = block_n < 32 ? block_n : 32;
+  auto aligned = [](const void* q) { return (reinterpret_cast<uintptr_t>(q) & 15) == 0; };
+  if (ep.out_mode == OUT_NHWC_SPLIT) {
+    SMK_CHECK(aligned(ep.out_hi) && (ep.out_lo == nullptr || aligned(ep.out_lo)), "NHWC output planes 16-byte aligned");
+    for (int s = 0; s < (ep.out_lo != nullptr ? 2 : 1); ++s)
+      p.tmO[s] = make_map_2d_any(s == 0 ? ep.out_hi : ep.out_lo, (uint64_t)p.Cout, (uint64_t)p.M, hbox, 64, hbox * 2);
+  } else if (ep.out_mode == OUT_NHWC_F32) {
+    SMK_CHECK(aligned(ep.out_f32), "NHWC fp32 output 16-byte aligned");
+    p.tmO[0] = make_map_2d_f32(ep.out_f32, (uint64_t)p.Cout, (uint64_t)p.M, fbox, 64, fbox * 4);
   }
   if (residual != nullptr) {
-    SMK_CHECK(res_col0 >= 0 && res_col0 % 64 == 0 && res_col0 + g0.Cout <= w_ld && block_n % 64 == 0,
-              "identity segment needs a diagonal block in the packed weights");
+    SMK_CHECK(ep.out_mode == OUT_NHWC_SPLIT, "a residual needs an NHWC split-plane output");
     SMK_CHECK(residual->C == g0.Cout && residual->M() == p.M, "residual shape");
     SMK_CHECK(nsplit == 1 || residual->lo != nullptr, "exact mode residual needs both planes");
-    GemmSegment& sg = p.seg[p.nseg++];
-    sg.kind = 1;
-    sg.mode = 0;
-    sg.num_kb = block_n / bk;
-    sg.cblks = sg.KW = sg.stride = sg.dil = 1;
-    sg.pad = 0;
-    sg.b_col0 = res_col0;
+    SMK_CHECK(aligned(residual->hi) && (nsplit == 1 || aligned(residual->lo)), "residual planes 16-byte aligned");
+    p.has_res = 1;
     for (int s = 0; s < nsplit; ++s)
-      sg.tmA[s] = make_map_2d(s == 0 ? residual->hi : residual->lo, g0.Cout, (uint64_t)p.M, bk, BLOCK_M);
-    if (nsplit == 1) sg.tmA[1] = sg.tmA[0];
-    ep.res_hi = ep.res_lo = nullptr;
-  }
-  if (p.nseg == 1) p.seg[1] = p.seg[0];
-  for (int s = 0; s < nsplit; ++s)
-    p.tmB[s] = make_map_2d(s == 0 ? w_hi : w_lo, (uint64_t)w_ld, cout_pad, bk, block_n);
-  if (nsplit == 1) p.tmB[1] = p.tmB[0];
+      p.tmR[s] = make_map_2d_any(s == 0 ? residual->hi : residual->lo, (uint64_t)p.Cout, (uint64_t)p.M, hbox, 64,
+                                 hbox * 2);
+  }
   p.ep = ep;
 
-#define SMK_DISPATCH(BN)                                             \
-  case BN:                                                           \
-    if (nsplit == 2) launch_cfg<BN, 2>(p, num_sms, st);              \
-    else launch_cfg<BN, 1>(p, num_sms, st);                          \
+#define SMK_DISPATCH(BN)                                                                         \
+  case BN:                                                                                       \
+    if (nsplit == 2) launch_cfg<BN, 2>(p, convs, w_hi, w_lo, cout_pad, w_ld, num_sms, st);       \
+    else launch_cfg<BN, 1>(p, convs, w_hi, w_lo, cout_pad, w_ld, num_sms, st);                   \
     break;
   switch (block_n) {
     SMK_DISPATCH(16)
diff --git a/siammask_b200/csrc/engine.cu b/siammask_b200/csrc/engine.cu
--- a/siammask_b200/csrc/engine.cu
+++ b/siammask_b200/csrc/engine.cu
@@ -26,8 +26,8 @@
   std::string conv_key, bn_key;
   ConvGeom g2{};
   std::string conv_key2, bn_key2;
-  bool fused2 = false, has_diag = false;
-  int w_ld = 0, col2 = 0, col_diag = -1;
+  bool fused2 = false;
+  int w_ld = 0, col2 = 0;
   size_t off_beta2 = 0;
   float* beta2 = nullptr;
   size_t off_whi = 0, off_wlo = 0, off_wref = 0, off_alpha = 0, off_beta = 0;
@@ -391,8 +391,6 @@
         c3.g2 = ds.g;
         c3.conv_key2 = ds.conv_key;
         c3.bn_key2 = ds.bn_key;
-      } else {
-        c3.has_diag = true;
       }
       inplanes = sp.planes * 4;
     }
@@ -432,7 +430,6 @@
     const size_t K = (size_t)w.g.KH * w.g.KW * w.g.Cin;
     w.w_ld = (int)K;
     if (w.fused2) { w.col2 = w.w_ld; w.w_ld += w.g2.KH * w.g2.KW * w.g2.Cin; }
-    if (w.has_diag) { w.col_diag = w.w_ld; w.w_ld += w.g.Cout; }
     if (w.gemm_ok) {
       w.off_whi = off; off = align_up(off + (size_t)w.cout_pad * w.w_ld * sizeof(__half));
       w.off_wlo = off; off = align_up(off + (size_t)w.cout_pad * w.w_ld * sizeof(__half));
@@ -707,12 +704,7 @@
     beta2[n] = (float)std::ldexp(L.shift[n] + (L2 ? L2->shift[n] : 0.0), L.s_out);
     alpha[n] = std::ldexp(1.f, L.s_out - L.s_in);
     if (!L.gemm_ok) continue;
-    int e = weight_exp(amax);
-    if (L.has_diag) {
-      const int d = L.s_in - L.s_res;
-      e = std::max(-14 - d, std::min(14 - d, e));
-      SMK_CHECK(e >= -24 && e <= 24, "activation scales of a residual block are too far apart");
-    }
+    const int e = weight_exp(amax);
     alpha[n] = std::ldexp(1.f, L.s_out - L.s_in - e);
     __half* rh = w_hi + (size_t)n * ld;
     __half* rl = w_lo + (size_t)n * ld;
@@ -728,7 +720,6 @@
       rh[L.col2 + k] = h;
       rl[L.col2 + k] = __float2half_rn(fw - __half2float(h));
     }
-    if (L.has_diag) rh[L.col_diag + n] = __float2half_rn(std::ldexp(1.f, e + L.s_in - L.s_res));
   }
 }
 
@@ -989,15 +980,12 @@
   const bool reverse = !use_patch && end_of(*big) > 0;
   GemmInput gi[2] = {{in, Lw.g, 0}, {in, Lw.g, 0}};
   int nconv = 1;
-  const Act* ident = nullptr;
   if (in2 != nullptr) {
     gi[1] = {*in2, Lw.g2, Lw.col2};
     nconv = 2;
     ep.beta = Lw.beta2;
-  } else if (res != nullptr) {
-    if (Lw.has_diag) ident = res;
-    else { ep.res_hi = res->hi; ep.res_lo = res->lo; }
-  }
+  }
+  if (res != nullptr) ep.res_scale = std::ldexp(1.f, Lw.s_out - Lw.s_res);
   launch(st, 1, Lw.conv_key, "conv_gemm", flops, bytes, [&] {
     const int now_end = reverse ? -1 : +1;
     last_end_[in.hi] = now_end;
@@ -1007,7 +995,7 @@
     if (use_patch)
       launch_conv3x3_patch(in, Lw.g, Lw.w_hi, Lw.w_lo, Lw.w_ld, ep, exact_ ? 2 : 1, num_sms_, st);
     else
-      launch_gemm_multi(gi, nconv, ident, Lw.col_diag, Lw.w_hi, Lw.w_lo, Lw.cout_pad, Lw.w_ld, ep, exact_ ? 2 : 1,
+      launch_gemm_multi(gi, nconv, res, Lw.w_hi, Lw.w_lo, Lw.cout_pad, Lw.w_ld, ep, exact_ ? 2 : 1,
                         num_sms_, st, reverse);
   });
 }
diff --git a/siammask_b200/custom.py b/siammask_b200/custom.py
--- a/siammask_b200/custom.py
+++ b/siammask_b200/custom.py
@@ -141,7 +141,7 @@
         _lib.check(self._lib.sm_engine_status(self._engine, C.byref(v)))
         return int(v.value)
 
-    _PACK_MAGIC = b"SMB200PK1"
+    _PACK_MAGIC = b"SMB200PK2"
 
     def _pack_tag(self) -> bytes:
         return ("%d,%d,%d,%d" % (self.search_size, self.precision, self.anchor_num, int(self.with_mask))).encode()
@@ -158,7 +158,11 @@
         if not self._engine.value:
             raise RuntimeError("call .to(cuda device) first")
         with open(path, "rb") as f:
-            if f.read(len(self._PACK_MAGIC)) != self._PACK_MAGIC:
+            magic = f.read(len(self._PACK_MAGIC))
+            if magic != self._PACK_MAGIC:
+                if magic.startswith(self._PACK_MAGIC[:-1]):
+                    raise ValueError(f"packed-weight file of another arena layout ({magic!r}; this engine reads "
+                                     f"{self._PACK_MAGIC!r}): pack the weights again")
                 raise ValueError("not a siammask_b200 packed-weight file")
             tag = f.read(int.from_bytes(f.read(4), "little"))
             n = int.from_bytes(f.read(8), "little")
```

New measurement: 4533, median of 6. +21.3%, better.
